# nv-tlabs/ChronoEdit

Measured on AMD Instinct MI355X. Metric: denoising-steps/sec, higher is better.
Workload: dtype bf16

## Files before the change

### chronoedit_amd/csrc/ce_attn.hip

```cpp
#include <cstdlib>

#include "ce_common.h"

namespace {

constexpr int HD = 128;
constexpr int QW = 32;
constexpr int KVB = 64;
constexpr int K_TILE_BYTES = KVB * HD * 2;
constexpr int VT_TILE_BYTES = HD * KVB * 2;
constexpr int BUF_BYTES = K_TILE_BYTES + VT_TILE_BYTES;
constexpr int OST_ROW = HD * 2 + 16;
constexpr int smem_bytes(int nwave, bool two_seg) {
  const int stage = nwave * QW * OST_ROW;
  return two_seg ? 2 * BUF_BYTES + stage : (stage > 2 * BUF_BYTES ? stage : 2 * BUF_BYTES);
}
constexpr float NEG_BIG = -1.0e30f;

__device__ __forceinline__ int vt_swz(int dv) {
  return ((((dv >> 2) & 7) << 1) | (((dv >> 1) ^ (dv >> 5)) & 1)) ^ (((dv >> 6) & 1) << 1);
}

struct KVSeg {
  const bf16* k;
  const bf16* v;
  int len;
  int ldk;
  int ldv;
};
struct BlkRows {
  int rows;
  int stride;
  uint32_t magic;
  int vt_cols;
  unsigned char* q8;
  unsigned char* s8;
  int ld8;
};

template <bool TWO_SEG, int NWAVE>
__global__ __launch_bounds__(NWAVE * 64, NWAVE == 8 ? 2 : 2) void attn_fwd_kernel(const bf16* __restrict__ Q, bf16* __restrict__ O, KVSeg seg0,
                                                       KVSeg seg1, int Nq, int H, int ldq, int ldo, int nqb,
                                                       float scale_log2e) {
  extern __shared__ __attribute__((aligned(16))) unsigned char smem[];
  {
    const size_t bz = blockIdx.y;
    Q += bz * Nq * ldq;
    O += bz * Nq * ldo;
    seg0.k += bz * seg0.len * seg0.ldk;
    seg0.v += bz * seg0.len * seg0.ldv;
    if (TWO_SEG) {
      seg1.k += bz * seg1.len * seg1.ldk;
      seg1.v += bz * seg1.len * seg1.ldv;
    }
  }
  const int tid = threadIdx.x, lane = tid & 63, wave = tid >> 6;
  const int l31 = lane & 31, hh = lane >> 5;

  int head, qb;
  if ((H & 7) == 0) {
    const int xcd = blockIdx.x & 7, local = blockIdx.x >> 3;
    head = xcd + 8 * (local / nqb);
    qb = local % nqb;
  } else {
    head = blockIdx.x / nqb;
    qb = blockIdx.x % nqb;
  }
  constexpr int QB = QW * NWAVE;
  constexpr int NT = NWAVE * 64;
  const int q0 = qb * QB + wave * QW;
  const int hoff = head * HD;

// ... 175 lines not shown
#pragma unroll
  for (int i = 0; i < 8; ++i) {
    const int c = lane + 64 * i;
    const int rl = c >> 4, cc = c & 15;
    const int q = q0 + rl;
    if (q < Nq) {
      const u32x4 v = *reinterpret_cast<const u32x4*>(smem + (TWO_SEG ? 2 * BUF_BYTES : 0) + (size_t)(wave * QW + rl) * OST_ROW + cc * 16);
      *reinterpret_cast<u32x4*>(O + (size_t)q * ldo + hoff + cc * 8) = v;
    }
  }
}


#define CE_EPOCH_BARRIER()                          \
  asm volatile("s_waitcnt lgkmcnt(0)" ::: "memory"); \
  __builtin_amdgcn_s_barrier()
constexpr int PK_ROW = HD * 2 + 16;
constexpr int PV_ROW = KVB * 2 + 16;
constexpr int PK_TILE = KVB * PK_ROW;
constexpr int PV_TILE = HD * PV_ROW;
typedef __attribute__((ext_vector_type(4))) unsigned pp_u4;
typedef __attribute__((ext_vector_type(2))) unsigned pp_u2;

constexpr int K_GRP = 1088;
typedef __attribute__((address_space(3))) void lds_void;
#ifdef CE_DIAGNOSTICS
__device__ unsigned long long g_sp_exact_hits = 0ull;
#endif
constexpr float SP_SPEC_THR = 1024.0f;
constexpr int SP_V0 = 2 * PK_TILE;
constexpr int SP_TILE_BYTES = 2 * PK_TILE + 3 * PV_TILE;
constexpr int sp_smem_bytes(bool two_seg) { return two_seg ? SP_TILE_BYTES + 8 * QW * OST_ROW : SP_TILE_BYTES; }

template <bool TWO_SEG, bool VT = false, bool QOUT = false>
__global__ __launch_bounds__(512, 2) void attn_fwd_sp_kernel(const bf16* __restrict__ Q_, bf16* __restrict__ O_, KVSeg seg0_,
                                                              KVSeg seg1_, int Nq, int H, int ldq, int ldo, int nqb,
                                                              float scale_log2e, int batch, BlkRows blk) {
  extern __shared__ __attribute__((aligned(16))) unsigned char smem[];
  constexpr int NWAVE = 8, QB = QW * NWAVE;
  const int tid = threadIdx.x, lane = tid & 63;
  const int wave = __builtin_amdgcn_readfirstlane(tid >> 6);
  const int l31 = lane & 31, hh = lane >> 5;
  for (int item = blockIdx.x; item < nqb * H * batch; item += gridDim.x) {
  const bf16* Q = Q_;
  bf16* O = O_;
  KVSeg seg0 = seg0_, seg1 = seg1_;

  int head, qb, bz;
  {
    const int nqb_full = Nq / QB;
    if ((H & 7) == 0) {
      const int xcd = item & 7, local = item >> 3, hx_n = H >> 3;
      const int full = batch * hx_n * nqb_full;
      if (local < full) {
        bz = local / (hx_n * nqb_full);
        const int r = local % (hx_n * nqb_full);
        head = xcd + 8 * (r / nqb_full);
        qb = r % nqb_full;
      } else {
        const int l2 = local - full;
        bz = l2 / hx_n;
        head = xcd + 8 * (l2 % hx_n);
        qb = nqb_full;
      }
    } else {
      bz = item / (nqb * H);
      const int r = item % (nqb * H);
      head = r / nqb;
      qb = r % nqb;
    }
  }
  {
    if (VT && blk.rows > 0) {
      Q += (size_t)bz * blk.rows * ldq;
      O += (size_t)bz * blk.rows * ldo;
      seg0.k += (size_t)bz * blk.rows * seg0.ldk;
      seg0.v += (size_t)bz * blk.vt_cols;
    } else {
      Q += (size_t)bz * Nq * ldq;
      O += (size_t)bz * Nq * ldo;
      seg0.k += (size_t)bz * seg0.len * seg0.ldk;
      seg0.v += VT ? (size_t)bz * (TWO_SEG ? blk.vt_cols : seg0.len) : (size_t)bz * seg0.len * seg0.ldv;
    }
    if (TWO_SEG) {
      seg1.k += (size_t)bz * seg1.len * seg1.ldk;
      seg1.v += VT ? (size_t)bz * blk.stride : (size_t)bz * seg1.len * seg1.ldv;
    }
  }
  const int q0 = qb * QB + wave * QW;
  const int hoff = head * HD;
  const bool active = q0 < Nq;
  const int q0row = (VT && blk.rows > 0) ? (q0 / blk.rows) * blk.stride + q0 % blk.rows : q0;

  bf16x8 qf[8];
  {
    const bf16* qrow = Q + (size_t)(q0 + l31 < Nq ? q0row + l31 : 0) * ldq + hoff + 8 * hh;
#pragma unroll
    for (int ks = 0; ks < 8; ++ks) qf[ks] = *reinterpret_cast<const bf16x8*>(qrow + 16 * ks);
  }
  auto scale_q = [&]() __attribute__((always_inline)) {
#pragma unroll
  for (int ks = 0; ks < 8; ++ks) {
    const u32x4 w = __builtin_bit_cast(u32x4, qf[ks]);
    u32x4 o;
#pragma unroll
    for (int i = 0; i < 4; ++i) o[i] = pack_bf16(bf16lo(w[i]) * scale_log2e, bf16hi(w[i]) * scale_log2e);
    qf[ks] = __builtin_bit_cast(bf16x8, o);
  }
#pragma unroll
  for (int ks = 0; ks < 8; ++ks) asm volatile("" : "+v"(qf[ks]));

  };
  const int v_dvq = (tid & 1) | (((tid >> 4) & 15) << 1), v_kvq = ((tid >> 1) & 7) | (((tid >> 8) & 1) << 3);
  const int v_chunk = (v_kvq & ~3) | ((v_kvq & 1) << 1) | ((v_kvq >> 1) & 1);
  unsigned char* ost = smem + (TWO_SEG ? SP_TILE_BYTES : 0) + (size_t)(wave * QW + l31) * OST_ROW;
  const int k_w = l31 & 3;
  const unsigned char* k_rd = smem + (l31 >> 2) * K_GRP + k_w * 256 + ((hh ^ (k_w & 1)) << 4);
  const int k_eo[2] = {(k_w >> 1) << 5, ((k_w >> 1) ^ 1) << 5};
  const unsigned char* v_rd = smem + SP_V0 + l31 * PV_ROW + hh * 16;
  int vt_off[4];
#pragma unroll
  for (int s4 = 0; s4 < 4; ++s4) {
    const int x = (l31 >> 1) & 7;
    vt_off[s4] = l31 * 128 + ((2 * (s4 ^ (x >> 1)) + (hh ^ (x & 1))) << 4);
  }
  unsigned char* v_wr = smem + SP_V0 + (4 * v_dvq) * PV_ROW + v_chunk * 8;

#pragma unroll
  for (int sidx = 0; sidx < (TWO_SEG ? 2 : 1); ++sidx) {
    const KVSeg sg = sidx == 0 ? seg0 : seg1;
    const int ntiles = (sg.len + KVB - 1) / KVB;
    const int k_rows_span = (VT && blk.rows > 0) ? ((sg.len - 1) / blk.rows) * blk.stride + blk.rows : sg.len;
    const auto k_rsrc = __builtin_amdgcn_make_buffer_rsrc((void*)(sg.k + hoff), 0, (k_rows_span - 1) * sg.ldk * 2 + HD * 2, 0x00020000);
// ... 862 lines not shown
CE_API int ce_set_attention_waves(int nwave) {
  const int old = g_attn_nwave;
  if (nwave == 0 || nwave == 4 || nwave == 8 || nwave == 16 || nwave == 64 || nwave == 128 || nwave == 129) g_attn_nwave = nwave;
  return old;
}
#endif

CE_API int ce_attention_batched_bf16(const void* Q, const void* K1, const void* V1, int len1, int ldk1, int ldv1,
                                         const void* K2, const void* V2, int len2, int ldk2, int ldv2, void* O, int Nq, int H,
                                         int head_dim, int ldq, int ldo, float softmax_scale, int batch, hipStream_t stream) {
  if (!Q || !K1 || !V1 || !O) return CE_ERR_ARG;
  if (head_dim != HD || Nq <= 0 || H <= 0 || len1 <= 0 || batch <= 0 || batch > 65535) return CE_ERR_SHAPE;
  if ((ldq & 7) || (ldo & 7) || (ldk1 & 7) || (ldv1 & 3)) return CE_ERR_ALIGN;
  const bool two = (K2 != nullptr && V2 != nullptr && len2 > 0);
  if (two && ((ldk2 & 7) || (ldv2 & 3))) return CE_ERR_ALIGN;
  KVSeg s0{(const bf16*)K1, (const bf16*)V1, len1, ldk1, ldv1};
  KVSeg s1{(const bf16*)K2, (const bf16*)V2, two ? len2 : 0, ldk2, ldv2};
  const float sl2 = softmax_scale * 1.4426950408889634f;
  const bool sp = g_attn_nwave == 64 || g_attn_nwave == 0 || g_attn_nwave >= 128;
  const int nwave = sp ? 8 : g_attn_nwave;
  const int nqb = (Nq + nwave * QW - 1) / (nwave * QW);
  dim3 grid(nqb * H, batch), block(nwave * 64);
  if (sp) {
#define CE_ATTN_SP(TWO)                                                                                              \
  do {                                                                                                               \
    static bool done_[CE_MAX_DEVICES] = {};                                                                          \
    bool& done = done_[ce_device_slot()];                                                                            \
    if (!done) {                                                                                                     \
      (void)hipFuncSetAttribute((const void*)attn_fwd_sp_kernel<TWO>, hipFuncAttributeMaxDynamicSharedMemorySize,    \
                                sp_smem_bytes(TWO));                                                                 \
      done = true;                                                                                                   \
    }                                                                                                                \
    hipLaunchKernelGGL((attn_fwd_sp_kernel<TWO>), dim3(nqb * H * batch), block, sp_smem_bytes(TWO), stream, (const bf16*)Q, \
                       (bf16*)O, s0, s1, Nq, H, ldq, ldo, nqb, sl2, batch, BlkRows{0, 0, 0u, 0});                    \
  } while (0)
    if (two) CE_ATTN_SP(true); else CE_ATTN_SP(false);
#undef CE_ATTN_SP
    return (int)hipGetLastError();
  }
#define CE_ATTN_LAUNCH(TWO, NW)                                                                                     \
  do {                                                                                                              \
    static bool done_[CE_MAX_DEVICES] = {};                                                                         \
    bool& done = done_[ce_device_slot()];                                                                           \
    if (!done) {                                                                                                    \
      (void)hipFuncSetAttribute((const void*)attn_fwd_kernel<TWO, NW>, hipFuncAttributeMaxDynamicSharedMemorySize,  \
                                smem_bytes(NW, TWO));                                                               \
      done = true;                                                                                                  \
    }                                                                                                               \
    hipLaunchKernelGGL((attn_fwd_kernel<TWO, NW>), grid, block, smem_bytes(NW, TWO), stream, (const bf16*)Q, (bf16*)O, \
                       s0, s1, Nq, H, ldq, ldo, nqb, sl2);                                                          \
  } while (0)
  if (two) {
    if (nwave == 8) CE_ATTN_LAUNCH(true, 8); else CE_ATTN_LAUNCH(true, 4);
  } else {
    if (nwave == 8) CE_ATTN_LAUNCH(false, 8); else CE_ATTN_LAUNCH(false, 4);
  }
#undef CE_ATTN_LAUNCH
  return (int)hipGetLastError();
}

CE_API int ce_attention_bf16(const void* Q, const void* K1, const void* V1, int len1, int ldk1, int ldv1, const void* K2,
                                 const void* V2, int len2, int ldk2, int ldv2, void* O, int Nq, int H, int head_dim, int ldq,
                                 int ldo, float softmax_scale, hipStream_t stream) {
  return ce_attention_batched_bf16(Q, K1, V1, len1, ldk1, ldv1, K2, V2, len2, ldk2, ldv2, O, Nq, H, head_dim, ldq, ldo,
                                   softmax_scale, 1, stream);
}

CE_API int ce_v_transpose_bf16(const void* v, int ldv, void* vt, int ldvt, int n_keys, int H, hipStream_t stream) {
  if (!v || !vt) return CE_ERR_ARG;
  if (n_keys <= 0 || H <= 0 || ldvt < n_keys) return CE_ERR_SHAPE;
  if ((ldv & 3) || (ldvt & 7)) return CE_ERR_ALIGN;
  hipLaunchKernelGGL(v_transpose_kernel, dim3((ldvt + KVB - 1) / KVB, H), dim3(256), 0, stream, (const bf16*)v, ldv, (bf16*)vt, ldvt, n_keys, 0, 0, 0);
  return (int)hipGetLastError();
}

CE_API int ce_v_transpose_blocked_bf16(const void* v, int ldv, void* vt, int ldvt, int n_keys, int H, int batch, int blk_rows, int blk_stride,
                                           int vt_sample_cols, hipStream_t stream) {
  if (!v || !vt) return CE_ERR_ARG;
  if (n_keys <= 0 || H <= 0 || batch <= 0 || blk_rows <= 0 || (blk_rows & 63) || blk_stride < batch * blk_rows || (vt_sample_cols & 63) ||
      vt_sample_cols < (n_keys + KVB - 1) / KVB * KVB || ldvt < batch * vt_sample_cols)
    return CE_ERR_SHAPE;
  if ((ldv & 3) || (ldvt & 7)) return CE_ERR_ALIGN;
  hipLaunchKernelGGL(v_transpose_kernel, dim3(vt_sample_cols / KVB, H, batch), dim3(256), 0, stream, (const bf16*)v, ldv, (bf16*)vt, ldvt, n_keys,
                     blk_rows, blk_stride, vt_sample_cols);
  return (int)hipGetLastError();
}

#ifdef CE_DIAGNOSTICS
extern "C" int ce_attn16_launch(const void* Q, const void* K, const void* Vt, int len, int ldk, int ldvt, void* O, int Nq, int H, int ldq, int ldo,
                                float sl2, int batch, int cus, hipStream_t stream);
#endif

static int attention_vt_launch(const void* Q, const void* K, const void* Vt, int len, int ldk, int ldvt, void* O, int Nq, int H, int head_dim,
                               int ldq, int ldo, float softmax_scale, int batch, int blk_rows, int blk_stride, int vt_sample_cols,
                               hipStream_t stream) {
  if (!Q || !K || !Vt || !O) return CE_ERR_ARG;
  if (head_dim != HD || Nq <= 0 || H <= 0 || len <= 0 || batch <= 0 || batch > 65535) return CE_ERR_SHAPE;
  const int ntiles_cols = (len + KVB - 1) / KVB * KVB;
  if (blk_rows == 0) {
    vt_sample_cols = len;
    if (ldvt < (batch - 1) * len + ntiles_cols) return CE_ERR_SHAPE;
  } else {
    if ((blk_rows & 63) || blk_stride < batch * blk_rows || (Nq % blk_rows) || vt_sample_cols < ntiles_cols ||
        ldvt < (batch - 1) * vt_sample_cols + ntiles_cols)
      return CE_ERR_SHAPE;
  }
  if ((ldq & 7) || (ldo & 7) || (ldk & 7) || (ldvt & 7) || (batch > 1 && (vt_sample_cols & 1))) return CE_ERR_ALIGN;
  KVSeg s0{(const bf16*)K, (const bf16*)Vt, len, ldk, ldvt};
  KVSeg s1{nullptr, nullptr, 0, 0, 0};
  BlkRows blk{blk_rows, blk_stride, 0u, vt_sample_cols};
  if (blk_rows > 0) {
    const uint32_t tps = (uint32_t)(blk_rows >> 6);
    blk.magic = tps == 1 ? 0u : (uint32_t)(((1ull << 32) + tps - 1) / tps);
  }
  const float sl2 = softmax_scale * 1.4426950408889634f;
  const int nqb = (Nq + 8 * QW - 1) / (8 * QW);
  static bool done_[CE_MAX_DEVICES] = {};
  bool& done = done_[ce_device_slot()];
  if (!done) {
    (void)hipFuncSetAttribute((const void*)attn_fwd_sp_kernel<false, true>, hipFuncAttributeMaxDynamicSharedMemorySize, sp_smem_bytes(false));
    done = true;
  }
  const int cus = ce_device_cus();
  const int items = nqb * H * batch;
#ifdef CE_DIAGNOSTICS
  if (g_attn_nwave == 16 && blk_rows == 0) {
    const int rc = ce_attn16_launch(Q, K, Vt, len, ldk, ldvt, O, Nq, H, ldq, ldo, sl2, batch, cus, stream);
    if (rc != CE_ERR_ALIGN) return rc;
  }
#endif
  if (g_attn_nwave == 128 || g_attn_nwave == 129) {
    static bool done4_[CE_MAX_DEVICES] = {};
    bool& done4 = done4_[ce_device_slot()];
    if (!done4) {
      (void)hipFuncSetAttribute((const void*)attn_fwd_w4_kernel, hipFuncAttributeMaxDynamicSharedMemorySize, W4_SMEM);
      done4 = true;
    }
    const int grid4 = (g_attn_nwave == 129 && items > cus) ? (cus & ~7) : items;
    hipLaunchKernelGGL(attn_fwd_w4_kernel, dim3(grid4), dim3(256), W4_SMEM, stream, (const bf16*)Q, (bf16*)O, s0, Nq, H, ldq, ldo, nqb,
                       sl2, batch, blk);
    return (int)hipGetLastError();
  }
  const int grid_vt = items <= 2 * cus ? items : ((2 * cus) & ~7);
  hipLaunchKernelGGL((attn_fwd_sp_kernel<false, true>), dim3(grid_vt), dim3(512), sp_smem_bytes(false), stream, (const bf16*)Q, (bf16*)O,
                     s0, s1, Nq, H, ldq, ldo, nqb, sl2, batch, blk);
  return (int)hipGetLastError();
}

CE_API int ce_attention_vt_bf16(const void* Q, const void* K, const void* Vt, int len, int ldk, int ldvt, void* O, int Nq, int H,
                                    int head_dim, int ldq, int ldo, float softmax_scale, int batch, hipStream_t stream) {
  return attention_vt_launch(Q, K, Vt, len, ldk, ldvt, O, Nq, H, head_dim, ldq, ldo, softmax_scale, batch, 0, 0, 0, stream);
}

CE_API int ce_attention_vt_blocked_bf16(const void* Q, const void* K, const void* Vt, int len, int ldk, int ldvt, void* O, int Nq, int H,
                                            int head_dim, int ldq, int ldo, float softmax_scale, int batch, int blk_rows, int blk_stride,
                                            int vt_sample_cols, hipStream_t stream) {
  if (blk_rows <= 0) return CE_ERR_SHAPE;
  return attention_vt_launch(Q, K, Vt, len, ldk, ldvt, O, Nq, H, head_dim, ldq, ldo, softmax_scale, batch, blk_rows, blk_stride, vt_sample_cols,
                             stream);
}


static int attention_2seg_vt_launch(const void* Q, const void* K1, const void* V1t, int len1, int ldk1, int ldv1t, int vt_cols1,
                                    const void* K2, const void* V2t, int len2, int ldk2, int ldv2t, int vt_cols2, void* O, int Nq,
                                    int H, int head_dim, int ldq, int ldo, float softmax_scale, int batch, void* O8, void* S8, int ldo8,
                                    hipStream_t stream) {
  if (!Q || !K1 || !V1t || !K2 || !V2t || (!O && !O8)) return CE_ERR_ARG;
  if (head_dim != HD || Nq <= 0 || H <= 0 || len1 <= 0 || len2 <= 0 || batch <= 0 || batch > 65535) return CE_ERR_SHAPE;
  const int c1 = (len1 + KVB - 1) / KVB * KVB, c2 = (len2 + KVB - 1) / KVB * KVB;
  if (vt_cols1 < len1 || vt_cols2 < len2 || ldv1t < (batch - 1) * vt_cols1 + c1 || ldv2t < (batch - 1) * vt_cols2 + c2) return CE_ERR_SHAPE;
  if ((ldq & 7) || (ldo & 7) || (ldk1 & 7) || (ldk2 & 7) || (ldv1t & 7) || (ldv2t & 7) || (vt_cols1 & 1) || (vt_cols2 & 1)) return CE_ERR_ALIGN;
  KVSeg s0{(const bf16*)K1, (const bf16*)V1t, len1, ldk1, ldv1t};
  KVSeg s1{(const bf16*)K2, (const bf16*)V2t, len2, ldk2, ldv2t};
  const float sl2 = softmax_scale * 1.4426950408889634f;
  const int nqb = (Nq + 8 * QW - 1) / (8 * QW);
  static bool done_[CE_MAX_DEVICES] = {};
  bool& done = done_[ce_device_slot()];
  if (!done) {
    (void)hipFuncSetAttribute((const void*)attn_fwd_sp_kernel<true, true>, hipFuncAttributeMaxDynamicSharedMemorySize, sp_smem_bytes(true));
    (void)hipFuncSetAttribute((const void*)attn_fwd_sp_kernel<true, true, true>, hipFuncAttributeMaxDynamicSharedMemorySize, sp_smem_bytes(true));
    done = true;
  }
  const BlkRows blk{0, vt_cols2, 0u, vt_cols1, (unsigned char*)O8, (unsigned char*)S8, ldo8};
  const int cus = ce_device_cus();
  const int items = nqb * H * batch;
  const int grid = items <= 2 * cus ? items : ((2 * cus) & ~7);
  if (O8)
    hipLaunchKernelGGL((attn_fwd_sp_kernel<true, true, true>), dim3(grid), dim3(512), sp_smem_bytes(true), stream, (const bf16*)Q,
                       (bf16*)O, s0, s1, Nq, H, ldq, ldo, nqb, sl2, batch, blk);
  else
    hipLaunchKernelGGL((attn_fwd_sp_kernel<true, true>), dim3(grid), dim3(512), sp_smem_bytes(true), stream, (const bf16*)Q, (bf16*)O,
                       s0, s1, Nq, H, ldq, ldo, nqb, sl2, batch, blk);
  return (int)hipGetLastError();
}

CE_API int ce_attention_2seg_vt_bf16(const void* Q, const void* K1, const void* V1t, int len1, int ldk1, int ldv1t, int vt_cols1,
                                         const void* K2, const void* V2t, int len2, int ldk2, int ldv2t, int vt_cols2, void* O, int Nq,
                                         int H, int head_dim, int ldq, int ldo, float softmax_scale, int batch, hipStream_t stream) {
  if (!O) return CE_ERR_ARG;
  return attention_2seg_vt_launch(Q, K1, V1t, len1, ldk1, ldv1t, vt_cols1, K2, V2t, len2, ldk2, ldv2t, vt_cols2, O, Nq, H, head_dim, ldq, ldo,
                                  softmax_scale, batch, nullptr, nullptr, 0, stream);
}

CE_API int ce_attention_2seg_vt_quant_bf16(const void* Q, const void* K1, const void* V1t, int len1, int ldk1, int ldv1t, int vt_cols1,
                                               const void* K2, const void* V2t, int len2, int ldk2, int ldv2t, int vt_cols2, void* o8,
                                               void* scale8, int Nq, int H, int head_dim, int ldq, int ldo8, float softmax_scale, int batch,
                                               hipStream_t stream) {
  if (!o8 || !scale8 || (ldo8 & 15) || ((H * head_dim) & 127)) return CE_ERR_ARG;
  return attention_2seg_vt_launch(Q, K1, V1t, len1, ldk1, ldv1t, vt_cols1, K2, V2t, len2, ldk2, ldv2t, vt_cols2, nullptr, Nq, H, head_dim, ldq,
                                  8, softmax_scale, batch, o8, scale8, ldo8, stream);
}
```

### chronoedit_amd/csrc/ce_common.h

```cpp
#pragma once
#include <hip/hip_runtime.h>
#include <stdint.h>

typedef __bf16 bf16;
typedef __attribute__((ext_vector_type(2))) __bf16 bf16x2;
typedef __attribute__((ext_vector_type(4))) __bf16 bf16x4;
typedef __attribute__((ext_vector_type(8))) __bf16 bf16x8;
typedef __attribute__((ext_vector_type(2))) float f32x2;
typedef __attribute__((ext_vector_type(4))) float f32x4;
typedef __attribute__((ext_vector_type(16))) float f32x16;
typedef __attribute__((ext_vector_type(4))) uint32_t u32x4;
typedef __attribute__((ext_vector_type(2))) uint32_t u32x2;

#define CE_WAVE 64

#define CE_API extern "C" __attribute__((visibility("default")))
#ifdef CE_DIAGNOSTICS
#define CE_KNOB static int
#define CE_DIAG_COUNT_EXACT(counter)                                        \
  do {                                                                      \
    if ((threadIdx.x & 63) == 0) atomicAdd(&(counter), 1ull);               \
  } while (0)
#else
#define CE_KNOB static constexpr int
#define CE_DIAG_COUNT_EXACT(counter) do { } while (0)
#endif

#define CE_OK 0
#define CE_ERR_ARG (-1)
#define CE_ERR_SHAPE (-2)
#define CE_ERR_ALIGN (-3)

#define CE_MAX_DEVICES 16
inline int ce_device_slot() {
  int d = 0;
  if (hipGetDevice(&d) != hipSuccess || d < 0 || d >= CE_MAX_DEVICES) d = 0;
  return d;
}

inline int ce_device_cus() {
  static int cus_[CE_MAX_DEVICES] = {};
  int& cus = cus_[ce_device_slot()];
  if (cus == 0) {
    int dev = 0, n = 0;
    cus = (hipGetDevice(&dev) == hipSuccess && hipDeviceGetAttribute(&n, hipDeviceAttributeMultiprocessorCount, dev) == hipSuccess && n > 0) ? n : 256;
  }
  return cus;
}

inline int ce_split_k(int tail, int kt, int cus, long long slab_bytes, long long ws_bytes) {
  if (tail <= 0) return 1;
  for (int s = cus / tail < 8 ? cus / tail : 8; s >= 2; --s)
    if (kt % (2 * s) == 0 && tail * s * slab_bytes <= ws_bytes) return s;
  return 1;
}

inline uint32_t ce_seg_magic(int seg_k, int bk, int kt) {
  if (seg_k <= 0 || seg_k % bk) return 0;
  const int tps = seg_k / bk;
  const uint32_t magic = 65536u / (uint32_t)tps + 1u;
  for (int t = 0; t < kt; ++t)
    if ((int)((uint32_t)t * magic >> 16) != t / tps) return 0;
  return magic;
}

__device__ __forceinline__ float bf16_bits_to_f32(uint32_t bits16) { return __uint_as_float(bits16 << 16); }
__device__ __forceinline__ float bf16lo(uint32_t packed) { return __uint_as_float(packed << 16); }
__device__ __forceinline__ float bf16hi(uint32_t packed) { return __uint_as_float(packed & 0xffff0000u); }

__device__ __forceinline__ uint32_t pack_bf16(float lo, float hi) {
  f32x2 v = {lo, hi};
  bf16x2 r = __builtin_convertvector(v, bf16x2);
  return __builtin_bit_cast(uint32_t, r);
}
__device__ __forceinline__ float round_bf16(float x) {
  bf16 b = (bf16)x;
  return (float)b;
}

__device__ __forceinline__ float mul_then_add(float y, float g, float r) {
#pragma clang fp contract(off)
  const float t = y * g;
  return r + t;
}

__device__ __forceinline__ float wave_sum(float v) {
#pragma unroll
  for (int o = 32; o > 0; o >>= 1) v += __shfl_xor(v, o, 64);
// ... 43 lines not shown
```

### chronoedit_amd/csrc/ce_gemm.hip

```cpp
#include <cmath>

#include "ce_common.h"

#define EPI_BIAS 0
#define EPI_BIAS_GELU 1
#define EPI_GATE_RES 2
#define EPI_BIAS_GELU_ERF 3
#define EPI_F32 4
#define EPI_BIAS_ROW 6
#define EPI_BIAS_T 7
#define EPI_MUL 5

namespace {

constexpr int BM = 128, BN = 128, BK = 64;
constexpr int TILE_BYTES = BM * BK * 2;
constexpr int LDC_BYTES = BN * 2 + 16;

__device__ __forceinline__ int swz_chunk(int row, int chunk) { return chunk ^ ((row >> 1) & 7); }

template <int EPI>
__global__ __launch_bounds__(256) void gemm_bf16_128(const bf16* __restrict__ A, const bf16* __restrict__ W,
                                                     bf16* __restrict__ C, const float* __restrict__ bias,
                                                     const float* __restrict__ gate, const bf16* __restrict__ res, int M,
                                                     int N, int K, int lda, int ldw, int ldc, int ldres, int gate_rows,
                                                     int tiles_m, int tiles_n, int batch0, long long sA0, long long sA1,
                                                     long long sW0, long long sW1, long long sC0, long long sC1,
                                                     int a_seg_tiles, long long a_seg_extra) {
  __shared__ __attribute__((aligned(16))) unsigned char smem[2 * 2 * TILE_BYTES];
  if (gridDim.y > 1) {
    const int z0 = blockIdx.y % batch0, z1 = blockIdx.y / batch0;
    A += z0 * sA0 + z1 * sA1;
    W += z0 * sW0 + z1 * sW1;
    const long long oc = z0 * sC0 + z1 * sC1;
    C = EPI == EPI_F32 ? reinterpret_cast<bf16*>(reinterpret_cast<float*>(C) + oc) : C + oc;
  }
  const int tid = threadIdx.x, lane = tid & 63, wave = tid >> 6;
  const int wm = wave >> 1, wn = wave & 1;

  const int nwg = tiles_m * tiles_n;
  const int wg = xcd_remap(blockIdx.x, nwg);
  constexpr int GROUP = 8;
  const int group_sz = GROUP * tiles_n;
// ... 257 lines not shown
      if (g_gemm_variant == 7 || rows_auto == 288)
        return ce_gemm288_launch(A, W, C, bias, epilogue, gate, res, M, N, K, lda, ldw, ldc, ldres, gate_rows, a_seg_k, a_seg_stride,
                                 w_seg_k, w_seg_stride, slabs, ws_bytes, stream);
      if (g_gemm_variant == 1 || g_gemm_variant == 2)
        return ce_gemm256_launch(A, W, C, bias, epilogue, gate, res, M, N, K, lda, ldw, ldc, ldres, gate_rows, a_seg_k, a_seg_stride,
                                 w_seg_k, w_seg_stride, slabs, ws_bytes, stream);
      return ce_gemm256w4_launch(A, W, C, bias, epilogue, gate, res, M, N, K, lda, ldw, ldc, ldres, gate_rows, a_seg_k, a_seg_stride,
                                 w_seg_k, w_seg_stride, g_gemm_variant == 3 ? 3 : g_gemm_variant == 5 ? 1 : 2, slabs, ws_bytes, stream);
    }
  }
  if (w_seg_k) return CE_ERR_SHAPE;
  const int a_seg_tiles = a_seg_k > 0 ? a_seg_k / BK : 0;
  const long long a_seg_extra = a_seg_k > 0 ? a_seg_stride - a_seg_k : 0;
  const int tiles_m = (M + BM - 1) / BM, tiles_n = (N + BN - 1) / BN;
  dim3 grid(tiles_m * tiles_n), block(256);
#define CE_LAUNCH(E)                                                                                              \
  hipLaunchKernelGGL(gemm_bf16_128<E>, grid, block, 0, stream, (const bf16*)A, (const bf16*)W, (bf16*)C, bias, gate, \
                     (const bf16*)res, M, N, K, lda, ldw, ldc, ldres, gate_rows, tiles_m, tiles_n, 1, 0ll, 0ll, 0ll, 0ll, 0ll, 0ll, \
                     a_seg_tiles, a_seg_extra)
  switch (epilogue) {
    case EPI_BIAS: CE_LAUNCH(EPI_BIAS); break;
    case EPI_BIAS_GELU: CE_LAUNCH(EPI_BIAS_GELU); break;
    case EPI_GATE_RES: CE_LAUNCH(EPI_GATE_RES); break;
    case EPI_BIAS_GELU_ERF: CE_LAUNCH(EPI_BIAS_GELU_ERF); break;
    case EPI_F32: CE_LAUNCH(EPI_F32); break;
    case EPI_MUL: CE_LAUNCH(EPI_MUL); break;
    case EPI_BIAS_ROW: CE_LAUNCH(EPI_BIAS_ROW); break;
    default: return CE_ERR_ARG;
  }
#undef CE_LAUNCH
  return (int)hipGetLastError();
}

CE_API int ce_gemm_batched_bf16(const void* A, const void* W, void* C, const float* bias, int epilogue, int M, int N, int K,
                                    int lda, int ldw, int ldc, int batch0, int batch1, long long sA0, long long sA1, long long sW0,
                                    long long sW1, long long sC0, long long sC1, hipStream_t stream) {
  if (!A || !W || !C) return CE_ERR_ARG;
  if (M <= 0 || N <= 0 || K <= 0 || (K % BK) || (N & 7) || batch0 <= 0 || batch1 <= 0 || (long long)batch0 * batch1 > 65535)
    return CE_ERR_SHAPE;
  if ((lda & 7) || (ldw & 7) || (ldc & 7) || (sA0 & 7) || (sA1 & 7) || (sW0 & 7) || (sW1 & 7) || (sC0 & 7) || (sC1 & 7))
    return CE_ERR_ALIGN;
  if (epilogue != EPI_BIAS && epilogue != EPI_F32) return CE_ERR_ARG;
  const int tiles_m = (M + BM - 1) / BM, tiles_n = (N + BN - 1) / BN;
  dim3 grid(tiles_m * tiles_n, batch0 * batch1), block(256);
#define CE_LAUNCH(E)                                                                                                 \
  hipLaunchKernelGGL(gemm_bf16_128<E>, grid, block, 0, stream, (const bf16*)A, (const bf16*)W, (bf16*)C, bias, nullptr, \
                     nullptr, M, N, K, lda, ldw, ldc, 0, 0, tiles_m, tiles_n, batch0, sA0, sA1, sW0, sW1, sC0, sC1, 0, 0ll)
  if (epilogue == EPI_BIAS) CE_LAUNCH(EPI_BIAS); else CE_LAUNCH(EPI_F32);
#undef CE_LAUNCH
  return (int)hipGetLastError();
}
```

### chronoedit_amd/csrc/ce_gemm256w4.hip

```cpp
#include "ce_common.h"
#include "ce_gemm_epi.h"

namespace {

constexpr int BM = 256, BN = 256, BK = 64;
constexpr int TILE = 256 * BK * 2;
constexpr int CROW = BN * 2 + 16;
constexpr int QROW = 128 * 2 + 16;

typedef __attribute__((address_space(3))) void lds_void;

#define W4_VM(N) asm volatile("s_waitcnt vmcnt(" #N ")" ::: "memory")
#define W4_LGKM0() asm volatile("s_waitcnt lgkmcnt(0)" ::: "memory")
#define W4_BAR() __builtin_amdgcn_s_barrier()
#define W4_PIN() __builtin_amdgcn_sched_barrier(0)

__device__ __forceinline__ void tile_origin_w4(int wg, int tiles_m, int tiles_n, int bn, int& m0, int& n0) {
  constexpr int GROUP = 4;
  const int group_sz = GROUP * tiles_n;
  const int gid = wg / group_sz;
  const int first_m = gid * GROUP;
  const int gm = min(tiles_m - first_m, GROUP);
  m0 = (first_m + (wg % group_sz) % gm) * BM;
  n0 = ((wg % group_sz) / gm) * bn;
}

template <int NG>
struct FragSet {
  bf16x8 a[8], b[NG];
};

#define W4_MMA(F, G, S)                                                                                                      \
  if ((G) < NG) {                                                                                                            \
    if constexpr (REGEPI)                                                                                                    \
      asm volatile("v_mfma_f32_16x16x32_bf16 %0, %1, %2, %0" : "+a"(acc[F][(G) < NG ? (G) : 0]) : "v"((S).a[F]), "v"((S).b[(G) < NG ? (G) : 0])); \
    else                                                                                                                     \
      asm volatile("v_mfma_f32_16x16x32_bf16 %0, %1, %2, %0" : "+a"(acc[F][(G) < NG ? (G) : 0]) : "v"((S).b[(G) < NG ? (G) : 0]), "v"((S).a[F])); \
  }

template <int EPI, int NSA, bool ONEBAR, bool SEG2 = false, int NG = 8>
__global__ __launch_bounds__(256) __attribute__((amdgpu_waves_per_eu(1, 1))) void gemm_bf16_w4(
    const bf16* __restrict__ A, const bf16* __restrict__ W, bf16* __restrict__ C, const float* __restrict__ bias,
    const float* __restrict__ gate, const bf16* __restrict__ res, int M, int N, int K, int lda, int ldw, int ldc, int ldres,
    int gate_rows, int tiles_m, int tiles_n, int t_full, int split, float* __restrict__ ws, uint32_t a_seg_magic,
    uint32_t a_seg_extra, uint32_t w_seg_magic, uint32_t w_seg_extra, uint32_t a_seg2_magic, uint32_t a_seg2_extra) {
  extern __shared__ __attribute__((aligned(16))) unsigned char smem[];
  constexpr int BN = 32 * NG;
  constexpr bool REGEPI = NG == 8;
  constexpr int NW = NG;
  constexpr int WTILE = BN * BK * 2;
  constexpr int CROW = BN * 2 + 16;
  constexpr int W_RING = NSA * TILE;
  const int tid = threadIdx.x, lane = tid & 63;
  const int wave = __builtin_amdgcn_readfirstlane(tid >> 6);
  const int wm = wave >> 1, wn = wave & 1;
  const int fr = lane & 15, fg = lane >> 4;

  const bool partial = (int)blockIdx.x >= t_full;
  int wg, kt0 = 0, ktn = K / BK;
  if (!partial) {
    wg = xcd_remap(blockIdx.x, t_full);
  } else {
    const int tb = blockIdx.x - t_full;
    wg = t_full + tb / split;
    ktn = ktn / split;
    kt0 = (tb % split) * ktn;
  }
  int m0, n0;
  tile_origin_w4(wg, tiles_m, tiles_n, BN, m0, n0);
  const int kt_last = ktn - 1;

  uint32_t a_voff[8], w_voff[8];
#pragma unroll
  for (int p = 0; p < 8; ++p) {
    const int row = 8 * (wave + 4 * p) + (lane >> 3);
    const int chunk = (lane & 7) ^ ((row >> 1) & 7);
    a_voff[p] = (uint32_t)min(m0 + row, M - 1) * (uint32_t)(lda * 2) + chunk * 16;
    const int wrow = REGEPI ? ((row & 128) | ((row & 15) << 3) | ((row & 127) >> 4)) : row;
// ... 114 lines not shown
  asm volatile("s_nop 15\n\ts_nop 15" ::: "memory");
  static_assert(NG == 8 || ((NG == 4 || NG == 3) && NSA == 2 && !ONEBAR), "the 256 x 128 / 256 x 96 tiles exist for the two-stage loop only");
  if constexpr (REGEPI) {
    const int col0 = n0 + wn * 128 + fr * 8;
    const bool col_ok = col0 < N;
    const int colc = min(col0, N - 8);
    const int row_base = m0 + wm * 128 + fg * 4;
    if (partial) {
      float* slab = ws + (size_t)(blockIdx.x - t_full) * (BM * BN);
#pragma unroll
      for (int f = 0; f < 8; ++f) {
        f32x4 av[8];
#pragma unroll
        for (int g = 0; g < 8; ++g) {
          asm volatile("" : "+a"(acc[f][g]));
          av[g] = acc[f][g];
        }
#pragma unroll
        for (int jj = 0; jj < 4; ++jj)
#pragma unroll
          for (int h = 0; h < 2; ++h) {
            const f32x4 o = {av[4 * h + 0][jj], av[4 * h + 1][jj], av[4 * h + 2][jj], av[4 * h + 3][jj]};
            const int lane_o = fg * 4 + jj + 16 * (2 * (fr & 1) + h);
            *reinterpret_cast<f32x4*>(slab + (((wave * 64 + f * 8 + (fr >> 1)) * 64) + lane_o) * 4) = o;
          }
      }
      return;
    }
    f32x4 bvv[2];
#pragma unroll
    for (int h = 0; h < 2; ++h)
      bvv[h] = (EPI != EPI_BIAS_ROW && bias != nullptr) ? *reinterpret_cast<const f32x4*>(bias + colc + 4 * h) : f32x4{0.f, 0.f, 0.f, 0.f};
    const auto c_rsrc = __builtin_amdgcn_make_buffer_rsrc((void*)C, 0, (uint32_t)(M - 1) * (uint32_t)(ldc * 2) + (uint32_t)N * 2u, 0x00020000);
    f32x4 gA[2], gB[2];
    int g_switch = 0x7fffffff;
    u32x4 rv[8][4];
    if (EPI == EPI_GATE_RES) {
      gA[0] = gA[1] = gB[0] = gB[1] = f32x4{1.f, 1.f, 1.f, 1.f};
      if (gate != nullptr) {
        const int s0 = gate_rows > 0 ? m0 / gate_rows : 0;
        const int s1 = gate_rows > 0 ? min(M - 1, m0 + BM - 1) / gate_rows : 0;
        const float* ga = gate + (size_t)s0 * N + colc;
        const float* gb = gate + (size_t)s1 * N + colc;
        gA[0] = *reinterpret_cast<const f32x4*>(ga);
        gA[1] = *reinterpret_cast<const f32x4*>(ga + 4);
        gB[0] = *reinterpret_cast<const f32x4*>(gb);
        gB[1] = *reinterpret_cast<const f32x4*>(gb + 4);
        if (s1 != s0) g_switch = s1 * gate_rows;
      }
#pragma unroll
      for (int f = 0; f < 8; ++f)
#pragma unroll
        for (int jj = 0; jj < 4; ++jj)
          rv[f][jj] = *reinterpret_cast<const u32x4*>(res + (size_t)min(row_base + f * 16 + jj, M - 1) * ldres + colc);
    }
#pragma unroll
    for (int f = 0; f < 8; ++f) {
      f32x4 av[8];
#pragma unroll
      for (int g = 0; g < 8; ++g) {
        asm volatile("" : "+a"(acc[f][g]));
        av[g] = acc[f][g];
      }
      f32x4 brow4 = {0.f, 0.f, 0.f, 0.f};
      if (EPI == EPI_BIAS_ROW) brow4 = *reinterpret_cast<const f32x4*>(bias + min(row_base + f * 16, M - 4));
#pragma unroll
      for (int jj = 0; jj < 4; ++jj) {
        const int m = row_base + f * 16 + jj;
        u32x4 y;
#pragma unroll
        for (int q = 0; q < 4; ++q) {
          const int h = q >> 1, e = 2 * (q & 1);
          const float b0 = EPI == EPI_BIAS_ROW ? brow4[jj] : bvv[h][e], b1 = EPI == EPI_BIAS_ROW ? brow4[jj] : bvv[h][e + 1];
          y[q] = pack_bf16(av[2 * q][jj] + b0, av[2 * q + 1][jj] + b1);
        }
        u32x4 o = y;
        if (EPI == EPI_BIAS_GELU) {
#pragma unroll
          for (int q = 0; q < 4; ++q) o[q] = pack_bf16(gelu_tanh(bf16lo(y[q])), gelu_tanh(bf16hi(y[q])));
        } else if (EPI == EPI_BIAS_GELU_ERF) {
#pragma unroll
          for (int q = 0; q < 4; ++q) o[q] = pack_bf16(gelu_erf(bf16lo(y[q])), gelu_erf(bf16hi(y[q])));
        } else if (EPI == EPI_GATE_RES) {
          const u32x4 r = rv[f][jj];
          const bool second = m >= g_switch;
          const f32x4 g0 = second ? gB[0] : gA[0], g1 = second ? gB[1] : gA[1];
#pragma unroll
          for (int q = 0; q < 4; ++q) {
            const float ga = q < 2 ? g0[2 * q] : g1[2 * q - 4], gb = q < 2 ? g0[2 * q + 1] : g1[2 * q - 3];
            o[q] = pack_bf16(mul_then_add(bf16lo(y[q]), ga, bf16lo(r[q])), mul_then_add(bf16hi(y[q]), gb, bf16hi(r[q])));
          }
        }
        const uint32_t coff = (m < M && col_ok) ? (uint32_t)m * (uint32_t)(ldc * 2) + (uint32_t)col0 * 2u : 0xffffffffu;
        __builtin_amdgcn_raw_buffer_store_b128(o, c_rsrc, coff, 0, 0);
      }
    }
    return;
  }
  W4_BAR();

  if (partial) {
    float* slab = ws + (size_t)(blockIdx.x - t_full) * (BM * BN);
#pragma unroll
    for (int f = 0; f < 8; ++f)
#pragma unroll
      for (int g = 0; g < NG; ++g)
        *reinterpret_cast<f32x4*>(slab + (((wave * 64 + f * 8 + g) * 64) + lane) * 4) = acc[f][g];
    return;
  }
  constexpr int CPR = BN / 8;
  constexpr bool CPOW2 = (CPR & (CPR - 1)) == 0;
  constexpr int RPT = 256 / CPR;
  constexpr int CH = CPOW2 ? 64 * CPR / 256 : (64 + RPT - 1) / RPT;
  const int my_cc = CPOW2 ? (tid & (CPR - 1)) : tid % CPR;
  auto chunk_row = [&](int tt, bool& ok) __attribute__((always_inline)) -> int {
    if (CPOW2) {
      ok = true;
      return (tid + 256 * tt) / CPR;
    }
    const int rl = tid / CPR + RPT * tt;
    ok = tid < RPT * CPR && rl < 64;
    return min(rl, 63);
  };

  f32x4 bcol[NG];
#pragma unroll
  for (int g = 0; g < NG; ++g) {
// ... 97 lines not shown
#pragma unroll
  for (int ff = 0; ff < 2; ++ff) {
    const int f = 2 * w + ff;
    const int rl = f * 16 + fr;
    float brow = 0.f;
    if (EPI == EPI_BIAS_ROW) brow = bias[min(m0 + rl, M - 1)];
#pragma unroll
    for (int g = 0; g < 8; ++g) {
      const int cl = g * 16 + fg * 4;
      f32x4 bv = (EPI != EPI_BIAS_ROW && bias != nullptr) ? *reinterpret_cast<const f32x4*>(bias + min(n0 + cl, N - 4)) : f32x4{0.f, 0.f, 0.f, 0.f};
      if (EPI == EPI_BIAS_ROW) bv[0] = bv[1] = bv[2] = bv[3] = brow;
      const int e = (((q * 64 + f * 8 + g) * 64) + lane) * 4;
      f32x4 v = *reinterpret_cast<const f32x4*>(slab + e);
      for (int sidx = 1; sidx < split; ++sidx) v += *reinterpret_cast<const f32x4*>(slab + (size_t)sidx * (BM * BN) + e);
      const u32x2 pk = {pack_bf16(v[0] + bv[0], v[1] + bv[1]), pack_bf16(v[2] + bv[2], v[3] + bv[3])};
      *reinterpret_cast<u32x2*>(smem + rl * QROW + cl * 2) = pk;
    }
  }
  __syncthreads();
  epi_chunks<EPI, 8>(smem, QROW, [&](int tt, int& rl, int& cc, int& mr) { const int c = tid + 256 * tt; rl = mr = c >> 4; cc = c & 15; }, m0, n0,
                     C, gate, res, M, N, ldc, ldres, gate_rows);
}

}

extern "C" int ce_gemm256_launch(const void* A, const void* W, void* C, const float* bias, int epilogue, const float* gate,
                                 const void* res, int M, int N, int K, int lda, int ldw, int ldc, int ldres, int gate_rows,
                                 int a_seg_k, long long a_seg_stride, int w_seg_k, long long w_seg_stride, float* ws, size_t ws_bytes,
                                 hipStream_t stream);

static int w4_launch(const void* A, const void* W, void* C, const float* bias, int epilogue, const float* gate, const void* res, int M, int N,
                     int K, int lda, int ldw, int ldc, int ldres, int gate_rows, int a_seg_k, long long a_seg_stride, int w_seg_k,
                     long long w_seg_stride, int a_seg2_k, long long a_seg2_stride, int nsa, int ng, float* ws, size_t ws_bytes,
                     hipStream_t stream) {
  const bool seg2 = a_seg2_k > 0;
  if ((ng != 8 && ng != 4 && ng != 3) || (ng != 8 && !seg2)) return CE_ERR_ARG;
  if (seg2 && (a_seg_k <= 0 || a_seg2_k % a_seg_k || (epilogue != EPI_BIAS && epilogue != EPI_GATE_RES) || nsa != 2 ||
               (epilogue == EPI_GATE_RES && gate != nullptr)))
    return CE_ERR_ARG;
  if (epilogue == EPI_GATE_RES && ((gate != nullptr && gate_rows > 0 && gate_rows < BM) || (long long)M * ldc * 2 >= (1ll << 32)))
    return ce_gemm256_launch(A, W, C, bias, epilogue, gate, res, M, N, K, lda, ldw, ldc, ldres, gate_rows, a_seg_k, a_seg_stride, w_seg_k,
                             w_seg_stride, ws, ws_bytes, stream);
  if (ng == 8 && ((long long)M * ldc * 2 >= (1ll << 32) || (epilogue == EPI_BIAS_ROW && (M & 3))))
    return ce_gemm256_launch(A, W, C, bias, epilogue, gate, res, M, N, K, lda, ldw, ldc, ldres, gate_rows, a_seg_k, a_seg_stride, w_seg_k,
                             w_seg_stride, ws, ws_bytes, stream);
  const int bn = 32 * ng;
  const int tiles_m = (M + BM - 1) / BM, tiles_n = (N + bn - 1) / bn;
  const int nwg = tiles_m * tiles_n, kt = K / BK;
  uint32_t a_seg_magic = 0, a_seg_extra = 0, w_seg_magic = 0, w_seg_extra = 0;
  auto seg = [&](int seg_k, long long seg_stride, uint32_t& magic, uint32_t& extra_out) -> int {
    if (seg_k <= 0 || seg_k >= K) return CE_OK;
    magic = ce_seg_magic(seg_k, BK, kt);
    const long long extra = (seg_stride - seg_k) * 2;
    if (!magic || extra < 0 || extra * ((K + seg_k - 1) / seg_k) + (long long)K * 2 >= (1ll << 31)) return CE_ERR_SHAPE;
    extra_out = (uint32_t)extra;
    return CE_OK;
  };
  if (int rc = seg(a_seg_k, a_seg_stride, a_seg_magic, a_seg_extra)) return rc;
  if (int rc = seg(w_seg_k, w_seg_stride, w_seg_magic, w_seg_extra)) return rc;
  uint32_t a_seg2_magic = 0, a_seg2_extra = 0;
  if (seg2 && a_seg2_k < K) {
    a_seg2_magic = ce_seg_magic(a_seg2_k, BK, kt);
    if (!a_seg2_magic) return CE_ERR_SHAPE;
    const long long extra = (a_seg2_stride - (long long)(a_seg2_k / a_seg_k) * a_seg_stride) * 2;
    const long long reach = ((long long)(K - 1) / a_seg2_k) * a_seg2_stride * 2 + (long long)(a_seg2_k / a_seg_k) * a_seg_stride * 2 + (long long)a_seg_k * 2;
    if (extra < 0 || reach >= (1ll << 31)) return CE_ERR_SHAPE;
    a_seg2_extra = (uint32_t)extra;
  }
  const int cus = ce_device_cus();
  int tail = nwg % cus;
  const int split = seg2 ? 1 : ce_split_k(tail, kt, cus, BM * BN * sizeof(float), ws ? (long long)ws_bytes : 0);
  if (split == 1) tail = 0;
  const int t_full2 = nwg - tail;
  dim3 grid(t_full2 + tail * split), block(256);
  const int lds3 = 5 * TILE, lds2 = 4 * TILE;
  if (seg2) {
    const int lds2n = 2 * TILE + 2 * (128 * BK * 2);
    const int lds2m = 2 * TILE + 2 * (96 * BK * 2);
    static bool seg2_done_[CE_MAX_DEVICES] = {};
    bool& seg2_done = seg2_done_[ce_device_slot()];
    if (!seg2_done) {
      if (hipFuncSetAttribute((const void*)gemm_bf16_w4<EPI_BIAS, 2, false, true>, hipFuncAttributeMaxDynamicSharedMemorySize, lds2) != hipSuccess ||
          hipFuncSetAttribute((const void*)gemm_bf16_w4<EPI_GATE_RES, 2, false, true>, hipFuncAttributeMaxDynamicSharedMemorySize, lds2) != hipSuccess ||
          hipFuncSetAttribute((const void*)gemm_bf16_w4<EPI_BIAS, 2, false, true, 4>, hipFuncAttributeMaxDynamicSharedMemorySize, lds2n) != hipSuccess ||
          hipFuncSetAttribute((const void*)gemm_bf16_w4<EPI_GATE_RES, 2, false, true, 4>, hipFuncAttributeMaxDynamicSharedMemorySize, lds2n) != hipSuccess ||
          hipFuncSetAttribute((const void*)gemm_bf16_w4<EPI_BIAS, 2, false, true, 3>, hipFuncAttributeMaxDynamicSharedMemorySize, lds2m) != hipSuccess ||
          hipFuncSetAttribute((const void*)gemm_bf16_w4<EPI_GATE_RES, 2, false, true, 3>, hipFuncAttributeMaxDynamicSharedMemorySize, lds2m) != hipSuccess)
        return CE_ERR_ARG;
      seg2_done = true;
    }
#define CE_LAUNCH_SEG2(E, NGV, LDS)                                                                                                     \
  hipLaunchKernelGGL((gemm_bf16_w4<E, 2, false, true, NGV>), grid, block, LDS, stream, (const bf16*)A, (const bf16*)W, (bf16*)C, bias, gate, \
                     (const bf16*)res, M, N, K, lda, ldw, ldc, ldres, gate_rows, tiles_m, tiles_n, t_full2, split, ws, a_seg_magic,   \
                     a_seg_extra, w_seg_magic, w_seg_extra, a_seg2_magic, a_seg2_extra)
    if (epilogue == EPI_BIAS) {
      if (ng == 8) CE_LAUNCH_SEG2(EPI_BIAS, 8, lds2); else if (ng == 4) CE_LAUNCH_SEG2(EPI_BIAS, 4, lds2n); else CE_LAUNCH_SEG2(EPI_BIAS, 3, lds2m);
    } else {
      if (ng == 8) CE_LAUNCH_SEG2(EPI_GATE_RES, 8, lds2); else if (ng == 4) CE_LAUNCH_SEG2(EPI_GATE_RES, 4, lds2n); else CE_LAUNCH_SEG2(EPI_GATE_RES, 3, lds2m);
    }
#undef CE_LAUNCH_SEG2
    return (int)hipGetLastError();
  }
  static bool attr_done_[CE_MAX_DEVICES][8] = {};
  bool* attr_done = attr_done_[ce_device_slot()];
#define CE_LAUNCH(E)                                                                                                       \
  do {                                                                                                                     \
    if (!attr_done[E]) {                                                                                                   \
      if (hipFuncSetAttribute((const void*)gemm_bf16_w4<E, 3, false>, hipFuncAttributeMaxDynamicSharedMemorySize, lds3) != hipSuccess) return CE_ERR_ARG; \
      if (hipFuncSetAttribute((const void*)gemm_bf16_w4<E, 3, true>, hipFuncAttributeMaxDynamicSharedMemorySize, lds3) != hipSuccess) return CE_ERR_ARG; \
      if (hipFuncSetAttribute((const void*)gemm_bf16_w4<E, 2, false>, hipFuncAttributeMaxDynamicSharedMemorySize, lds2) != hipSuccess) return CE_ERR_ARG; \
      (void)hipFuncSetAttribute((const void*)gemm256w4_reduce<E>, hipFuncAttributeMaxDynamicSharedMemorySize, 128 * QROW); \
      attr_done[E] = true;                                                                                                 \
    }                                                                                                                      \
    if (nsa == 1)                                                                                                          \
      hipLaunchKernelGGL((gemm_bf16_w4<E, 3, true>), grid, block, lds3, stream, (const bf16*)A, (const bf16*)W, (bf16*)C, bias, gate, \
                         (const bf16*)res, M, N, K, lda, ldw, ldc, ldres, gate_rows, tiles_m, tiles_n, t_full2, split, ws, \
                         a_seg_magic, a_seg_extra, w_seg_magic, w_seg_extra, 0u, 0u);                                      \
    else if (nsa == 3)                                                                                                     \
      hipLaunchKernelGGL((gemm_bf16_w4<E, 3, false>), grid, block, lds3, stream, (const bf16*)A, (const bf16*)W, (bf16*)C, bias, gate, \
                         (const bf16*)res, M, N, K, lda, ldw, ldc, ldres, gate_rows, tiles_m, tiles_n, t_full2, split, ws, \
                         a_seg_magic, a_seg_extra, w_seg_magic, w_seg_extra, 0u, 0u);                                      \
    else                                                                                                                   \
      hipLaunchKernelGGL((gemm_bf16_w4<E, 2, false>), grid, block, lds2, stream, (const bf16*)A, (const bf16*)W, (bf16*)C, bias, gate, \
                         (const bf16*)res, M, N, K, lda, ldw, ldc, ldres, gate_rows, tiles_m, tiles_n, t_full2, split, ws, \
                         a_seg_magic, a_seg_extra, w_seg_magic, w_seg_extra, 0u, 0u);                                      \
    if (tail)                                                                                                              \
      hipLaunchKernelGGL((gemm256w4_reduce<E>), dim3(4 * tail), block, 128 * QROW, stream, (bf16*)C, bias, gate,           \
                         (const bf16*)res, M, N, ldc, ldres, gate_rows, tiles_m, tiles_n, t_full2, split, ws);           \
  } while (0)
  switch (epilogue) {
    case EPI_BIAS: CE_LAUNCH(EPI_BIAS); break;
    case EPI_BIAS_GELU: CE_LAUNCH(EPI_BIAS_GELU); break;
    case EPI_GATE_RES: CE_LAUNCH(EPI_GATE_RES); break;
    case EPI_BIAS_GELU_ERF: CE_LAUNCH(EPI_BIAS_GELU_ERF); break;
    case EPI_BIAS_ROW: CE_LAUNCH(EPI_BIAS_ROW); break;
    default: return CE_ERR_ARG;
  }
#undef CE_LAUNCH
  return (int)hipGetLastError();
}

extern "C" int ce_gemm256w4_launch(const void* A, const void* W, void* C, const float* bias, int epilogue, const float* gate,
                                   const void* res, int M, int N, int K, int lda, int ldw, int ldc, int ldres, int gate_rows,
                                   int a_seg_k, long long a_seg_stride, int w_seg_k, long long w_seg_stride, int nsa, float* ws,
                                   size_t ws_bytes, hipStream_t stream) {
  return w4_launch(A, W, C, bias, epilogue, gate, res, M, N, K, lda, ldw, ldc, ldres, gate_rows, a_seg_k, a_seg_stride, w_seg_k, w_seg_stride,
                   0, 0, nsa, 8, ws, ws_bytes, stream);
}

extern "C" int ce_gemm256w4_seg2_launch(const void* A, const void* W, void* C, const float* bias, int epilogue, const void* res, int M, int N,
                                        int K, int lda, int ldw, int ldc, int ldres, int a_seg_k, long long a_seg_stride, int a_seg2_k,
                                        long long a_seg2_stride, int n_tile, hipStream_t stream) {
  return w4_launch(A, W, C, bias, epilogue, nullptr, res, M, N, K, lda, ldw, ldc, ldres, 0, a_seg_k, a_seg_stride, 0, 0, a_seg2_k, a_seg2_stride,
                   2, n_tile / 32, nullptr, 0, stream);
}

extern "C" int ce_gemm256w4_reduce_launch(int epilogue, void* C, const float* bias, const float* gate, const void* res, int M, int N, int ldc,
                                          int ldres, int gate_rows, int tiles_m, int tiles_n, int t_full, int split, const float* ws, int tail,
                                          hipStream_t stream) {
  static bool done_[CE_MAX_DEVICES][8] = {};
  bool* done = done_[ce_device_slot()];
#define CE_RED(E)                                                                                                            \
  do {                                                                                                                       \
    if (!done[E]) {                                                                                                          \
      (void)hipFuncSetAttribute((const void*)gemm256w4_reduce<E>, hipFuncAttributeMaxDynamicSharedMemorySize, 128 * QROW);    \
      done[E] = true;                                                                                                        \
    }                                                                                                                        \
    hipLaunchKernelGGL((gemm256w4_reduce<E>), dim3(4 * tail), dim3(256), 128 * QROW, stream, (bf16*)C, bias, gate, (const bf16*)res, M, N, \
                       ldc, ldres, gate_rows, tiles_m, tiles_n, t_full, split, ws);                                          \
  } while (0)
  switch (epilogue) {
    case EPI_BIAS: CE_RED(EPI_BIAS); break;
// ... 8 lines not shown
```

### chronoedit_amd/csrc/ce_gemm384.hip

```cpp
#include "ce_common.h"
#include "ce_gemm_epi.h"

namespace {

constexpr int BN = 256, BK = 64;
constexpr int W_TILE = BN * BK * 2;
template <int NF> struct T384 {
  static constexpr int BM = 32 * NF;
  static constexpr int A_TILE = BM * BK * 2;
  static constexpr int STAGE = A_TILE + W_TILE;
  static constexpr int NG = 2 * NF;
  static constexpr int NP = NF + 8;
};
constexpr int CROW = BN * 2 + 16;
constexpr int QROW = 128 * 2 + 16;

typedef __attribute__((address_space(3))) void lds_void;

#define X_BAR() __builtin_amdgcn_s_barrier()
#define X_PIN() __builtin_amdgcn_sched_barrier(0)

template <int BM>
__device__ __forceinline__ void tile_origin_384(int wg, int tiles_m, int tiles_n, int& m0, int& n0) {
  constexpr int GROUP = 4;
  const int group_sz = GROUP * tiles_n;
  const int gid = wg / group_sz;
  const int first_m = gid * GROUP;
  const int gm = min(tiles_m - first_m, GROUP);
  m0 = (first_m + (wg % group_sz) % gm) * BM;
  n0 = ((wg % group_sz) / gm) * BN;
}

template <int F>
__device__ __forceinline__ void mma1(f32x4& acc, const bf16x8& b, const bf16x8& a) {
  if constexpr (F < 8)
    asm volatile("v_mfma_f32_16x16x32_bf16 %0, %1, %2, %0" : "+a"(acc) : "v"(a), "v"(b));
  else
    asm volatile("v_mfma_f32_16x16x32_bf16 %0, %1, %2, %0" : "+v"(acc) : "v"(a), "v"(b));
}

template <int EPI, int NF = 12>
__global__ __launch_bounds__(256) __attribute__((amdgpu_waves_per_eu(1, 1))) void gemm_bf16_384(
    const bf16* __restrict__ A, const bf16* __restrict__ W, bf16* __restrict__ C, const float* __restrict__ bias,
    const float* __restrict__ gate, const bf16* __restrict__ res, int M, int N, int K, int lda, int ldw, int ldc, int ldres,
    int gate_rows, int tiles_m, int tiles_n, int t_full, int split, float* __restrict__ ws, uint32_t a_seg_magic,
    uint32_t a_seg_extra, uint32_t w_seg_magic, uint32_t w_seg_extra) {
  constexpr int BM = T384<NF>::BM, A_TILE = T384<NF>::A_TILE, STAGE = T384<NF>::STAGE, NG = T384<NF>::NG, NP = T384<NF>::NP;
  static_assert(NF >= 9 && NF <= 12, "the W fragments of the second k-step are read in groups 1..8 of the first; rows 8.. of the accumulator live in 128 VGPRs");
  extern __shared__ __attribute__((aligned(16))) unsigned char smem[];
  const int tid = threadIdx.x, lane = tid & 63;
  const int wave = __builtin_amdgcn_readfirstlane(tid >> 6);
  const int wm = wave >> 1, wn = wave & 1;
  const int fr = lane & 15, fg = lane >> 4;

#ifdef G384_STAGGER_CYC
  if (blockIdx.x < 256) {
    const long long t0 = __builtin_readcyclecounter();
    const long long wait = (long long)((blockIdx.x >> 3) & 3) * G384_STAGGER_CYC;
    while (__builtin_readcyclecounter() - t0 < wait) __builtin_amdgcn_s_sleep(8);
  }
#endif
  const bool partial = (int)blockIdx.x >= t_full;
  int wg, kt0 = 0, ktn = K / BK;
  if (!partial) {
    wg = xcd_remap(blockIdx.x, t_full);
  } else {
    const int tb = blockIdx.x - t_full;
    wg = t_full + tb / split;
    ktn = ktn / split;
    kt0 = (tb % split) * ktn;
  }
  int m0, n0;
  tile_origin_384<BM>(wg, tiles_m, tiles_n, m0, n0);
  const int kt_last = ktn - 1;

  const int prow = 8 * wave + (lane >> 3);
  const uint32_t pchunk = (uint32_t)(((lane & 7) ^ ((prow >> 1) & 7)) << 4);
  const uint32_t a_off0 = (uint32_t)(m0 + prow) * (uint32_t)(lda * 2) + pchunk, a_lim = (uint32_t)(M - 1) * (uint32_t)(lda * 2) + pchunk;
  const uint32_t w_rowb = (uint32_t)(ldw * 2);
// ... 177 lines not shown
        asm volatile("s_waitcnt lgkmcnt(0)" ::: "memory");
#pragma unroll
        for (int i = 0; i < 16; ++i) {
          const int r = 8 * i + (lane >> 3), c = lane & 7;
          const u32x4 v = *reinterpret_cast<const u32x4*>(tb + r * TROW + c * 16);
          const int n = n_base + r, m = m_base + pass * 64 + c * 8;
          const uint32_t toff = (n < N && m < M) ? (uint32_t)n * (uint32_t)(ldc * 2) + (uint32_t)m * 2u : 0xffffffffu;
          __builtin_amdgcn_raw_buffer_store_b128(v, t_rsrc, toff, 0, 0);
        }
        asm volatile("s_waitcnt lgkmcnt(0)" ::: "memory");
      }
      return;
    }
#pragma unroll
    for (int f = 0; f < NF; ++f) {
      f32x4 av[8];
#pragma unroll
      for (int g = 0; g < 8; ++g) {
        if (f < 8) asm volatile("" : "+a"(acc[f][g])); else asm volatile("" : "+v"(acc[f][g]));
        av[g] = acc[f][g];
      }
      const int m = row_base + f * 16;
#pragma unroll
      for (int g = 0; g < 8; ++g) {
        const float b = bvv[g >> 2][g & 3];
        const u32x2 y = {pack_bf16(av[g][0] + b, av[g][1] + b), pack_bf16(av[g][2] + b, av[g][3] + b)};
        const uint32_t toff = (m < M && col_ok) ? (uint32_t)(col0 + g) * (uint32_t)(ldc * 2) + (uint32_t)m * 2u : 0xffffffffu;
        __builtin_amdgcn_raw_buffer_store_b64(y, t_rsrc, toff, 0, 0);
      }
    }
    return;
  }
  const auto c_rsrc = __builtin_amdgcn_make_buffer_rsrc((void*)C, 0, (uint32_t)(M - 1) * (uint32_t)(ldc * 2) + (uint32_t)N * 2u, 0x00020000);
  f32x4 gA[2], gB[2];
  int g_switch = 0x7fffffff;
  constexpr int RA = 2;
  u32x4 rv[RA + 1][4];
  auto res_load = [&](int f, u32x4* dst) __attribute__((always_inline)) {
#pragma unroll
    for (int jj = 0; jj < 4; ++jj) dst[jj] = *reinterpret_cast<const u32x4*>(res + (size_t)min(row_base + f * 16 + jj, M - 1) * ldres + colc);
  };
  if (EPI == EPI_GATE_RES) {
    gA[0] = gA[1] = gB[0] = gB[1] = f32x4{1.f, 1.f, 1.f, 1.f};
    if (gate != nullptr) {
      const int s0 = gate_rows > 0 ? m0 / gate_rows : 0;
      const int s1 = gate_rows > 0 ? min(M - 1, m0 + BM - 1) / gate_rows : 0;
      const float* ga = gate + (size_t)s0 * N + colc;
      const float* gb = gate + (size_t)s1 * N + colc;
      gA[0] = *reinterpret_cast<const f32x4*>(ga);
      gA[1] = *reinterpret_cast<const f32x4*>(ga + 4);
      gB[0] = *reinterpret_cast<const f32x4*>(gb);
      gB[1] = *reinterpret_cast<const f32x4*>(gb + 4);
      if (s1 != s0) g_switch = s1 * gate_rows;
    }
#pragma unroll
    for (int f = 0; f < RA; ++f) res_load(f, rv[f % (RA + 1)]);
  }
#pragma unroll
  for (int f = 0; f < NF; ++f) {
    if (EPI == EPI_GATE_RES && f + RA < NF) res_load(f + RA, rv[(f + RA) % (RA + 1)]);
    f32x4 av[8];
#pragma unroll
    for (int g = 0; g < 8; ++g) {
      if (f < 8) asm volatile("" : "+a"(acc[f][g])); else asm volatile("" : "+v"(acc[f][g]));
      av[g] = acc[f][g];
    }
    f32x4 brow4 = {0.f, 0.f, 0.f, 0.f};
    if (EPI == EPI_BIAS_ROW) brow4 = *reinterpret_cast<const f32x4*>(bias + min(row_base + f * 16, M - 4));
#pragma unroll
    for (int jj = 0; jj < 4; ++jj) {
      const int m = row_base + f * 16 + jj;
      u32x4 y;
#pragma unroll
      for (int q = 0; q < 4; ++q) {
        const int h = q >> 1, e = 2 * (q & 1);
        const float b0 = EPI == EPI_BIAS_ROW ? brow4[jj] : bvv[h][e], b1 = EPI == EPI_BIAS_ROW ? brow4[jj] : bvv[h][e + 1];
        y[q] = pack_bf16(av[2 * q][jj] + b0, av[2 * q + 1][jj] + b1);
      }
      u32x4 o = y;
      if (EPI == EPI_BIAS_GELU) {
#pragma unroll
        for (int q = 0; q < 4; ++q) o[q] = pack_bf16(gelu_tanh(bf16lo(y[q])), gelu_tanh(bf16hi(y[q])));
      } else if (EPI == EPI_BIAS_GELU_ERF) {
#pragma unroll
        for (int q = 0; q < 4; ++q) o[q] = pack_bf16(gelu_erf(bf16lo(y[q])), gelu_erf(bf16hi(y[q])));
      } else if (EPI == EPI_GATE_RES) {
        const u32x4 r = rv[f % (RA + 1)][jj];
        const bool second = m >= g_switch;
        const f32x4 g0 = second ? gB[0] : gA[0], g1 = second ? gB[1] : gA[1];
#pragma unroll
        for (int q = 0; q < 4; ++q) {
          const float ga = q < 2 ? g0[2 * q] : g1[2 * q - 4], gb = q < 2 ? g0[2 * q + 1] : g1[2 * q - 3];
          o[q] = pack_bf16(mul_then_add(bf16lo(y[q]), ga, bf16lo(r[q])), mul_then_add(bf16hi(y[q]), gb, bf16hi(r[q])));
        }
      }
      const uint32_t coff = (m < M && col_ok) ? (uint32_t)m * (uint32_t)(ldc * 2) + (uint32_t)col0 * 2u : 0xffffffffu;
      __builtin_amdgcn_raw_buffer_store_b128(o, c_rsrc, coff, 0, 0);
    }
  }
}

template <int EPI, int NF = 12>
__global__ __launch_bounds__(256) void gemm384_reduce(bf16* __restrict__ C, const float* __restrict__ bias, const float* __restrict__ gate,
                                                      const bf16* __restrict__ res, int M, int N, int ldc, int ldres, int gate_rows,
                                                      int tiles_m, int tiles_n, int t_full, int split, const float* __restrict__ ws) {
  extern __shared__ __attribute__((aligned(16))) unsigned char smem[];
  const int tid = threadIdx.x, lane = tid & 63, w = tid >> 6;
  const int fr = lane & 15, fg = lane >> 4;
  const int tile = blockIdx.x >> 2, q = blockIdx.x & 3;
  constexpr int BM = T384<NF>::BM;
  int m0, n0;
  tile_origin_384<BM>(t_full + tile, tiles_m, tiles_n, m0, n0);
  m0 += (q >> 1) * (16 * NF);
  n0 += (q & 1) * 128;
  const float* slab = ws + (size_t)tile * split * (BM * BN);
#pragma unroll
  for (int ff = 0; ff < 3; ++ff) {
    const int f = 3 * w + ff;
    if (f >= NF) break;
    const int rl = f * 16 + fr;
    float brow = 0.f;
    if (EPI == EPI_BIAS_ROW) brow = bias[min(m0 + rl, M - 1)];
#pragma unroll
    for (int g = 0; g < 8; ++g) {
      const int cl = g * 16 + fg * 4;
      f32x4 bv = (EPI != EPI_BIAS_ROW && bias != nullptr) ? *reinterpret_cast<const f32x4*>(bias + min(n0 + cl, N - 4)) : f32x4{0.f, 0.f, 0.f, 0.f};
      if (EPI == EPI_BIAS_ROW) bv[0] = bv[1] = bv[2] = bv[3] = brow;
      const int e = (((q * (8 * NF) + f * 8 + g) * 64) + lane) * 4;
      f32x4 v = *reinterpret_cast<const f32x4*>(slab + e);
      for (int sidx = 1; sidx < split; ++sidx) v += *reinterpret_cast<const f32x4*>(slab + (size_t)sidx * (BM * BN) + e);
      const u32x2 pk = {pack_bf16(v[0] + bv[0], v[1] + bv[1]), pack_bf16(v[2] + bv[2], v[3] + bv[3])};
      *reinterpret_cast<u32x2*>(smem + rl * QROW + cl * 2) = pk;
    }
  }
  __syncthreads();
  epi_chunks<EPI, NF>(smem, QROW, [&](int tt, int& rl, int& cc, int& mr) { const int c = tid + 256 * tt; rl = mr = c >> 4; cc = c & 15; }, m0, n0,
                      C, gate, res, M, N, ldc, ldres, gate_rows);
}

}

extern "C" int ce_gemm256_launch(const void* A, const void* W, void* C, const float* bias, int epilogue, const float* gate,
                                 const void* res, int M, int N, int K, int lda, int ldw, int ldc, int ldres, int gate_rows,
                                 int a_seg_k, long long a_seg_stride, int w_seg_k, long long w_seg_stride, float* ws, size_t ws_bytes,
                                 hipStream_t stream);

template <int NF>
static int gemm384_launch_impl(const void* A, const void* W, void* C, const float* bias, int epilogue, const float* gate, const void* res, int M, int N,
                               int K, int lda, int ldw, int ldc, int ldres, int gate_rows, int a_seg_k, long long a_seg_stride, int w_seg_k,
                               long long w_seg_stride, float* ws, size_t ws_bytes, hipStream_t stream) {
  constexpr int BM = T384<NF>::BM, STAGE = T384<NF>::STAGE;
  if (epilogue == EPI_BIAS_T) {
    if ((M & 7) || (long long)N * ldc * 2 >= (1ll << 32) || !bias) return CE_ERR_SHAPE;
  } else
  if ((epilogue == EPI_GATE_RES && gate != nullptr && gate_rows > 0 && gate_rows < BM) || (long long)M * ldc * 2 >= (1ll << 32) ||
      (epilogue == EPI_BIAS_ROW && (M & 3)))
    return ce_gemm256_launch(A, W, C, bias, epilogue, gate, res, M, N, K, lda, ldw, ldc, ldres, gate_rows, a_seg_k, a_seg_stride, w_seg_k,
                             w_seg_stride, ws, ws_bytes, stream);
  const int tiles_m = (M + BM - 1) / BM, tiles_n = (N + BN - 1) / BN;
  const int nwg = tiles_m * tiles_n, kt = K / BK;
  uint32_t a_seg_magic = 0, a_seg_extra = 0, w_seg_magic = 0, w_seg_extra = 0;
  auto seg = [&](int seg_k, long long seg_stride, uint32_t& magic, uint32_t& extra_out) -> int {
    if (seg_k <= 0 || seg_k >= K) return CE_OK;
    magic = ce_seg_magic(seg_k, BK, kt);
    const long long extra = (seg_stride - seg_k) * 2;
    if (!magic || extra < 0 || extra * (K / seg_k) + (long long)K * 2 >= (1ll << 31)) return CE_ERR_SHAPE;
    extra_out = (uint32_t)extra;
    return CE_OK;
  };
  if (int rc = seg(a_seg_k, a_seg_stride, a_seg_magic, a_seg_extra)) return rc;
  if (int rc = seg(w_seg_k, w_seg_stride, w_seg_magic, w_seg_extra)) return rc;
  const int cus = ce_device_cus();
  int tail = nwg % cus;
  const int split = epilogue == EPI_BIAS_T ? 1 : ce_split_k(tail, kt, cus, BM * BN * sizeof(float), ws ? (long long)ws_bytes : 0);
  if (split == 1) tail = 0;
  const int t_full2 = nwg - tail;
  dim3 grid(t_full2 + tail * split), block(256);
  const int lds = 2 * STAGE;
  static bool attr_done_[CE_MAX_DEVICES][8] = {};
  bool* attr_done = attr_done_[ce_device_slot()];
#define CE_LAUNCH(E)                                                                                                       \
  do {                                                                                                                     \
    if (!attr_done[E]) {                                                                                                   \
      if (hipFuncSetAttribute((const void*)gemm_bf16_384<E, NF>, hipFuncAttributeMaxDynamicSharedMemorySize, lds) != hipSuccess) return CE_ERR_ARG; \
      (void)hipFuncSetAttribute((const void*)gemm384_reduce<E, NF>, hipFuncAttributeMaxDynamicSharedMemorySize, 16 * NF * QROW); \
      attr_done[E] = true;                                                                                                 \
    }                                                                                                                      \
    hipLaunchKernelGGL((gemm_bf16_384<E, NF>), grid, block, lds, stream, (const bf16*)A, (const bf16*)W, (bf16*)C, bias, gate, \
                       (const bf16*)res, M, N, K, lda, ldw, ldc, ldres, gate_rows, tiles_m, tiles_n, t_full2, split, ws, \
                       a_seg_magic, a_seg_extra, w_seg_magic, w_seg_extra);                                                \
    if (tail)                                                                                                              \
      hipLaunchKernelGGL((gemm384_reduce<E, NF>), dim3(4 * tail), block, 16 * NF * QROW, stream, (bf16*)C, bias, gate,     \
                         (const bf16*)res, M, N, ldc, ldres, gate_rows, tiles_m, tiles_n, t_full2, split, ws);           \
  } while (0)
  switch (epilogue) {
    case EPI_BIAS: CE_LAUNCH(EPI_BIAS); break;
    case EPI_BIAS_GELU: CE_LAUNCH(EPI_BIAS_GELU); break;
    case EPI_GATE_RES: CE_LAUNCH(EPI_GATE_RES); break;
    case EPI_BIAS_GELU_ERF: CE_LAUNCH(EPI_BIAS_GELU_ERF); break;
    case EPI_BIAS_ROW: CE_LAUNCH(EPI_BIAS_ROW); break;
    case EPI_BIAS_T: {
      static bool t_done_[CE_MAX_DEVICES] = {};
      bool& t_done = t_done_[ce_device_slot()];
      if (!t_done) {
        if (hipFuncSetAttribute((const void*)gemm_bf16_384<EPI_BIAS_T, NF>, hipFuncAttributeMaxDynamicSharedMemorySize, lds) != hipSuccess) return CE_ERR_ARG;
        t_done = true;
      }
      hipLaunchKernelGGL((gemm_bf16_384<EPI_BIAS_T, NF>), grid, block, lds, stream, (const bf16*)A, (const bf16*)W, (bf16*)C, bias, gate, (const bf16*)res,
                         M, N, K, lda, ldw, ldc, ldres, gate_rows, tiles_m, tiles_n, t_full2, split, ws, a_seg_magic, a_seg_extra, w_seg_magic,
                         w_seg_extra);
      break;
    }
    default: return CE_ERR_ARG;
  }
#undef CE_LAUNCH
  return (int)hipGetLastError();
}

extern "C" int ce_gemm384_launch(const void* A, const void* W, void* C, const float* bias, int epilogue, const float* gate,
                                 const void* res, int M, int N, int K, int lda, int ldw, int ldc, int ldres, int gate_rows,
                                 int a_seg_k, long long a_seg_stride, int w_seg_k, long long w_seg_stride, float* ws, size_t ws_bytes,
                                 hipStream_t stream) {
  return gemm384_launch_impl<12>(A, W, C, bias, epilogue, gate, res, M, N, K, lda, ldw, ldc, ldres, gate_rows, a_seg_k, a_seg_stride, w_seg_k,
                                 w_seg_stride, ws, ws_bytes, stream);
}

extern "C" int ce_gemm288_launch(const void* A, const void* W, void* C, const float* bias, int epilogue, const float* gate,
                                 const void* res, int M, int N, int K, int lda, int ldw, int ldc, int ldres, int gate_rows,
                                 int a_seg_k, long long a_seg_stride, int w_seg_k, long long w_seg_stride, float* ws, size_t ws_bytes,
                                 hipStream_t stream) {
  return gemm384_launch_impl<9>(A, W, C, bias, epilogue, gate, res, M, N, K, lda, ldw, ldc, ldres, gate_rows, a_seg_k, a_seg_stride, w_seg_k,
                                w_seg_stride, ws, ws_bytes, stream);
}
```

### chronoedit_amd/csrc/ce_gemm_epi.h

```cpp
#pragma once
#include "ce_common.h"

#ifndef EPI_BIAS
#define EPI_BIAS 0
#define EPI_BIAS_GELU 1
#define EPI_GATE_RES 2
#define EPI_BIAS_GELU_ERF 3
#endif
#ifndef EPI_BIAS_ROW
#define EPI_BIAS_ROW 6
#endif
#ifndef EPI_BIAS_T
#define EPI_BIAS_T 7
#endif

namespace {

template <int EPI, int NCH, bool HAS_GATE, typename RowCol>
__device__ __forceinline__ void epi_chunks_impl(const unsigned char* smem, int row_bytes, RowCol rowcol, int m0, int n0,
                                                bf16* __restrict__ C, const float* __restrict__ gate, const bf16* __restrict__ res,
                                                int M, int N, int ldc, int ldres, int gate_rows) {
  u32x4 v[NCH], rv[NCH];
  f32x4 g0[NCH], g1[NCH];
  int ms[NCH], ns[NCH];
#pragma unroll
  for (int t = 0; t < NCH; ++t) {
    int rl, cc, mr;
    rowcol(t, rl, cc, mr);
    ms[t] = m0 + mr;
    ns[t] = n0 + cc * 8;
    v[t] = *reinterpret_cast<const u32x4*>(smem + rl * row_bytes + cc * 16);
    if (EPI == EPI_GATE_RES) {
      const int mc = min(ms[t], M - 1), nc = min(ns[t], N - 8);
      rv[t] = *reinterpret_cast<const u32x4*>(res + (size_t)mc * ldres + nc);
      if (HAS_GATE) {
        const float* gp = gate + (gate_rows > 0 ? (size_t)(mc / gate_rows) * N : 0) + nc;
        g0[t] = *reinterpret_cast<const f32x4*>(gp);
        g1[t] = *reinterpret_cast<const f32x4*>(gp + 4);
      }
    }
  }
#pragma unroll
  for (int t = 0; t < NCH; ++t) {
    u32x4 o = v[t];
    if (EPI == EPI_BIAS_GELU) {
#pragma unroll
      for (int q = 0; q < 4; ++q) o[q] = pack_bf16(gelu_tanh(bf16lo(o[q])), gelu_tanh(bf16hi(o[q])));
    } else if (EPI == EPI_BIAS_GELU_ERF) {
#pragma unroll
// ... 24 lines not shown
```

### chronoedit_amd/csrc/ce_rowops.hip

```cpp
#include "ce_common.h"

#define ROW_MAXC 10
#ifndef CE_LN_ROWS
#define CE_LN_ROWS 2
#endif

template <int FP8, bool FULL, int R>
__global__ __launch_bounds__(256) void ln_affine_kernel(const bf16* __restrict__ x, bf16* __restrict__ y,
                                                        const float* __restrict__ a, const float* __restrict__ b,
                                                        int M, int D, int ldx, int ldy, float eps, int ab_rows, int ab_stride,
                                                        unsigned char* __restrict__ q8, float* __restrict__ qscale, int ldq) {
  const int lane = threadIdx.x & 63;
  const int row0 = (blockIdx.x * 4 + (threadIdx.x >> 6)) * R;
  if (row0 >= M) return;
  if (ab_rows > 0) {
    a += (size_t)(row0 / ab_rows) * ab_stride;
    b += (size_t)(row0 / ab_rows) * ab_stride;
  }
  const int nch = D >> 3;
  u32x4 raw[R][ROW_MAXC];
  float mean[R], rstd[R];
#pragma unroll
  for (int k = 0; k < R; ++k) {
    const bf16* xr = x + (size_t)min(row0 + k, M - 1) * ldx;
// ... 79 lines not shown
          if ((lane & 3) == 0) reinterpret_cast<unsigned char*>(qscale)[mx_gemm_scale_offset(row0 + k, c >> 2, D >> 7)] = (unsigned char)byte;
        }
      }
    }
  }
  if (FP8 == 1) {
#pragma unroll
    for (int k = 0; k < R; ++k) {
      const float am = wave_max(amax[k]);
      const float sc = am > 0.f ? am * (1.0f / 448.0f) : 1.0f;
      const float inv = 1.0f / sc;
      if (row0 + k >= M) continue;
      if (lane == 0) qscale[row0 + k] = sc;
      unsigned char* qr = q8 + (size_t)(row0 + k) * ldq;
#pragma unroll
      for (int i = 0; i < ROW_MAXC; ++i) {
        const int c = lane + 64 * i;
        if (FULL || c < nch) {
          const u32x4 v = raw[k][i];
          int w0 = 0, w1 = 0;
          w0 = __builtin_amdgcn_cvt_pk_fp8_f32(bf16lo(v[0]) * inv, bf16hi(v[0]) * inv, w0, false);
          w0 = __builtin_amdgcn_cvt_pk_fp8_f32(bf16lo(v[1]) * inv, bf16hi(v[1]) * inv, w0, true);
          w1 = __builtin_amdgcn_cvt_pk_fp8_f32(bf16lo(v[2]) * inv, bf16hi(v[2]) * inv, w1, false);
          w1 = __builtin_amdgcn_cvt_pk_fp8_f32(bf16lo(v[3]) * inv, bf16hi(v[3]) * inv, w1, true);
          u32x2 o = {(uint32_t)w0, (uint32_t)w1};
          *reinterpret_cast<u32x2*>(qr + c * 8) = o;
        }
      }
    }
  }
}

template <bool FULL>
__global__ __launch_bounds__(256) void rmsnorm_rope_kernel(bf16* __restrict__ x0, const float* __restrict__ w0,
                                                           bf16* __restrict__ x1, const float* __restrict__ w1,
                                                           const float* __restrict__ cs, int M, int D, int ld,
                                                           int head_dim, float eps, int rope_rows) {
  const int lane = threadIdx.x & 63;
  const int row = blockIdx.x * 4 + (threadIdx.x >> 6);
  if (row >= M) return;
  bf16* __restrict__ x = blockIdx.y ? x1 : x0;
  const float* __restrict__ w = blockIdx.y ? w1 : w0;
  const int cs_row = rope_rows > 0 ? row % rope_rows : row;
  const int nch = D >> 3;
  bf16* xr = x + (size_t)row * ld;
  u32x4 raw[ROW_MAXC];
  float s = 0.f;
#pragma unroll
  for (int i = 0; i < ROW_MAXC; ++i) {
    const int c = lane + 64 * i;
    if (FULL || c < nch) {
      raw[i] = *reinterpret_cast<const u32x4*>(xr + c * 8);
#pragma unroll
      for (int j = 0; j < 4; ++j) {
        const float v0 = bf16lo(raw[i][j]), v1 = bf16hi(raw[i][j]);
        s += v0 * v0 + v1 * v1;
      }
    }
  }
  const float rstd = 1.0f / sqrtf(wave_sum(s) / (float)D + eps);
  const int half = head_dim >> 1;
  const bool cs_once = cs != nullptr && (512 % head_dim) == 0;
  f32x4 csa = {0.f, 0.f, 0.f, 0.f}, csb = {0.f, 0.f, 0.f, 0.f};
  if (cs_once) {
    const float* p = cs + ((size_t)cs_row * half + (((lane * 8) % head_dim) >> 1)) * 2;
    csa = *reinterpret_cast<const f32x4*>(p);
    csb = *reinterpret_cast<const f32x4*>(p + 4);
  }
#pragma unroll
  for (int i = 0; i < ROW_MAXC; ++i) {
    const int c = lane + 64 * i;
    if (FULL || c < nch) {
      const f32x4 w0 = *reinterpret_cast<const f32x4*>(w + c * 8), w1 = *reinterpret_cast<const f32x4*>(w + c * 8 + 4);
      u32x4 o;
      f32x4 cs0 = csa, cs1 = csb;
      if (cs != nullptr && !cs_once) {
        const int pair0 = ((c * 8) % head_dim) >> 1;
        const float* p = cs + ((size_t)cs_row * half + pair0) * 2;
        cs0 = *reinterpret_cast<const f32x4*>(p);
        cs1 = *reinterpret_cast<const f32x4*>(p + 4);
      }
#pragma unroll
      for (int j = 0; j < 4; ++j) {
        const float ww0 = j < 2 ? w0[2 * j] : w1[2 * j - 4], ww1 = j < 2 ? w0[2 * j + 1] : w1[2 * j - 3];
        float v0 = round_bf16(round_bf16(bf16lo(raw[i][j]) * rstd) * ww0);
        float v1 = round_bf16(round_bf16(bf16hi(raw[i][j]) * rstd) * ww1);
        if (cs != nullptr) {
          const float co = j < 2 ? cs0[2 * j] : cs1[2 * j - 4], si = j < 2 ? cs0[2 * j + 1] : cs1[2 * j - 3];
          const float r0 = v0 * co - v1 * si, r1 = v0 * si + v1 * co;
          v0 = r0;
          v1 = r1;
        }
        o[j] = pack_bf16(v0, v1);
      }
      *reinterpret_cast<u32x4*>(xr + c * 8) = o;
    }
  }
}

template <bool FULL>
__global__ __launch_bounds__(256) void rope_scatter_kernel(const bf16* __restrict__ x, int ldx, bf16* __restrict__ send,
                                                           int M, int D, int W, int nt, int col0, const float* __restrict__ w0,
                                                           int col1, const float* __restrict__ w1, int col2,
                                                           const float* __restrict__ w2, const float* __restrict__ cs,
                                                           int head_dim, float eps, int rope_rows) {
  const int lane = threadIdx.x & 63;
  const int row = blockIdx.x * 4 + (threadIdx.x >> 6);
  if (row >= M) return;
  const int ti = blockIdx.y;
  const int col = ti == 0 ? col0 : ti == 1 ? col1 : col2;
  const float* __restrict__ w = ti == 0 ? w0 : ti == 1 ? w1 : w2;
  const int cs_row = rope_rows > 0 ? row % rope_rows : row;
  const int nch = D >> 3;
  const int Dl = D / W;
  const bf16* xr = x + (size_t)row * ldx + col;
  u32x4 raw[ROW_MAXC];
  float s = 0.f;
#pragma unroll
  for (int i = 0; i < ROW_MAXC; ++i) {
    const int c = lane + 64 * i;
    if (FULL || c < nch) {
      raw[i] = *reinterpret_cast<const u32x4*>(xr + c * 8);
#pragma unroll
      for (int j = 0; j < 4; ++j) {
        const float v0 = bf16lo(raw[i][j]), v1 = bf16hi(raw[i][j]);
        s += v0 * v0 + v1 * v1;
      }
    }
  }
  const float rstd = 1.0f / sqrtf(wave_sum(s) / (float)D + eps);
// ... 159 lines not shown
                       ldx, 0, eps, ab_rows, ab_stride, (unsigned char*)q, scale, ldq);
  else
    hipLaunchKernelGGL((ln_affine_kernel<1, false, 1>), dim3((M + 3) / 4), dim3(256), 0, stream, (const bf16*)x, nullptr, a, b, M, D,
                       ldx, 0, eps, ab_rows, ab_stride, (unsigned char*)q, scale, ldq);
  return (int)hipGetLastError();
}

CE_API int ce_ln_affine_mxfp8(const void* x, void* q, void* scale8, const float* a, const float* b, int M, int D, int ldx, int ldq, float eps,
                                  int ab_rows, int ab_stride, hipStream_t stream) {
  if (!x || !q || !scale8 || !a || !b) return CE_ERR_ARG;
  if (M <= 0 || D <= 0 || (D & 127) || D > 64 * 8 * ROW_MAXC || (ldx & 7) || (ldq & 7) || (ab_rows > 0 && (ab_stride & 3))) return CE_ERR_SHAPE;
  if (D == 64 * 8 * ROW_MAXC)
    hipLaunchKernelGGL((ln_affine_kernel<2, true, 1>), dim3((M + 3) / 4), dim3(256), 0, stream, (const bf16*)x, nullptr, a, b, M, D, ldx, 0, eps,
                       ab_rows, ab_stride, (unsigned char*)q, (float*)scale8, ldq);
  else
    hipLaunchKernelGGL((ln_affine_kernel<2, false, 1>), dim3((M + 3) / 4), dim3(256), 0, stream, (const bf16*)x, nullptr, a, b, M, D, ldx, 0, eps,
                       ab_rows, ab_stride, (unsigned char*)q, (float*)scale8, ldq);
  return (int)hipGetLastError();
}

CE_API int ce_rmsnorm_rope_bf16(void* x, const float* w, void* x2, const float* w2, const float* cos_sin, int M, int D, int ld,
                                    int head_dim, float eps, int rope_rows, hipStream_t stream) {
  if (!x || !w || (x2 && !w2)) return CE_ERR_ARG;
  if (M <= 0 || D <= 0 || (D & 7) || D > 64 * 8 * ROW_MAXC || (ld & 7) || (head_dim & 7) || D % head_dim) return CE_ERR_SHAPE;
  if (D == 64 * 8 * ROW_MAXC)
    hipLaunchKernelGGL(rmsnorm_rope_kernel<true>, dim3((M + 3) / 4, x2 ? 2 : 1), dim3(256), 0, stream, (bf16*)x, w, (bf16*)x2, w2,
                       cos_sin, M, D, ld, head_dim, eps, rope_rows);
  else
    hipLaunchKernelGGL(rmsnorm_rope_kernel<false>, dim3((M + 3) / 4, x2 ? 2 : 1), dim3(256), 0, stream, (bf16*)x, w, (bf16*)x2, w2,
                       cos_sin, M, D, ld, head_dim, eps, rope_rows);
  return (int)hipGetLastError();
}

CE_API int ce_timestep_sinusoid(const int64_t* t, float* out, int dim, hipStream_t stream) {
  if (!t || !out || dim <= 0 || (dim & 1)) return CE_ERR_ARG;
  hipLaunchKernelGGL(timestep_sinusoid_kernel<int64_t>, dim3((dim + 255) / 256), dim3(256), 0, stream, t, out, dim);
  return (int)hipGetLastError();
}

CE_API int ce_timestep_sinusoid_f32(const float* t, float* out, int dim, hipStream_t stream) {
  if (!t || !out || dim <= 0 || (dim & 1)) return CE_ERR_ARG;
  hipLaunchKernelGGL(timestep_sinusoid_kernel<float>, dim3((dim + 255) / 256), dim3(256), 0, stream, t, out, dim);
  return (int)hipGetLastError();
}

CE_API int ce_gemv(const void* W, int w_is_bf16, const float* x, const float* bias, float* y, int N, int K, int flags,
                       hipStream_t stream) {
  if (!W || !x || !y || N <= 0 || K <= 0) return CE_ERR_ARG;
  if (K > 16384) return CE_ERR_SHAPE;
  if (w_is_bf16)
    hipLaunchKernelGGL(gemv_kernel<bf16>, dim3((N + GEMV_ROWS - 1) / GEMV_ROWS), dim3(256), (size_t)K * 4, stream, (const bf16*)W, x, bias, y,
                       N, K, flags);
  else
    hipLaunchKernelGGL(gemv_kernel<float>, dim3((N + GEMV_ROWS - 1) / GEMV_ROWS), dim3(256), (size_t)K * 4, stream, (const float*)W, x, bias,
                       y, N, K, flags);
  return (int)hipGetLastError();
}

CE_API int ce_modulation(const float* table, const float* v, float* mod, int L, int J, int D, int v_rows, int one_mask,
                             hipStream_t stream) {
  if (!table || !v || !mod || L <= 0 || J <= 0 || D <= 0 || (v_rows != 1 && v_rows != J)) return CE_ERR_ARG;
  const size_t total = (size_t)L * J * D;
  hipLaunchKernelGGL(modulation_kernel, dim3((unsigned)((total + 255) / 256)), dim3(256), 0, stream, table, v, mod, L, J, D,
                     v_rows, one_mask);
  return (int)hipGetLastError();
}
// ... 39 lines not shown
```

### chronoedit_amd/hiplib.py

```python
from __future__ import annotations

import ctypes
import os
import re
import subprocess
from typing import Dict, List

PKG_DIR = os.path.dirname(os.path.abspath(__file__))
ROOT = os.path.dirname(PKG_DIR)
CSRC = os.path.join(PKG_DIR, "csrc")
LIB_DIR = os.path.join(PKG_DIR, "lib")
LIB_PATH = os.path.join(LIB_DIR, "libchronoedit_hip.so")
DIAG_LIB_PATH = os.path.join(LIB_DIR, "libchronoedit_hip_diag.so")
OBJ_DIR = os.path.join(LIB_DIR, "obj")
HEADER = os.path.join(ROOT, "include", "chronoedit_hip.h")
DIAG_HEADER = os.path.join(ROOT, "include", "chronoedit_hip_diag.h")

DIAG_SOURCES = ["ce_gemm.hip", "ce_gemm256.hip", "ce_attn.hip", "ce_attn_fp8.hip", "ce_gemm_fp8.hip", "ce_gemm_fp8w4.hip"]
DIAG_ONLY_SOURCES = ["ce_attn16.hip"]
SOURCES = ["ce_rowops.hip", "ce_gemm.hip", "ce_gemm256.hip", "ce_gemm256w4.hip", "ce_gemm384.hip", "ce_attn.hip", "ce_attn16.hip", "ce_attn_fp8.hip", "ce_sched.hip", "ce_conv.hip", "ce_enc.hip", "ce_gemm_fp8.hip", "ce_gemm_fp8w4.hip", "ce_comm.hip"]

_c = ctypes
_P, _I, _F = _c.c_void_p, _c.c_int, _c.c_float

SIGNATURES: Dict[str, List] = {
    "ce_ln_affine_bf16": [_P, _P, _P, _P, _I, _I, _I, _I, _F, _I, _I, _P],
    "ce_rmsnorm_rope_bf16": [_P, _P, _P, _P, _P, _I, _I, _I, _I, _F, _I, _P],
    "ce_gemm_bf16": [_P, _P, _P, _P, _I, _P, _P, _I, _I, _I, _I, _I, _I, _I, _I, _I, _c.c_longlong, _I, _c.c_longlong, _P, _c.c_size_t, _P],
    "ce_rmsnorm_rope_mxfp8": [_P, _P, _P, _P, _P, _I, _I, _I, _I, _I, _F, _I, _F, _P],
    "ce_v_mxfp8_transpose": [_P, _I, _P, _P, _I, _I, _I, _I, _P],
    "ce_attention_mxfp8": [_P, _P, _P, _P, _P, _P, _P, _I, _I, _I, _I, _I, _I, _I, _I, _I, _P],
    "ce_attention_mxfp8_quant": [_P, _P, _P, _P, _P, _P, _P, _P, _I, _I, _I, _I, _I, _I, _I, _I, _I, _P],
    "ce_attention_mxfp8_add": [_P, _P, _P, _P, _P, _P, _P, _I, _P, _I, _P, _P, _I, _I, _I, _I, _I, _I, _I, _I, _I, _P],
    "ce_rope_scatter_bf16": [_P, _I, _P, _I, _I, _I, _I, _I, _P, _I, _P, _I, _P, _P, _I, _F, _I, _P],
    "ce_patchify_rows_bf16": [_P, _P, _I, _I, _I, _I, _I, _I, _I, _P],
    "ce_comm_load": [ctypes.c_char_p],
    "ce_comm_unique_id": [_P],
    "ce_comm_init": [ctypes.POINTER(ctypes.c_void_p), _P, _I, _I],
    "ce_comm_destroy": [_P],
    "ce_comm_all_to_all": [_P, _P, _P, ctypes.c_size_t, _P],
    "ce_comm_all_gather": [_P, _P, _P, ctypes.c_size_t, _P],
    "ce_ln_affine_fp8": [_P, _P, _P, _P, _P, _I, _I, _I, _I, _F, _I, _I, _P],
    "ce_quant_rows_fp8": [_P, _P, _P, _I, _I, _I, _I, _P],
    "ce_gemm_fp8": [_P, _P, _P, _P, _P, _P, _I, _P, _P, _I, _I, _I, _I, _I, _I, _I, _I, _P, _c.c_size_t, _P],
    "ce_quant_rows_mxfp8": [_P, _P, _P, _I, _I, _I, _I, _P],
    "ce_quant_rows_mxfp8_w": [_P, _P, _P, _I, _I, _I, _I, _P],
    "ce_ln_affine_mxfp8": [_P, _P, _P, _P, _P, _I, _I, _I, _I, _F, _I, _I, _P],
    "ce_gemm_mxfp8": [_P, _P, _P, _P, _P, _P, _I, _P, _P, _I, _I, _I, _I, _I, _I, _I, _I, _P, _c.c_size_t, _P],
    "ce_gemm_mxfp8_gelu_quant": [_P, _P, _P, _P, _P, _P, _P, _I, _I, _I, _I, _I, _I, _P, _c.c_size_t, _P],
    "ce_gemm_batched_bf16": [_P, _P, _P, _P, _I, _I, _I, _I, _I, _I, _I, _I, _I] + [ctypes.c_longlong] * 6 + [_P],
    "ce_im2col_patch2d_bf16": [_P, _P, _I, _I, _I, _I, _I, _I, _P],
    "ce_gather_rows_bf16": [_P, _P, _P, _I, _I, _I, _I, _I, _P],
    "ce_rmsnorm_bf16": [_P, _P, _P, _I, _I, _I, _I, _F, _P],
    "ce_softmax_t5_bf16": [_P, _P, _I, _I, _I, _I, _I, _I, _P, _P, _P, _P],
    "ce_attention_bf16": [_P, _P, _P, _I, _I, _I, _P, _P, _I, _I, _I, _P, _I, _I, _I, _I, _I, _F, _P],
    "ce_attention_batched_bf16": [_P, _P, _P, _I, _I, _I, _P, _P, _I, _I, _I, _P, _I, _I, _I, _I, _I, _F, _I, _P],
    "ce_attention_vt_bf16": [_P, _P, _P, _I, _I, _I, _P, _I, _I, _I, _I, _I, _F, _I, _P],
    "ce_attention_2seg_vt_bf16": [_P, _P, _P, _I, _I, _I, _I, _P, _P, _I, _I, _I, _I, _P, _I, _I, _I, _I, _I, _F, _I, _P],
    "ce_attention_2seg_vt_quant_bf16": [_P, _P, _P, _I, _I, _I, _I, _P, _P, _I, _I, _I, _I, _P, _P, _I, _I, _I, _I, _I, _F, _I, _P],
    "ce_v_transpose_bf16": [_P, _I, _P, _I, _I, _I, _P],
    "ce_attention_vt_blocked_bf16": [_P, _P, _P, _I, _I, _I, _P, _I, _I, _I, _I, _I, _F, _I, _I, _I, _I, _P],
    "ce_v_transpose_blocked_bf16": [_P, _I, _P, _I, _I, _I, _I, _I, _I, _I, _P],
    "ce_timestep_sinusoid": [_P, _P, _I, _P],
    "ce_timestep_sinusoid_f32": [_P, _P, _I, _P],
    "ce_gemv": [_P, _I, _P, _P, _P, _I, _I, _I, _P],
    "ce_modulation": [_P, _P, _P, _I, _I, _I, _I, _I, _P],
    "ce_patchify_bf16": [_P, _P, _I, _I, _I, _I, _I, _P],
    "ce_unpatchify_bf16": [_P, _P, _I, _I, _I, _I, _I, _P],
    "ce_conv_igemm_bf16": [_P, _I, _P, _P, _P, _I, _P] + [_I] * 16 + [_P],
    "ce_conv3d_head_bf16": [_P, _I, _P, _P, _P, _I] + [_I] * 10 + [_P],
    "ce_gemm_bf16_tile_rows": [_I, _I, _I, _I, _c.c_longlong],
    "ce_zero_border_bf16": [_P, _I, _I, _I, _I, _I, _P],
    "ce_conv3d_gemm_bf16": [_P, _P, _I, _P, _P, _P, _I, _I, _I, _I, _I, _I, _I, _I, _P],
    "ce_conv3d_gemm_rms_silu_bf16": [_P, _P, _I, _P, _P, _P, _P, _I, _I, _I, _I, _I, _I, _I, _P, _I, _P],
    "ce_rms_silu_bf16": [_P, _P, _P, _c.c_longlong, _I, _I, _I, _I, _I, _I, _P],
    "ce_upsample2x_bf16": [_P, _P, _I, _I, _I, _I, _P],
    "ce_softmax_rows_f32_bf16": [_P, _P, _I, _I, _I, _I, _I, _F, _P],
    "ce_attention_1head_bf16": [_P, _P, _P, _P, _I, _I, _I, _I, _I, _I, _I, _F, _P, _c.c_longlong, _P],
    "ce_cfg_unipc_step": [_P, _P, _P, _P, _P, _P, _P, _P, _P, _c.c_longlong, _I, _P],
    "ce_build_info": [],
}
DIAG_SIGNATURES: Dict[str, List] = {
    "ce_set_gemm_variant": [_I],
    "ce_set_attention_waves": [_I],
    "ce_set_gemm_fp8_variant": [_I],
    "ce_set_attention_mxfp8_variant": [_I],
    "ce_set_attention_mxfp8_persistent": [_I],
    "ce_diag_attention_exact_route_hits": [_P, _I],
}


def header_symbols(diag: bool = False) -> List[str]:
    txt = open(DIAG_HEADER if diag else HEADER).read()
    return re.findall(r"^int (ce_\w+)\(", txt, flags=re.M)


def exported_symbols(path: str) -> List[str]:
    nm = "/opt/rocm/lib/llvm/bin/llvm-nm" if os.path.exists("/opt/rocm/lib/llvm/bin/llvm-nm") else "nm"
    out = subprocess.run([nm, "-D", "--defined-only", path], check=True, capture_output=True, text=True).stdout
    return sorted(l.split()[-1] for l in out.splitlines() if l.split() and l.split()[-2] in ("T", "t", "W", "D", "B"))


HIPCC_FLAGS = ["--offload-arch=gfx950", "-O3", "-std=c++17", "-fPIC", "-fvisibility=hidden"]


def build(force: bool = False, verbose: bool = False, jobs: int = 0) -> str:
    import glob
    from concurrent.futures import ThreadPoolExecutor
    srcs = [s for s in SOURCES if os.path.exists(os.path.join(CSRC, s))]
    hdrs = sorted(glob.glob(os.path.join(CSRC, "*.h"))) + [HEADER, DIAG_HEADER]
    hdr_m = max(os.path.getmtime(d) for d in hdrs)
    os.makedirs(OBJ_DIR, exist_ok=True)
    hipcc = os.environ.get("HIPCC", "/opt/rocm/bin/hipcc")
    todo, objs, diag_objs = [], [], []
    for s_ in srcs:
        src, stem = os.path.join(CSRC, s_), s_[:-4]
        variants = [("", [])] + ([(".diag", ["-DCE_DIAGNOSTICS"])] if s_ in DIAG_SOURCES else [])
        for tag, defs in variants:
            obj = os.path.join(OBJ_DIR, stem + tag + ".o")
            if force or not os.path.exists(obj) or os.path.getmtime(obj) < max(os.path.getmtime(src), hdr_m):
                todo.append([hipcc, *HIPCC_FLAGS, *defs, "-I", CSRC, "-c", src, "-o", obj])
# ... 79 lines not shown
```

### chronoedit_amd/ops.py

```python
from __future__ import annotations

import ctypes
from typing import Optional

import torch

from . import hiplib

EPI_BIAS, EPI_BIAS_GELU, EPI_GATE_RES, EPI_BIAS_GELU_ERF = 0, 1, 2, 3
EPI_F32, EPI_MUL, EPI_BIAS_ROW, EPI_BIAS_T = 4, 5, 6, 7

_lib = None
_product = None

_KNOB_DEFAULTS = {"ce_set_gemm_variant": -1, "ce_set_attention_waves": 0, "ce_set_gemm_fp8_variant": 1,
                  "ce_set_attention_mxfp8_variant": 1, "ce_set_attention_mxfp8_persistent": 512}
_knobs = dict(_KNOB_DEFAULTS)


def lib():
    global _lib, _product
    if _lib is None:
        _lib = _product = hiplib.load()
        import os
# ... 150 lines not shown
        S, M, Ks = a.shape
        if a.stride(2) != 1 or a.stride(1) < Ks:
            raise ValueError(f"gemm: segmented a needs unit inner stride, got {a.stride()}")
        K, lda, a_seg_k, a_seg_stride = S * Ks, a.stride(1), Ks, a.stride(0)
    else:
        M, K, lda = _rows(a, "a")
    N, K2, ldw = _rows(w, "w")
    if K != K2:
        raise ValueError(f"gemm: K mismatch {K} vs {K2}")
    if bias is not None:
        _dev(bias, torch.float32, "bias")
        assert bias.numel() == (M if epilogue == EPI_BIAS_ROW else N) and bias.is_contiguous()
    oshape = (N, M) if epilogue == EPI_BIAS_T else (M, N)
    if out is None:
        out = torch.empty(oshape, dtype=torch.bfloat16, device=a.device)
    _dev(out, torch.bfloat16, "out")
    Mo, No, ldc = _rows(out, "out")
    assert (Mo, No) == oshape, ((Mo, No), oshape)
    ldres = 0
    if epilogue in (EPI_GATE_RES, EPI_MUL):
        if res is None:
            raise ValueError("EPI_GATE_RES / EPI_MUL need res")
        _dev(res, torch.bfloat16, "res")
        _, _, ldres = _rows(res, "res")
        if gate is not None:
            _dev(gate, torch.float32, "gate")
            assert gate.is_contiguous() and gate.numel() == (N if gate_rows <= 0 else (M + gate_rows - 1) // gate_rows * N)
    ws, ws_bytes = _gemm_scratch(a.device)
    st = _prof_begin()
    _check(lib().ce_gemm_bf16(_ptr(a), _ptr(w), _ptr(out), _ptr(bias), epilogue, _ptr(gate), _ptr(res), M, N, K, lda, ldw, ldc, ldres,
                              int(gate_rows), int(a_seg_k), int(a_seg_stride), 0, 0, ws, ws_bytes, _stream()), "ce_gemm_bf16")
    _prof_end(st, f"gemm_{M}x{N}x{K}_epi{epilogue}", 2.0 * M * N * K)
    return out


def rope_scatter(x: torch.Tensor, cols, weights, D: int, world: int, cos_sin: Optional[torch.Tensor], head_dim: int, eps: float,
                 out: Optional[torch.Tensor] = None):
    _dev(x, torch.bfloat16, "x")
    M, _, ldx = _rows(x, "x")
    nt = len(cols)
    assert 1 <= nt <= 3 and len(weights) == nt
    for w in weights:
        if w is not None:
            _dev(w, torch.float32, "w")
            assert w.is_contiguous() and w.numel() == D
    rope_rows = 0
    if cos_sin is not None:
        _dev(cos_sin, torch.float32, "cos_sin")
        assert cos_sin.is_contiguous() and cos_sin.shape[1:] == (head_dim // 2, 2) and M % cos_sin.shape[0] == 0
        rope_rows = cos_sin.shape[0]
    if out is None:
        out = torch.empty((world, M, nt, D // world), dtype=torch.bfloat16, device=x.device)
    _dev(out, torch.bfloat16, "out")
    assert out.is_contiguous() and out.numel() == M * nt * D
    c = list(cols) + [0] * (3 - nt)
    w = list(weights) + [None] * (3 - nt)
    st = _prof_begin()
    _check(lib().ce_rope_scatter_bf16(_ptr(x), ldx, _ptr(out), M, D, world, nt, c[0], _ptr(w[0]), c[1], _ptr(w[1]), c[2], _ptr(w[2]),
                                      _ptr(cos_sin), head_dim, float(eps), rope_rows, _stream()), "ce_rope_scatter_bf16")
    _prof_end(st, f"rope_scatter_{M}x{D}x{nt}", 4.0 * M * D * nt)
    return out


_gemm_split = True
GEMM_WS_BYTES = 256 * 384 * 256 * 4

# ... 65 lines not shown
        _dev(k2, torch.bfloat16, "k2"), _dev(v2, torch.bfloat16, "v2")
        L2, _, ldk2 = _rows(k2, "k2")
        _, _, ldv2 = _rows(v2, "v2")
    if scale is None:
        scale = head_dim ** -0.5
    st = _prof_begin()
    nq, l1, l2 = Nq // batch, L1 // batch, L2 // batch
    _check(lib().ce_attention_batched_bf16(_ptr(q), _ptr(k), _ptr(v), l1, ldk, ldv, _ptr(k2), _ptr(v2), l2, ldk2, ldv2, _ptr(out),
                                           nq, heads, head_dim, ldq, ldo, float(scale), batch, _stream()), "ce_attention_bf16")
    _prof_end(st, f"attention_{nq}x{l1}+{l2}_h{heads}" + (f"_b{batch}" if batch > 1 else ""),
              4.0 * nq * (l1 + l2) * head_dim * heads * batch)
    return out


def vt_columns(n_keys_total: int) -> int:
    return (n_keys_total + 63) // 64 * 64 + 64


def v_transpose(v: torch.Tensor, heads: int, out: Optional[torch.Tensor] = None):
    _dev(v, torch.bfloat16, "v")
    n, D, ldv = _rows(v, "v")
    assert D == heads * 128
    if out is None:
        out = torch.empty((D, vt_columns(n)), dtype=torch.bfloat16, device=v.device)
    _dev(out, torch.bfloat16, "vt")
    assert out.shape[0] == D and out.is_contiguous() and out.shape[1] >= n
    st = _prof_begin()
    _check(lib().ce_v_transpose_bf16(_ptr(v), ldv, _ptr(out), out.shape[1], n, heads, _stream()), "ce_v_transpose_bf16")
    _prof_end(st, f"v_transpose_{n}x{D}", 4.0 * n * D)
    return out


def attention_vt(q: torch.Tensor, k: torch.Tensor, vt: torch.Tensor, heads: int, out: Optional[torch.Tensor] = None,
                 scale: Optional[float] = None, batch: int = 1):
    for n, t in (("q", q), ("k", k), ("vt", vt)):
        _dev(t, torch.bfloat16, n)
    Nq, Dq, ldq = _rows(q, "q")
    L1, _, ldk = _rows(k, "k")
    assert Dq == heads * 128 and vt.shape[0] == Dq and vt.stride(1) == 1
    if batch < 1 or Nq % batch or L1 % batch:
        raise ValueError(f"attention_vt: row counts must be multiples of batch={batch}")
    if out is None:
        out = torch.empty((Nq, Dq), dtype=torch.bfloat16, device=q.device)
    _, _, ldo = _rows(out, "out")
    if scale is None:
        scale = 128 ** -0.5
    st = _prof_begin()
    nq, l1 = Nq // batch, L1 // batch
    _check(lib().ce_attention_vt_bf16(_ptr(q), _ptr(k), _ptr(vt), l1, ldk, vt.stride(0), _ptr(out), nq, heads, 128, ldq, ldo, float(scale),
                                      batch, _stream()), "ce_attention_vt_bf16")
    _prof_end(st, f"attention_{nq}x{l1}+0_h{heads}" + (f"_b{batch}" if batch > 1 else ""), 4.0 * nq * l1 * 128 * heads * batch)
    return out


def attention_2seg_vt(q: torch.Tensor, k1: torch.Tensor, v1t: torch.Tensor, len1: int, k2: torch.Tensor, v2t: torch.Tensor, len2: int,
                      heads: int, out: Optional[torch.Tensor] = None, scale: Optional[float] = None, batch: int = 1,
                      cols1: Optional[int] = None, cols2: Optional[int] = None, out8: Optional[torch.Tensor] = None,
                      scale8: Optional[torch.Tensor] = None):
    for n, t in (("q", q), ("k1", k1), ("v1t", v1t), ("k2", k2), ("v2t", v2t)):
        _dev(t, torch.bfloat16, n)
    Nq, Dq, ldq = _rows(q, "q")
    _, _, ldk1 = _rows(k1, "k1")
    _, _, ldk2 = _rows(k2, "k2")
    assert Dq == heads * 128 and v1t.shape[0] == Dq and v2t.shape[0] == Dq and v1t.stride(1) == 1 and v2t.stride(1) == 1
    assert Nq % batch == 0 and k1.shape[0] == batch * len1 and k2.shape[0] == batch * len2
    if cols1 is None:
        assert v1t.shape[1] % batch == 0
        cols1 = v1t.shape[1] // batch
    if cols2 is None:
        assert v2t.shape[1] % batch == 0
        cols2 = v2t.shape[1] // batch
    if scale is None:
        scale = 128 ** -0.5
    nq = Nq // batch
    if out8 is not None:
        _dev(out8, torch.uint8, "out8"), _dev(scale8, torch.uint8, "scale8")
        _, D8, ld8 = _rows(out8, "out8")
        assert out8.shape[0] == Nq and D8 == Dq and scale8.is_contiguous() and scale8.numel() >= mx_scale_bytes(Nq, Dq)
        st = _prof_begin()
        _check(lib().ce_attention_2seg_vt_quant_bf16(_ptr(q), _ptr(k1), _ptr(v1t), len1, ldk1, v1t.stride(0), int(cols1), _ptr(k2), _ptr(v2t),
                                                     len2, ldk2, v2t.stride(0), int(cols2), _ptr(out8), _ptr(scale8), nq, heads, 128, ldq, ld8,
                                                     float(scale), batch, _stream()), "ce_attention_2seg_vt_quant_bf16")
        _prof_end(st, f"attention_{nq}x{len1}+{len2}_h{heads}" + (f"_b{batch}" if batch > 1 else "") + "_mxq",
                  4.0 * nq * (len1 + len2) * 128 * heads * batch)
        return out8
    if out is None:
        out = torch.empty((Nq, Dq), dtype=torch.bfloat16, device=q.device)
    _, _, ldo = _rows(out, "out")
    st = _prof_begin()
    _check(lib().ce_attention_2seg_vt_bf16(_ptr(q), _ptr(k1), _ptr(v1t), len1, ldk1, v1t.stride(0), int(cols1), _ptr(k2), _ptr(v2t),
                                           len2, ldk2, v2t.stride(0), int(cols2), _ptr(out), nq, heads, 128, ldq, ldo,
                                           float(scale), batch, _stream()), "ce_attention_2seg_vt_bf16")
    _prof_end(st, f"attention_{nq}x{len1}+{len2}_h{heads}" + (f"_b{batch}" if batch > 1 else ""), 4.0 * nq * (len1 + len2) * 128 * heads * batch)
    return out


def v_transpose_blocked(v: torch.Tensor, heads: int, batch: int, blk_rows: int, n_keys: int, out: Optional[torch.Tensor] = None):
    _dev(v, torch.bfloat16, "v")
    rows, D, ldv = _rows(v, "v")
    assert D == heads * 128 and blk_rows % 64 == 0 and rows % (batch * blk_rows) == 0
    cols = (n_keys + 63) // 64 * 64 + 64
    if out is None:
        out = torch.empty((D, batch * cols), dtype=torch.bfloat16, device=v.device)
    assert out.shape == (D, batch * cols) and out.is_contiguous()
    st = _prof_begin()
    _check(lib().ce_v_transpose_blocked_bf16(_ptr(v), ldv, _ptr(out), out.shape[1], n_keys, heads, batch, blk_rows, batch * blk_rows, cols,
                                             _stream()), "ce_v_transpose_blocked_bf16")
    _prof_end(st, f"v_transpose_{batch * n_keys}x{D}", 4.0 * batch * n_keys * D)
    return out


def attention_vt_blocked(q: torch.Tensor, k: torch.Tensor, vt: torch.Tensor, heads: int, batch: int, blk_rows: int, n_keys: int,
                         out: Optional[torch.Tensor] = None, scale: Optional[float] = None):
    for n, t in (("q", q), ("k", k), ("vt", vt)):
        _dev(t, torch.bfloat16, n)
    rows, Dq, ldq = _rows(q, "q")
    rk, _, ldk = _rows(k, "k")
    assert Dq == heads * 128 and vt.shape[0] == Dq and vt.stride(1) == 1 and rows == rk and rows % (batch * blk_rows) == 0
    nq = rows // batch
    cols = vt.shape[1] // batch
    if out is None:
        out = torch.empty((rows, Dq), dtype=torch.bfloat16, device=q.device)
    _, _, ldo = _rows(out, "out")
    if scale is None:
        scale = 128 ** -0.5
# ... 564 lines not shown
```

### chronoedit_amd/transformer.py

```python
from __future__ import annotations

import inspect
import math
from dataclasses import dataclass
from types import SimpleNamespace
from typing import Any, Dict, Optional, Tuple, Union

import torch
import torch.nn as nn

from . import ops, weights
from .weights import LoraMixin


_VT_GEMM_SWAPPED = __import__("os").environ.get("CE_VT_GEMM") == "row"


@dataclass
class Transformer2DModelOutput:
    sample: torch.Tensor


class _Config(SimpleNamespace):
    def __getitem__(self, k):
        return getattr(self, k)

    def get(self, k, d=None):
        return getattr(self, k, d)


class RMSNormParams(nn.Module):

    def __init__(self, dim: int, eps: float, device=None, dtype=None):
        super().__init__()
        self.eps = eps
        self.weight = nn.Parameter(torch.ones(dim, device=device, dtype=dtype))


class AttentionParams(nn.Module):

    def __init__(self, dim: int, heads: int, eps: float, added_kv_proj_dim: Optional[int], device=None, dtype=None):
        super().__init__()
        kw = dict(device=device, dtype=dtype)
        self.heads = heads
        self.to_q = nn.Linear(dim, dim, **kw)
        self.to_k = nn.Linear(dim, dim, **kw)
        self.to_v = nn.Linear(dim, dim, **kw)
        self.to_out = nn.ModuleList([nn.Linear(dim, dim, **kw), nn.Dropout(0.0)])
# ... 104 lines not shown
        super().__init__()
        if qk_norm != "rms_norm_across_heads":
            raise NotImplementedError("only qk_norm='rms_norm_across_heads' (the ChronoEdit/Wan setting) is supported")
        if tuple(patch_size) != (1, 2, 2):
            raise NotImplementedError("patch_size must be (1, 2, 2)")
        if attention_head_dim != 128:
            raise NotImplementedError("the gfx950 attention kernel is specialised for head_dim 128")
        self.config = _Config(
            patch_size=tuple(patch_size), num_attention_heads=num_attention_heads, attention_head_dim=attention_head_dim,
            in_channels=in_channels, out_channels=out_channels or in_channels, text_dim=text_dim, freq_dim=freq_dim,
            ffn_dim=ffn_dim, num_layers=num_layers, cross_attn_norm=cross_attn_norm, qk_norm=qk_norm, eps=eps,
            image_dim=image_dim, added_kv_proj_dim=added_kv_proj_dim, rope_max_seq_len=rope_max_seq_len,
            rope_temporal_skip_len=rope_temporal_skip_len,
        )
        inner = num_attention_heads * attention_head_dim
        kw = dict(device=device, dtype=dtype)
        self.patch_embedding = nn.Conv3d(in_channels, inner, kernel_size=patch_size, stride=patch_size, **kw)
        self.condition_embedder = ConditionEmbedderParams(inner, freq_dim, inner * 6, text_dim, image_dim, **kw)
        self.blocks = nn.ModuleList(
            [BlockParams(inner, ffn_dim, num_attention_heads, cross_attn_norm, eps, added_kv_proj_dim, **kw) for _ in range(num_layers)]
        )
        self.proj_out = nn.Linear(inner, self.config.out_channels * math.prod(patch_size), **kw)
        self.scale_shift_table = nn.Parameter(torch.randn(1, 2, inner, device=device, dtype=torch.float32) / inner**0.5)
        self._engine: Optional["DiTEngine"] = None
        self._gen = next(_GENERATION)
        self.cache_context = False
        self.gemm_dtype = "bf16"
        self.fp8_linears = self.FP8_LINEARS
        self.attn_dtype = "bf16"
        self.v_transposed = True
        self.sp_batch_cfg = True
        self.fp8_fuse_quant = True
        self.fp8_fuse_attn_quant = True
        self.cross_vt = True
        self._sp = None
        self._cfgp = None

    @property
    def dtype(self) -> torch.dtype:
        return self.proj_out.weight.dtype

    @property
    def device(self) -> torch.device:
        return self.proj_out.weight.device

    @classmethod
    def from_pretrained(cls, path: str, subfolder: Optional[str] = None, torch_dtype: torch.dtype = torch.bfloat16,
                        device=None, **unused) -> "ChronoEditTransformer3DModel":
        cfg = weights.read_config(path, subfolder)
        known = set(inspect.signature(cls.__init__).parameters) - {"self", "device", "dtype"}
        model = cls(**{k: v for k, v in cfg.items() if k in known}, device=device, dtype=torch_dtype)
        sd = weights.load_state_dict_files(weights.shard_files(path, subfolder))
        weights.assign_state_dict(model, sd, ignore_unexpected=cls._keys_to_ignore_on_load_unexpected)
        model.invalidate()
        return model

    def load_wan_native_state_dict(self, sd: Dict[str, torch.Tensor]):
        renamed = weights.wan_native_to_diffusers(sd, [k for k, _ in self.named_parameters()])
        weights.assign_state_dict(self, renamed, ignore_unexpected=self._keys_to_ignore_on_load_unexpected)
        self.invalidate()
        return self

    def wan_native_state_dict(self) -> Dict[str, torch.Tensor]:
        return {weights.diffusers_to_wan_native_key(k): p.detach() for k, p in self.named_parameters()}

    def save_pretrained(self, path: str, max_shard_bytes: int = 5 << 30):
# ... 41 lines not shown
        if self.cache_context:
            self.engine()._context(encoder_hidden_states, encoder_hidden_states_image)

    def invalidate(self):
        self._engine = None

    FP8_LINEARS = ("qkv", "o1", "q2", "o2", "f1", "f2")
    FP8_POLICIES = {"fast": ("qkv", "o1", "q2", "o2", "f1", "f2"), "accurate": ("qkv", "o1", "q2", "f1", "f2")}

    def enable_fp8_gemms(self, on: bool = True, mx: bool = True, linears=None, policy: Optional[str] = None):
        if policy is not None:
            if linears is not None:
                raise ValueError("enable_fp8_gemms: give `linears` or `policy`, not both")
            if policy not in self.FP8_POLICIES:
                raise ValueError(f"enable_fp8_gemms: unknown policy {policy!r} (one of {sorted(self.FP8_POLICIES)})")
            linears = self.FP8_POLICIES[policy]
        linears = tuple(self.FP8_LINEARS if linears is None else linears)
        bad = [n for n in linears if n not in self.FP8_LINEARS]
        if bad:
            raise ValueError(f"enable_fp8_gemms: unknown Linear name(s) {bad} (of {self.FP8_LINEARS})")
        self.fp8_linears = tuple(n for n in self.FP8_LINEARS if n in linears)
        self.gemm_dtype = ("mxfp8" if mx else "fp8") if (on and self.fp8_linears) else "bf16"
        self._engine = None
        return self

    def enable_transposed_v(self, on: bool = True):
        self.v_transposed = bool(on)
        if self._engine is not None:
            self._engine.v_transposed = self.v_transposed
            self._engine._ws = {}
            self._engine.ws_generation += 1
        return self

    def enable_cross_vt(self, on: bool = True):
        self.cross_vt = bool(on)
        self._engine = None
        return self

    def enable_fp8_attention(self, on: bool = True, cross: bool = False):
        self.attn_dtype = "mxfp8" if on else "bf16"
        self.fp8_cross = bool(on and cross)
        self._engine = None
        return self

    def attention_path(self) -> str:
        sharded = self._sp is not None and self._sp.sharded
        return "mxfp8" if (self.attn_dtype == "mxfp8" and not sharded) else "bf16"

    def _apply(self, fn, *a, **kw):
        self._engine = None
        return super()._apply(fn, *a, **kw)

    def load_state_dict(self, *a, **kw):
        self._engine = None
        return super().load_state_dict(*a, **kw)

    def engine(self) -> "DiTEngine":
        if self._engine is None:
            self._engine = DiTEngine(self)
            self._gen = next(_GENERATION)
        return self._engine

    def engine_generation(self):
        eng = self._engine
        sp = self._sp
        return (self._gen, None if eng is None else eng.ws_generation, self.gemm_dtype, self.fp8_linears, self.attn_dtype, self.v_transposed, self.cross_vt,
                self.sp_batch_cfg, bool(getattr(self, "rope_plain_temporal", False)), self.cache_context,
                None if sp is None else (sp.world, sp.rank), self._cfgp is not None)

    @torch.no_grad()
    def forward(
        self,
        hidden_states: torch.Tensor,
        timestep: torch.LongTensor,
        encoder_hidden_states: torch.Tensor,
        encoder_hidden_states_image: Optional[torch.Tensor] = None,
        return_dict: bool = True,
        attention_kwargs: Optional[Dict[str, Any]] = None,
    ) -> Union[Transformer2DModelOutput, Tuple[torch.Tensor]]:
        if not hidden_states.is_cuda:
            raise ops.HipKernelError("ChronoEditTransformer3DModel (chronoedit_amd) runs only on an MI355X device: "
                                     "there is no CPU fallback (use oracle/ for CPU reference numbers)")
        B = hidden_states.shape[0]
        ts = timestep.reshape(-1)
        if ts.numel() == 1 and B > 1:
            ts = ts.expand(B)
        output = self.engine().forward(hidden_states, ts, encoder_hidden_states, encoder_hidden_states_image).to(hidden_states.dtype)
        if not return_dict:
            return (output,)
        return Transformer2DModelOutput(sample=output)


def rope_cos_sin(head_dim: int, max_len: int, skip_len: int, T: int, Hp: int, Wp: int, theta: float = 10000.0,
                 plain_temporal: bool = False) -> torch.Tensor:
    assert plain_temporal or T == 2 or T == skip_len, f"num_frames must be 2 or {skip_len}, but got {T}"
    h_dim = w_dim = 2 * (head_dim // 6)
    t_dim = head_dim - h_dim - w_dim

    def ang(dim, idx):
        f = 1.0 / (theta ** (torch.arange(0, dim, 2, dtype=torch.float64)[: dim // 2] / dim))
# ... 71 lines not shown
            self.im_n2 = (f32(ie.norm2.weight), f32(ie.norm2.bias), ie.norm2.eps)

        self.blk = []
        tables = []
        for blk in model.blocks:
            p = SimpleNamespace()
            a1, a2 = blk.attn1, blk.attn2
            p.w_qkv = self._fuse([a1.to_q, a1.to_k, a1.to_v])
            p.b_qkv = torch.cat([f32(a1.to_q.bias), f32(a1.to_k.bias), f32(a1.to_v.bias)])
            p.nq1, p.nk1 = f32(a1.norm_q.weight), f32(a1.norm_k.weight)
            p.w_o1, p.b_o1 = a1.to_out[0].weight.detach().contiguous(), f32(a1.to_out[0].bias)
            p.w_q2, p.b_q2 = a2.to_q.weight.detach().contiguous(), f32(a2.to_q.bias)
            p.nq2, p.nk2 = f32(a2.norm_q.weight), f32(a2.norm_k.weight)
            p.has_img = a2.add_k_proj is not None
            if p.has_img:
                p.nk_i = f32(a2.norm_added_k.weight)
            p.w_o2, p.b_o2 = a2.to_out[0].weight.detach().contiguous(), f32(a2.to_out[0].bias)
            if cfg.cross_attn_norm:
                p.n2w, p.n2b = f32(blk.norm2.weight), f32(blk.norm2.bias)
            else:
                p.n2w = p.n2b = None
            p.w_f1, p.b_f1 = blk.ffn.net[0].proj.weight.detach().contiguous(), f32(blk.ffn.net[0].proj.bias)
            p.w_f2, p.b_f2 = blk.ffn.net[2].weight.detach().contiguous(), f32(blk.ffn.net[2].bias)
            tables.append(f32(blk.scale_shift_table).reshape(6, self.D))
            self.blk.append(p)
        self.fp8_attn = model.attn_dtype == "mxfp8"
        self.fp8_cross = self.fp8_attn and bool(getattr(model, "fp8_cross", False))
        self.fp8 = model.gemm_dtype in ("fp8", "mxfp8")
        self.mx = model.gemm_dtype == "mxfp8"
        self.fp8_set = frozenset(getattr(model, "fp8_linears", model.FP8_LINEARS)) if self.fp8 else frozenset()
        self.fuse_quant = bool(getattr(model, "fp8_fuse_quant", True)) and self.F % 128 == 0
        self.fuse_attn_quant = self.fuse_quant and bool(getattr(model, "fp8_fuse_attn_quant", True))
        self.v_transposed = bool(getattr(model, "v_transposed", True))
        if self.fp8:
            if self.D % 256 or self.F % 256:
                raise NotImplementedError("fp8 GEMMs need inner and ffn dims that are multiples of 256")
            for p in self.blk:
                for name in sorted(self.fp8_set):
                    w = getattr(p, "w_" + name)
                    setattr(p, "q_" + name, ops.quant_rows_mxfp8(w, w_order=True) if self.mx else ops.quant_rows_fp8(w))
        self.w_k_t_all = self._fuse([blk.attn2.to_k for blk in model.blocks])
        self.b_k_t_all = torch.cat([f32(blk.attn2.to_k.bias) for blk in model.blocks])
        self.w_v_t_all = self._fuse([blk.attn2.to_v for blk in model.blocks])
        self.b_v_t_all = torch.cat([f32(blk.attn2.to_v.bias) for blk in model.blocks])
        self.all_img = all(p.has_img for p in self.blk)
        if self.all_img:
            self.w_k_i_all = self._fuse([blk.attn2.add_k_proj for blk in model.blocks])
            self.b_k_i_all = torch.cat([f32(blk.attn2.add_k_proj.bias) for blk in model.blocks])
            self.w_v_i_all = self._fuse([blk.attn2.add_v_proj for blk in model.blocks])
            self.b_v_i_all = torch.cat([f32(blk.attn2.add_v_proj.bias) for blk in model.blocks])
        self.cross_vt = bool(getattr(model, "cross_vt", True))
        self._ctx_bufs = {}
        self.tables = torch.stack(tables, 0).contiguous()
        self.table_out = f32(model.scale_shift_table).reshape(1, 2, self.D)
        self.w_out, self.b_out = _pad_n(model.proj_out.weight.detach().contiguous(), f32(model.proj_out.bias))
        self.ones = torch.ones(self.D, dtype=torch.float32, device=dev)
        self.zeros = torch.zeros(self.D, dtype=torch.float32, device=dev)
        self._rope = {}
        self._ws = {}
        self.ws_generation = 0
        self._ctx_key = None
        self._ctx = None
        self._ctx_refs = None

    def _fuse(self, linears) -> torch.Tensor:
        w = torch.cat([l.weight.detach() for l in linears], dim=0).contiguous()
        o = 0
        for l in linears:
            n = l.weight.shape[0]
            l.weight.data = w[o : o + n]
            o += n
        return w

    def _ln_linear(self, ws, x: torch.Tensor, a_row, b_row, p, name: str, out: torch.Tensor, ab_rows: int = 0, ab_stride: int = 0, **kw):
        eps = self.cfg.eps
        if name not in self.fp8_set:
            ops.ln_affine(x, a_row, b_row, eps, out=ws.h, ab_rows=ab_rows, ab_stride=ab_stride)
            return ops.gemm(ws.h, getattr(p, "w_" + name), getattr(p, "b_" + name), out=out, **kw)
        aq = ws.a8[:, : x.shape[1]]
        wq, sw = getattr(p, "q_" + name)
        if self.mx:
            ops.ln_affine_mxfp8(x, a_row, b_row, eps, out=aq, scale=ws.s8, ab_rows=ab_rows, ab_stride=ab_stride)
            return ops.gemm_mxfp8(aq, ws.s8, wq, sw, getattr(p, "b_" + name), out=out, **kw)
# ... 27 lines not shown
            if self.mx:
                ops.ln_affine_mxfp8(x, a_row, b_row, eps, out=aq, scale=ws.s8, ab_rows=Nl, ab_stride=6 * D)
                sblk = (D // 128) * 512
                lin = lambda lo, hi, out: ops.gemm_mxfp8(aq, ws.s8, wq[lo:hi], sw[lo // 128 * sblk: hi // 128 * sblk], p.b_qkv[lo:hi], out=out)
            else:
                ops.ln_affine_fp8(x, a_row, b_row, eps, out=aq, scale=ws.s8, ab_rows=Nl, ab_stride=6 * D)
                lin = lambda lo, hi, out: ops.gemm_fp8(aq, ws.s8, wq[lo:hi], sw[lo:hi], p.b_qkv[lo:hi], out=out)
        lin(D, 3 * D, ws.qkv[:, D:])
        ops.rope_scatter(ws.qkv, (D, 2 * D), (p.nk1, None), D, W, cs, hd, eps, out=ws.send_kv)
        _, wait_kv = sp.all_to_all(ws.send_kv, ws.recv_kv, async_op=True)
        lin(0, D, ws.qkv[:, :D])
        ops.rope_scatter(ws.qkv, (0,), (p.nq1,), D, W, cs, hd, eps, out=ws.send_q)
        _, wait_q = sp.all_to_all(ws.send_q, ws.recv_q, async_op=True)
        wait_kv.wait()
        wait_q.wait()
        kv = sp.gathered_view(ws.recv_kv)
        if B > 1:
            vt_shape = (Dl, B * ops.vt_columns(N))
            ws.vt_sp = ops.v_transpose_blocked(kv[:, Dl:], H // W, B, Nl, N, out=ws.vt_sp if getattr(ws, "vt_sp", torch.empty(0)).shape == vt_shape else None)
            ops.attention_vt_blocked(sp.gathered_view(ws.recv_q), kv[:, :Dl], ws.vt_sp, H // W, B, Nl, N, out=ws.att_g)
        elif self.v_transposed:
            if getattr(ws, "vt_sp", None) is None or ws.vt_sp.shape != (Dl, ops.vt_columns(N)):
                ws.vt_sp = torch.zeros((Dl, ops.vt_columns(N)), dtype=torch.bfloat16, device=self.dev)
            ops.v_transpose(kv[:N, Dl:], H // W, out=ws.vt_sp)
            ops.attention_vt(sp.gathered_view(ws.recv_q), kv[:N, :Dl], ws.vt_sp, H // W, out=ws.att_g)
        else:
            ops.attention(sp.gathered_view(ws.recv_q), kv[:N, :Dl], kv[:N, Dl:], H // W, out=ws.att_g)
        y, _ = sp.all_to_all(ws.att_g.view(W, B * Nl, Dl), ws.att_seg)
        if "o1" in self.fp8_set:
            ws.att.copy_(sp.merge_heads_reference(y))
            return ws.att
        return y

    def _workspace(self, N: int):
        ws = self._ws.get(N)
        if ws is None:
            D, F, dev = self.D, self.F, self.dev
            e = lambda *s: torch.empty(s, dtype=torch.bfloat16, device=dev)
            ws = SimpleNamespace(x=e(N, D), h=e(N, D), qkv=e(N, 3 * D), att=e(N, D), q2=e(N, D), ffn=e(N, F),
                                 cols=e(N, self.kpatch), head=e(N, self.w_out.shape[0]))
            if self.fp8:
                ws.a8 = torch.empty((N, max(D, F)), dtype=torch.uint8, device=dev)
                ws.s8 = (torch.empty((ops.mx_scale_bytes(N, max(D, F)),), dtype=torch.uint8, device=dev) if self.mx else
                         torch.empty((N,), dtype=torch.float32, device=dev))
                if self.mx and self.fuse_quant and F % 128 == 0:
                    ws.a8b = torch.empty((N, F), dtype=torch.uint8, device=dev)
                    ws.s8b = torch.empty((ops.mx_scale_bytes(N, F),), dtype=torch.uint8, device=dev)
            if self.fp8_attn:
                u8 = lambda *s: torch.empty(s, dtype=torch.uint8, device=dev)
                ws.q8, ws.k8, ws.sq, ws.sk = u8(N, D), u8(N, D), u8(N, D // 32), u8(N, D // 32)
                ws.v8t = ws.sv = None
            sp = self.model._sp
            if sp is not None and sp.sharded:
                W, Dl = sp.world, D // sp.world
                ws.send_kv, ws.recv_kv = e(W, N, 2, Dl), e(W, N, 2, Dl)
                ws.send_q, ws.recv_q = e(W, N, 1, Dl), e(W, N, 1, Dl)
                ws.att_g, ws.att_seg = e(W * N, Dl), e(W, N, Dl)
            if len(self._ws) > 1:
                self.ws_generation += 1
            keep = list(self._ws.items())[-1:]
            self._ws = dict(keep + [(N, ws)])
        return ws

    def _rope_table(self, T, Hp, Wp):
        plain = bool(getattr(self.model, "rope_plain_temporal", False))
        key = (T, Hp, Wp, plain)
        if key not in self._rope:
            c = self.cfg
            if len(self._rope) >= 4:
                self._rope.pop(next(iter(self._rope)))
            self._rope[key] = rope_cos_sin(c.attention_head_dim, c.rope_max_seq_len, c.rope_temporal_skip_len, T, Hp, Wp,
                                           plain_temporal=plain).to(self.dev)
        return self._rope[key]
# ... 42 lines not shown
            w, b, eps = self.im_n2
            enc_i = ops.ln_affine(h_img, w, b, eps)
        eps = self.cfg.eps
        hd = self.cfg.attention_head_dim
        L = self.L
        f8 = self.fp8_cross and (self.model._sp is None or not self.model._sp.sharded) and getattr(self.model, "_cfgp", None) is None
        use_vt = self.cross_vt and enc_i is not None and self.all_img and Tt % 8 == 0 and not f8
        k_t_all = ops.gemm(enc_t, self.w_k_t_all, self.b_k_t_all)
        k_i_all = v_t_all = v_i_all = v1t = v2t = None
        c1 = c2 = 0
        if enc_i is not None and self.all_img:
            k_i_all = ops.gemm(enc_i, self.w_k_i_all, self.b_k_i_all)
        if use_vt:
            c1, c2 = Tt, (Ti + 7) // 8 * 8
            ld1 = ((B - 1) * c1 + (Tt + 63) // 64 * 64 + 7) // 8 * 8
            ld2 = ((B - 1) * c2 + (Ti + 63) // 64 * 64 + 7) // 8 * 8
            bufs = self._ctx_bufs.get((B, Tt, Ti))
            if bufs is None:
                z = lambda *sh: torch.zeros(sh, dtype=torch.bfloat16, device=self.dev)
                bufs = SimpleNamespace(enc_i_pad=z(B * c2, D), v1t=z(L * D, ld1), v2t=z(L * D, ld2))
                self._ctx_bufs = dict(list(self._ctx_bufs.items())[-1:] + [((B, Tt, Ti), bufs)])
            v1t, v2t = bufs.v1t, bufs.v2t
            self._ctx_key = self._ctx = self._ctx_refs = None
            w, b, eps_i = self.im_n2
            for bi in range(B):
                ops.ln_affine(h_img[bi * Ti:(bi + 1) * Ti], w, b, eps_i, out=bufs.enc_i_pad[bi * c2: bi * c2 + Ti])
            ops.gemm(self.w_v_t_all, enc_t, self.b_v_t_all, out=v1t[:, : B * Tt], epilogue=ops.EPI_BIAS_ROW)
            ops.gemm(self.w_v_i_all, bufs.enc_i_pad, self.b_v_i_all, out=v2t[:, : B * c2], epilogue=ops.EPI_BIAS_ROW)
        else:
            v_t_all = ops.gemm(enc_t, self.w_v_t_all, self.b_v_t_all)
            if k_i_all is not None:
                v_i_all = ops.gemm(enc_i, self.w_v_i_all, self.b_v_i_all)
        kv = []
        for li, p in enumerate(self.blk if not f8 else ()):
            cols = slice(li * D, (li + 1) * D)
            k_t = k_t_all[:, cols]
            ops.rmsnorm_rope_(k_t, p.nk2, None, hd, eps)
            k_i = None
            if k_i_all is not None:
                k_i = k_i_all[:, cols]
                ops.rmsnorm_rope_(k_i, p.nk_i, None, hd, eps)
            if use_vt:
                kv.append((k_t, v1t[cols], k_i, v2t[cols]))
            else:
                kv.append((k_t, v_t_all[:, cols], k_i, None if v_i_all is None else v_i_all[:, cols]))
        if f8:
            for li, p in enumerate(self.blk):
                cols = slice(li * D, (li + 1) * D)
                seg_t = ops.rmsnorm_rope_mxfp8(k_t_all[:, cols], p.nk2, None, hd, eps) + ops.v_mxfp8_transpose(v_t_all[:, cols], Tt, B, self.H)
                seg_i = None
                if k_i_all is not None:
                    seg_i = ops.rmsnorm_rope_mxfp8(k_i_all[:, cols], p.nk_i, None, hd, eps) + ops.v_mxfp8_transpose(v_i_all[:, cols], Ti, B, self.H)
                kv.append((seg_t, seg_i))
        ctx = SimpleNamespace(kv=kv, Tt=Tt, Ti=Ti, vt=use_vt, c1=c1, c2=c2, f8=f8)
        if key is not None:
            self._ctx_key, self._ctx, self._ctx_refs = key, ctx, keyed
        return ctx

    def clear_context_cache(self):
        self._ctx_key = self._ctx = self._ctx_refs = None

    def forward(self, hidden: torch.Tensor, timestep: torch.Tensor, text: torch.Tensor, image: Optional[torch.Tensor]):
        cfg, D, H = self.cfg, self.D, self.H
        B, C, T, Hh, Ww = hidden.shape
        if C != cfg.in_channels:
            raise ValueError(f"expected {cfg.in_channels} input channels, got {C}")
        Hp, Wp = Hh // 2, Ww // 2
        N = T * Hp * Wp
        hd = cfg.attention_head_dim
        eps = cfg.eps
        cs = self._rope_table(T, Hp, Wp)
        sp = self.model._sp
        if sp is not None and sp.sharded:
            if B != 1 and not self.v_transposed:
# ... 37 lines not shown
        mod_out = torch.stack(mods_out, dim=0).contiguous()
        if B > 1:
            gate_msa = mod[:, :, 2].contiguous()
            gate_ffn = mod[:, :, 5].contiguous()

        if text.shape[0] != B or (image is not None and image.shape[0] != B):
            raise ValueError("encoder_hidden_states / encoder_hidden_states_image batch size must match hidden_states")
        ctx = self._context(text, image)
        Tt, Ti = ctx.Tt, ctx.Ti
        grow = Nl if B > 1 else 0

        x = ws.x
        fuse_o = self.mx and self.fuse_attn_quant and D % 128 == 0
        fuse_o1, fuse_o2 = fuse_o and "o1" in self.fp8_set, fuse_o and "o2" in self.fp8_set
        for li, p in enumerate(self.blk):
            q_o1 = False
            if sp is None and self.fp8_attn:
                self._ln_linear(ws, x, mod[li, 0, 1], mod[li, 0, 0], p, "qkv", ws.qkv, ab_rows=Nl, ab_stride=6 * D)
                ops.rmsnorm_rope_mxfp8(ws.qkv[:, :D], p.nq1, cs, hd, eps, out=ws.q8, scale=ws.sq, post_scale=ops.MXFP8_Q_SCALE)
                ops.rmsnorm_rope_mxfp8(ws.qkv[:, D : 2 * D], p.nk1, cs, hd, eps, out=ws.k8, scale=ws.sk)
                if ws.v8t is None or ws.v8t.shape[0] != B:
                    ws.v8t = ws.sv = None
                ws.v8t, ws.sv = ops.v_mxfp8_transpose(ws.qkv[:, 2 * D :], Nl, B, H, out=ws.v8t, scale=ws.sv)
                if fuse_o1:
                    ops.attention_mxfp8(ws.q8, ws.sq, ws.k8, ws.sk, ws.v8t, ws.sv, H, batch=B, out8=ws.a8[:, :D], scale8=ws.s8)
                    q_o1 = True
                else:
                    ops.attention_mxfp8(ws.q8, ws.sq, ws.k8, ws.sk, ws.v8t, ws.sv, H, out=ws.att, batch=B)
                att = ws.att
            elif sp is None and self.v_transposed and "qkv" not in self.fp8_set and (B * Nl) % 8 == 0 and (B == 1 or Nl % 2 == 0):
                if getattr(ws, "vt", None) is None:
                    ws.vt = torch.zeros((D, ops.vt_columns(B * Nl)), dtype=torch.bfloat16, device=self.dev)
                ops.ln_affine(x, mod[li, 0, 1], mod[li, 0, 0], eps, out=ws.h, ab_rows=Nl, ab_stride=6 * D)
                ops.gemm(ws.h, p.w_qkv[: 2 * D], p.b_qkv[: 2 * D], out=ws.qkv[:, : 2 * D])
                if _VT_GEMM_SWAPPED:
                    ops.gemm(p.w_qkv[2 * D :], ws.h, p.b_qkv[2 * D :], out=ws.vt[:, : B * Nl], epilogue=ops.EPI_BIAS_ROW)
                else:
                    ops.gemm(ws.h, p.w_qkv[2 * D :], p.b_qkv[2 * D :], out=ws.vt[:, : B * Nl], epilogue=ops.EPI_BIAS_T)
                ops.rmsnorm_rope_(ws.qkv[:, :D], p.nq1, cs, hd, eps, x2=ws.qkv[:, D : 2 * D], w2=p.nk1)
                ops.attention_vt(ws.qkv[:, :D], ws.qkv[:, D : 2 * D], ws.vt, H, out=ws.att, batch=B)
                att = ws.att
            elif sp is None:
                self._ln_linear(ws, x, mod[li, 0, 1], mod[li, 0, 0], p, "qkv", ws.qkv, ab_rows=Nl, ab_stride=6 * D)
                ops.rmsnorm_rope_(ws.qkv[:, :D], p.nq1, cs, hd, eps, x2=ws.qkv[:, D : 2 * D], w2=p.nk1)
                ops.attention(ws.qkv[:, :D], ws.qkv[:, D : 2 * D], ws.qkv[:, 2 * D :], H, out=ws.att, batch=B)
                att = ws.att
            else:
                att = self._self_attention_ulysses(ws, sp, x, mod[li, 0, 1], mod[li, 0, 0], p, cs, N, Nl, B)
            self._linear(ws, att, p, "o1", x, quantised=q_o1, epilogue=ops.EPI_GATE_RES, gate=gate_msa[li] if B > 1 else mods[0][li, 2],
                         res=x, gate_rows=grow)
            if p.n2w is not None:
                self._ln_linear(ws, x, p.n2w, p.n2b, p, "q2", ws.q2)
            else:
                self._linear(ws, x, p, "q2", ws.q2)
            q_o2 = bool(ctx.vt and fuse_o2)
            if ctx.f8:
                seg_t, seg_i = ctx.kv[li]
                ops.rmsnorm_rope_mxfp8(ws.q2, p.nq2, None, hd, eps, out=ws.q8, scale=ws.sq, post_scale=ops.MXFP8_Q_SCALE)
                if seg_i is None and fuse_o2:
                    ops.attention_mxfp8(ws.q8, ws.sq, *seg_t, H, batch=B, out8=ws.a8[:, :D], scale8=ws.s8)
                else:
                    ops.attention_mxfp8(ws.q8, ws.sq, *seg_t, H, out=ws.att, batch=B)
                    if seg_i is not None and fuse_o2:
                        ops.attention_mxfp8(ws.q8, ws.sq, *seg_i, H, batch=B, out8=ws.a8[:, :D], scale8=ws.s8, add=ws.att)
                    elif seg_i is not None:
                        ops.attention_mxfp8(ws.q8, ws.sq, *seg_i, H, out=ws.att, batch=B, add=ws.att)
                q_o2 = fuse_o2
                self._linear(ws, ws.att, p, "o2", x, quantised=q_o2, epilogue=ops.EPI_GATE_RES, gate=None, res=x)
                k_t = None
            else:
                ops.rmsnorm_rope_(ws.q2, p.nq2, None, hd, eps)
                k_t, v_t, k_i, v_i = ctx.kv[li]
            if k_t is None:
                pass
            elif ctx.vt and fuse_o2:
                ops.attention_2seg_vt(ws.q2, k_t, v_t, Tt, k_i, v_i, Ti, H, batch=B, cols1=ctx.c1, cols2=ctx.c2, out8=ws.a8[:, :D], scale8=ws.s8)
            elif ctx.vt:
                ops.attention_2seg_vt(ws.q2, k_t, v_t, Tt, k_i, v_i, Ti, H, out=ws.att, batch=B, cols1=ctx.c1, cols2=ctx.c2)
            elif k_i is not None:
                ops.attention(ws.q2, k_t, v_t, H, out=ws.att, k2=k_i, v2=v_i, batch=B)
            else:
                ops.attention(ws.q2, k_t, v_t, H, out=ws.att, batch=B)
            if k_t is not None:
                self._linear(ws, ws.att, p, "o2", x, quantised=q_o2, epilogue=ops.EPI_GATE_RES, gate=None, res=x)
            if self.mx and self.fuse_quant and "f1" in self.fp8_set and "f2" in self.fp8_set:
                aq = ws.a8[:, :D]
                ops.ln_affine_mxfp8(x, mod[li, 0, 4], mod[li, 0, 3], eps, out=aq, scale=ws.s8, ab_rows=Nl, ab_stride=6 * D)
                ops.gemm_mxfp8_gelu_quant(aq, ws.s8, *p.q_f1, p.b_f1, out=ws.a8b, scale=ws.s8b)
                ops.gemm_mxfp8(ws.a8b, ws.s8b, *p.q_f2, p.b_f2, out=x, epilogue=ops.EPI_GATE_RES,
                               gate=gate_ffn[li] if B > 1 else mods[0][li, 5], res=x, gate_rows=grow)
            else:
                self._ln_linear(ws, x, mod[li, 0, 4], mod[li, 0, 3], p, "f1", ws.ffn, ab_rows=Nl, ab_stride=6 * D, epilogue=ops.EPI_BIAS_GELU)
                self._linear(ws, ws.ffn, p, "f2", x, epilogue=ops.EPI_GATE_RES, gate=gate_ffn[li] if B > 1 else mods[0][li, 5],
                             res=x, gate_rows=grow)

        ops.ln_affine(x, mod_out[0, 0, 1], mod_out[0, 0, 0], eps, out=ws.h, ab_rows=Nl, ab_stride=2 * D)
        ops.gemm(ws.h, self.w_out, self.b_out, out=ws.head)
        out = torch.empty((B, cfg.out_channels, T, Hh, Ww), dtype=torch.bfloat16, device=self.dev)
        if sp is None:
            for b in range(B):
                ops.unpatchify(ws.head[rows[b]], cfg.out_channels, T, Hh, Ww, out=out[b])
        else:
            full = sp.all_gather_rows(ws.head).view(sp.world, B, Nl, -1)
            for b in range(B):
                ops.unpatchify(full[:, b].reshape(sp.world * Nl, -1)[:N].contiguous(), cfg.out_channels, T, Hh, Ww, out=out[b])
        return out
```

### include/chronoedit_hip.h

```cpp
#ifndef CHRONOEDIT_HIP_H
#define CHRONOEDIT_HIP_H

#include <stddef.h>
#include <stdint.h>

#ifdef __cplusplus
extern "C" {
#endif

#ifndef __HIP_PLATFORM_AMD__
typedef struct ihipStream_t* hipStream_t;
#endif

#define CE_OK 0
#define CE_ERR_ARG (-1)
#define CE_ERR_SHAPE (-2)
#define CE_ERR_ALIGN (-3)

#define CE_EPI_BIAS 0
#define CE_EPI_BIAS_GELU 1
#define CE_EPI_GATE_RES 2
#define CE_EPI_BIAS_GELU_ERF 3
#define CE_EPI_BIAS_ROW 6
#define CE_EPI_BIAS_T 7
#define CE_EPI_F32 4

int ce_ln_affine_bf16(const void* x, void* y, const float* a, const float* b, int M, int D, int ldx, int ldy, float eps,
                      int ab_rows, int ab_stride, hipStream_t stream);

int ce_rmsnorm_rope_bf16(void* x, const float* w, void* x2, const float* w2, const float* cos_sin, int M, int D, int ld,
                         int head_dim, float eps, int rope_rows, hipStream_t stream);

int ce_gemm_bf16(const void* A, const void* W, void* C, const float* bias, int epilogue, const float* gate, const void* res,
                 int M, int N, int K, int lda, int ldw, int ldc, int ldres, int gate_rows, int a_seg_k, long long a_seg_stride,
                 int w_seg_k, long long w_seg_stride, void* ws, size_t ws_bytes, hipStream_t stream);



int ce_gemm_bf16_tile_rows(int M, int N, int K, int cus, long long ws_bytes);

int ce_attention_bf16(const void* Q, const void* K1, const void* V1, int len1, int ldk1, int ldv1, const void* K2,
                      const void* V2, int len2, int ldk2, int ldv2, void* O, int Nq, int H, int head_dim, int ldq, int ldo,
                      float softmax_scale, hipStream_t stream);

int ce_attention_batched_bf16(const void* Q, const void* K1, const void* V1, int len1, int ldk1, int ldv1, const void* K2,
                              const void* V2, int len2, int ldk2, int ldv2, void* O, int Nq, int H, int head_dim, int ldq,
                              int ldo, float softmax_scale, int batch, hipStream_t stream);

int ce_attention_vt_bf16(const void* Q, const void* K, const void* Vt, int len, int ldk, int ldvt, void* O, int Nq, int H, int head_dim,
                         int ldq, int ldo, float softmax_scale, int batch, hipStream_t stream);

int ce_attention_2seg_vt_bf16(const void* Q, const void* K1, const void* V1t, int len1, int ldk1, int ldv1t, int vt_cols1, const void* K2,
                              const void* V2t, int len2, int ldk2, int ldv2t, int vt_cols2, void* O, int Nq, int H, int head_dim, int ldq,
                              int ldo, float softmax_scale, int batch, hipStream_t stream);

int ce_attention_2seg_vt_quant_bf16(const void* Q, const void* K1, const void* V1t, int len1, int ldk1, int ldv1t, int vt_cols1, const void* K2,
                                    const void* V2t, int len2, int ldk2, int ldv2t, int vt_cols2, void* o8, void* scale8, int Nq, int H,
                                    int head_dim, int ldq, int ldo8, float softmax_scale, int batch, hipStream_t stream);

int ce_attention_vt_blocked_bf16(const void* Q, const void* K, const void* Vt, int len, int ldk, int ldvt, void* O, int Nq, int H, int head_dim,
                                 int ldq, int ldo, float softmax_scale, int batch, int blk_rows, int blk_stride, int vt_sample_cols,
                                 hipStream_t stream);

int ce_v_transpose_blocked_bf16(const void* v, int ldv, void* vt, int ldvt, int n_keys, int H, int batch, int blk_rows, int blk_stride,
                                int vt_sample_cols, hipStream_t stream);

int ce_v_transpose_bf16(const void* v, int ldv, void* vt, int ldvt, int n_keys, int H, hipStream_t stream);


int ce_timestep_sinusoid(const int64_t* t, float* out, int dim, hipStream_t stream);

int ce_timestep_sinusoid_f32(const float* t, float* out, int dim, hipStream_t stream);

int ce_gemv(const void* W, int w_is_bf16, const float* x, const float* bias, float* y, int N, int K, int flags,
            hipStream_t stream);

int ce_modulation(const float* table, const float* v, float* mod, int L, int J, int D, int v_rows, int one_mask,
                  hipStream_t stream);

int ce_patchify_bf16(const void* x, void* cols, int C, int T, int H, int W, int Kpad, hipStream_t stream);

int ce_patchify_rows_bf16(const void* x, void* cols, int C, int T, int H, int W, int Kpad, int row0, int nrows, hipStream_t stream);

int ce_rope_scatter_bf16(const void* x, int ldx, void* send, int M, int D, int W, int nt, int col0, const float* w0, int col1,
                         const float* w1, int col2, const float* w2, const float* cos_sin, int head_dim, float eps,
                         int rope_rows, hipStream_t stream);

// ... 109 lines not shown
```

### include/chronoedit_hip_diag.h

```cpp
#ifndef CHRONOEDIT_HIP_DIAG_H
#define CHRONOEDIT_HIP_DIAG_H

#include "chronoedit_hip.h"

#ifdef __cplusplus
extern "C" {
#endif

int ce_set_gemm_variant(int variant);

int ce_set_attention_waves(int nwave);

int ce_set_gemm_fp8_variant(int variant);

int ce_set_attention_mxfp8_variant(int variant);

int ce_set_attention_mxfp8_persistent(int n);

int ce_diag_attention_exact_route_hits(unsigned long long* hits, int reset);

#ifdef __cplusplus
}
#endif
#endif
```

Baseline: 3.050.

## Fuse query RMSNorm and RoPE into GEMM epilogue and attention prologue

The QKV and Q2 GEMM epilogues now write per-row, per-head-slab sums of squares into a small fp32 buffer. The attention kernel gains a RAWQ variant that reads the raw Q, reduces those partial sums, and applies the RMSNorm weight and RoPE in its prologue. This removes the separate read-modify-write rmsnorm_rope pass over Q. Cross-attention key norms across all layers are also batched into one rmsnorm_layers launch. In exchange the GEMM epilogue does extra reductions, the attention prologue does more loads and math, and rounding order differs slightly from the standalone norm.

```diff
diff --git a/chronoedit_amd/csrc/ce_attn.hip b/chronoedit_amd/csrc/ce_attn.hip
--- a/chronoedit_amd/csrc/ce_attn.hip
+++ b/chronoedit_amd/csrc/ce_attn.hip
@@ -38,6 +38,16 @@
   int ld8;
 };
 
+struct QNorm {
+  const float* ssq;
+  const float* w;
+  const float* cs;
+  int ssq_ld;
+  int rope_rows;
+  float eps;
+  bf16* qdump;
+};
+
 template <bool TWO_SEG, int NWAVE>
 __global__ __launch_bounds__(NWAVE * 64, NWAVE == 8 ? 2 : 2) void attn_fwd_kernel(const bf16* __restrict__ Q, bf16* __restrict__ O, KVSeg seg0,
                                                        KVSeg seg1, int Nq, int H, int ldq, int ldo, int nqb,
@@ -279,10 +289,10 @@
 constexpr int SP_TILE_BYTES = 2 * PK_TILE + 3 * PV_TILE;
 constexpr int sp_smem_bytes(bool two_seg) { return two_seg ? SP_TILE_BYTES + 8 * QW * OST_ROW : SP_TILE_BYTES; }
 
-template <bool TWO_SEG, bool VT = false, bool QOUT = false>
+template <bool TWO_SEG, bool VT = false, bool QOUT = false, bool RAWQ = false>
 __global__ __launch_bounds__(512, 2) void attn_fwd_sp_kernel(const bf16* __restrict__ Q_, bf16* __restrict__ O_, KVSeg seg0_,
                                                               KVSeg seg1_, int Nq, int H, int ldq, int ldo, int nqb,
-                                                              float scale_log2e, int batch, BlkRows blk) {
+                                                              float scale_log2e, int batch, BlkRows blk, QNorm qn) {
   extern __shared__ __attribute__((aligned(16))) unsigned char smem[];
   constexpr int NWAVE = 8, QB = QW * NWAVE;
   const int tid = threadIdx.x, lane = tid & 63;
@@ -345,7 +355,63 @@
 #pragma unroll
     for (int ks = 0; ks < 8; ++ks) qf[ks] = *reinterpret_cast<const bf16x8*>(qrow + 16 * ks);
   }
+  const int q_grow = bz * Nq + (q0 + l31 < Nq ? q0 + l31 : 0);
+  f32x4 q_p4[10];
+  if constexpr (RAWQ) {
+    const float* pp = qn.ssq + (size_t)q_grow * qn.ssq_ld;
+#pragma unroll
+    for (int j = 0; j < 10; ++j) q_p4[j] = *reinterpret_cast<const f32x4*>(pp + min(4 * j, H - 4));
+  }
   auto scale_q = [&]() __attribute__((always_inline)) {
+  if constexpr (RAWQ) {
+    float ss = 0.f;
+#pragma unroll
+    for (int j = 0; j < 10; ++j)
+      if (4 * j < H) ss = ((((ss + q_p4[j][0]) + q_p4[j][1]) + q_p4[j][2]) + q_p4[j][3]);
+    const float q_rstd = 1.0f / sqrtf(ss / (float)(H * HD) + qn.eps);
+    constexpr bool ROPE = !TWO_SEG;
+    const int cs_row = qn.rope_rows > 0 ? q_grow % qn.rope_rows : q_grow;
+    const float* wp = qn.w + hoff + 8 * hh;
+    const float* cp = qn.cs != nullptr ? qn.cs + ((size_t)cs_row * (HD / 2) + 4 * hh) * 2 : nullptr;
+#pragma unroll
+    for (int half = 0; half < 2; ++half) {
+      f32x4 w0[4], w1[4], cs0[4], cs1[4];
+#pragma unroll
+      for (int k4 = 0; k4 < 4; ++k4) {
+        const int ks = 4 * half + k4;
+        w0[k4] = *reinterpret_cast<const f32x4*>(wp + 16 * ks);
+        w1[k4] = *reinterpret_cast<const f32x4*>(wp + 16 * ks + 4);
+        cs0[k4] = cs1[k4] = f32x4{1.f, 0.f, 1.f, 0.f};
+        if (ROPE && qn.cs != nullptr) {
+          cs0[k4] = *reinterpret_cast<const f32x4*>(cp + 16 * ks);
+          cs1[k4] = *reinterpret_cast<const f32x4*>(cp + 16 * ks + 4);
+        }
+      }
+#pragma unroll
+      for (int k4 = 0; k4 < 4; ++k4) {
+        const int ks = 4 * half + k4;
+        const u32x4 raw = __builtin_bit_cast(u32x4, qf[ks]);
+        u32x4 o;
+#pragma unroll
+        for (int j = 0; j < 4; ++j) {
+          const float ww0 = j < 2 ? w0[k4][2 * j] : w1[k4][2 * j - 4], ww1 = j < 2 ? w0[k4][2 * j + 1] : w1[k4][2 * j - 3];
+          float v0 = round_bf16(round_bf16(bf16lo(raw[j]) * q_rstd) * ww0);
+          float v1 = round_bf16(round_bf16(bf16hi(raw[j]) * q_rstd) * ww1);
+          if (ROPE) {
+            const float co = j < 2 ? cs0[k4][2 * j] : cs1[k4][2 * j - 4], si = j < 2 ? cs0[k4][2 * j + 1] : cs1[k4][2 * j - 3];
+            const float r0 = v0 * co - v1 * si, r1 = v0 * si + v1 * co;
+            v0 = r0;
+            v1 = r1;
+          }
+          o[j] = pack_bf16(v0, v1);
+        }
+        qf[ks] = __builtin_bit_cast(bf16x8, o);
+#ifdef CE_DIAGNOSTICS
+        if (qn.qdump != nullptr && q0 + l31 < Nq) *reinterpret_cast<u32x4*>(qn.qdump + (size_t)q_grow * ldq + hoff + 16 * ks + 8 * hh) = o;
+#endif
+      }
+    }
+  }
 #pragma unroll
   for (int ks = 0; ks < 8; ++ks) {
     const u32x4 w = __builtin_bit_cast(u32x4, qf[ks]);
@@ -1274,7 +1340,7 @@
       done = true;                                                                                                   \
     }                                                                                                                \
     hipLaunchKernelGGL((attn_fwd_sp_kernel<TWO>), dim3(nqb * H * batch), block, sp_smem_bytes(TWO), stream, (const bf16*)Q, \
-                       (bf16*)O, s0, s1, Nq, H, ldq, ldo, nqb, sl2, batch, BlkRows{0, 0, 0u, 0});                    \
+                       (bf16*)O, s0, s1, Nq, H, ldq, ldo, nqb, sl2, batch, BlkRows{0, 0, 0u, 0}, QNorm{});           \
   } while (0)
     if (two) CE_ATTN_SP(true); else CE_ATTN_SP(false);
 #undef CE_ATTN_SP
@@ -1335,8 +1401,10 @@
 
 static int attention_vt_launch(const void* Q, const void* K, const void* Vt, int len, int ldk, int ldvt, void* O, int Nq, int H, int head_dim,
                                int ldq, int ldo, float softmax_scale, int batch, int blk_rows, int blk_stride, int vt_sample_cols,
-                               hipStream_t stream) {
+                               hipStream_t stream, const QNorm* qn = nullptr) {
   if (!Q || !K || !Vt || !O) return CE_ERR_ARG;
+  if (qn && (!qn->ssq || !qn->w || blk_rows != 0)) return CE_ERR_ARG;
+  if (qn && ((H & 3) || H > 40 || (qn->ssq_ld & 3) || qn->ssq_ld < H)) return CE_ERR_SHAPE;
   if (head_dim != HD || Nq <= 0 || H <= 0 || len <= 0 || batch <= 0 || batch > 65535) return CE_ERR_SHAPE;
   const int ntiles_cols = (len + KVB - 1) / KVB * KVB;
   if (blk_rows == 0) {
@@ -1365,6 +1433,18 @@
   }
   const int cus = ce_device_cus();
   const int items = nqb * H * batch;
+  if (qn) {
+    static bool doneq_[CE_MAX_DEVICES] = {};
+    bool& doneq = doneq_[ce_device_slot()];
+    if (!doneq) {
+      (void)hipFuncSetAttribute((const void*)attn_fwd_sp_kernel<false, true, false, true>, hipFuncAttributeMaxDynamicSharedMemorySize, sp_smem_bytes(false));
+      doneq = true;
+    }
+    const int grid_q = items <= 2 * cus ? items : ((2 * cus) & ~7);
+    hipLaunchKernelGGL((attn_fwd_sp_kernel<false, true, false, true>), dim3(grid_q), dim3(512), sp_smem_bytes(false), stream, (const bf16*)Q, (bf16*)O,
+                       s0, s1, Nq, H, ldq, ldo, nqb, sl2, batch, blk, *qn);
+    return (int)hipGetLastError();
+  }
 #ifdef CE_DIAGNOSTICS
   if (g_attn_nwave == 16 && blk_rows == 0) {
     const int rc = ce_attn16_launch(Q, K, Vt, len, ldk, ldvt, O, Nq, H, ldq, ldo, sl2, batch, cus, stream);
@@ -1385,8 +1465,26 @@
   }
   const int grid_vt = items <= 2 * cus ? items : ((2 * cus) & ~7);
   hipLaunchKernelGGL((attn_fwd_sp_kernel<false, true>), dim3(grid_vt), dim3(512), sp_smem_bytes(false), stream, (const bf16*)Q, (bf16*)O,
-                     s0, s1, Nq, H, ldq, ldo, nqb, sl2, batch, blk);
+                     s0, s1, Nq, H, ldq, ldo, nqb, sl2, batch, blk, QNorm{});
   return (int)hipGetLastError();
+}
+
+#ifdef CE_DIAGNOSTICS
+static void* g_rawq_dump = nullptr;
+CE_API int ce_diag_attention_rawq_dump(void* q_out) {
+  g_rawq_dump = q_out;
+  return CE_OK;
+}
+#define CE_RAWQ_DUMP ((bf16*)g_rawq_dump)
+#else
+#define CE_RAWQ_DUMP nullptr
+#endif
+
+CE_API int ce_attention_vt_rawq_bf16(const void* Q, const void* K, const void* Vt, int len, int ldk, int ldvt, void* O, int Nq, int H,
+                                     int head_dim, int ldq, int ldo, float softmax_scale, int batch, const float* ssq, int ssq_ld,
+                                     const float* nw, const float* cs, int rope_rows, float eps, hipStream_t stream) {
+  const QNorm qn{ssq, nw, cs, ssq_ld, rope_rows, eps, CE_RAWQ_DUMP};
+  return attention_vt_launch(Q, K, Vt, len, ldk, ldvt, O, Nq, H, head_dim, ldq, ldo, softmax_scale, batch, 0, 0, 0, stream, &qn);
 }
 
 CE_API int ce_attention_vt_bf16(const void* Q, const void* K, const void* Vt, int len, int ldk, int ldvt, void* O, int Nq, int H,
@@ -1406,8 +1504,10 @@
 static int attention_2seg_vt_launch(const void* Q, const void* K1, const void* V1t, int len1, int ldk1, int ldv1t, int vt_cols1,
                                     const void* K2, const void* V2t, int len2, int ldk2, int ldv2t, int vt_cols2, void* O, int Nq,
                                     int H, int head_dim, int ldq, int ldo, float softmax_scale, int batch, void* O8, void* S8, int ldo8,
-                                    hipStream_t stream) {
+                                    hipStream_t stream, const QNorm* qn = nullptr) {
   if (!Q || !K1 || !V1t || !K2 || !V2t || (!O && !O8)) return CE_ERR_ARG;
+  if (qn && (!qn->ssq || !qn->w || O8)) return CE_ERR_ARG;
+  if (qn && ((H & 3) || H > 40 || (qn->ssq_ld & 3) || qn->ssq_ld < H)) return CE_ERR_SHAPE;
   if (head_dim != HD || Nq <= 0 || H <= 0 || len1 <= 0 || len2 <= 0 || batch <= 0 || batch > 65535) return CE_ERR_SHAPE;
   const int c1 = (len1 + KVB - 1) / KVB * KVB, c2 = (len2 + KVB - 1) / KVB * KVB;
   if (vt_cols1 < len1 || vt_cols2 < len2 || ldv1t < (batch - 1) * vt_cols1 + c1 || ldv2t < (batch - 1) * vt_cols2 + c2) return CE_ERR_SHAPE;
@@ -1421,19 +1521,33 @@
   if (!done) {
     (void)hipFuncSetAttribute((const void*)attn_fwd_sp_kernel<true, true>, hipFuncAttributeMaxDynamicSharedMemorySize, sp_smem_bytes(true));
     (void)hipFuncSetAttribute((const void*)attn_fwd_sp_kernel<true, true, true>, hipFuncAttributeMaxDynamicSharedMemorySize, sp_smem_bytes(true));
+    (void)hipFuncSetAttribute((const void*)attn_fwd_sp_kernel<true, true, false, true>, hipFuncAttributeMaxDynamicSharedMemorySize, sp_smem_bytes(true));
     done = true;
   }
   const BlkRows blk{0, vt_cols2, 0u, vt_cols1, (unsigned char*)O8, (unsigned char*)S8, ldo8};
   const int cus = ce_device_cus();
   const int items = nqb * H * batch;
   const int grid = items <= 2 * cus ? items : ((2 * cus) & ~7);
-  if (O8)
+  if (qn)
+    hipLaunchKernelGGL((attn_fwd_sp_kernel<true, true, false, true>), dim3(grid), dim3(512), sp_smem_bytes(true), stream, (const bf16*)Q, (bf16*)O,
+                       s0, s1, Nq, H, ldq, ldo, nqb, sl2, batch, blk, *qn);
+  else if (O8)
     hipLaunchKernelGGL((attn_fwd_sp_kernel<true, true, true>), dim3(grid), dim3(512), sp_smem_bytes(true), stream, (const bf16*)Q,
-                       (bf16*)O, s0, s1, Nq, H, ldq, ldo, nqb, sl2, batch, blk);
+                       (bf16*)O, s0, s1, Nq, H, ldq, ldo, nqb, sl2, batch, blk, QNorm{});
   else
     hipLaunchKernelGGL((attn_fwd_sp_kernel<true, true>), dim3(grid), dim3(512), sp_smem_bytes(true), stream, (const bf16*)Q, (bf16*)O,
-                       s0, s1, Nq, H, ldq, ldo, nqb, sl2, batch, blk);
+                       s0, s1, Nq, H, ldq, ldo, nqb, sl2, batch, blk, QNorm{});
   return (int)hipGetLastError();
+}
+
+CE_API int ce_attention_2seg_vt_rawq_bf16(const void* Q, const void* K1, const void* V1t, int len1, int ldk1, int ldv1t, int vt_cols1,
+                                          const void* K2, const void* V2t, int len2, int ldk2, int ldv2t, int vt_cols2, void* O, int Nq,
+                                          int H, int head_dim, int ldq, int ldo, float softmax_scale, int batch, const float* ssq, int ssq_ld,
+                                          const float* nw, float eps, hipStream_t stream) {
+  if (!O) return CE_ERR_ARG;
+  const QNorm qn{ssq, nw, nullptr, ssq_ld, 0, eps, CE_RAWQ_DUMP};
+  return attention_2seg_vt_launch(Q, K1, V1t, len1, ldk1, ldv1t, vt_cols1, K2, V2t, len2, ldk2, ldv2t, vt_cols2, O, Nq, H, head_dim, ldq, ldo,
+                                  softmax_scale, batch, nullptr, nullptr, 0, stream, &qn);
 }
 
 CE_API int ce_attention_2seg_vt_bf16(const void* Q, const void* K1, const void* V1t, int len1, int ldk1, int ldv1t, int vt_cols1,
diff --git a/chronoedit_amd/csrc/ce_common.h b/chronoedit_amd/csrc/ce_common.h
--- a/chronoedit_amd/csrc/ce_common.h
+++ b/chronoedit_amd/csrc/ce_common.h
@@ -54,6 +54,13 @@
     if (kt % (2 * s) == 0 && tail * s * slab_bytes <= ws_bytes) return s;
   return 1;
 }
+
+struct RowSsq {
+  float* out;
+  int ld;
+  int col0;
+  int col1;
+};
 
 inline uint32_t ce_seg_magic(int seg_k, int bk, int kt) {
   if (seg_k <= 0 || seg_k % bk) return 0;
diff --git a/chronoedit_amd/csrc/ce_gemm.hip b/chronoedit_amd/csrc/ce_gemm.hip
--- a/chronoedit_amd/csrc/ce_gemm.hip
+++ b/chronoedit_amd/csrc/ce_gemm.hip
@@ -9,6 +9,7 @@
 #define EPI_F32 4
 #define EPI_BIAS_ROW 6
 #define EPI_BIAS_T 7
+#define EPI_BIAS_SSQ 8
 #define EPI_MUL 5
 
 namespace {
@@ -332,6 +333,24 @@
   return (int)hipGetLastError();
 }
 
+extern "C" int ce_gemm384_ssq_launch(int rows, const void* A, const void* W, void* C, const float* bias, int M, int N, int K, int lda, int ldw, int ldc,
+                                     float* ws, size_t ws_bytes, RowSsq ssq, hipStream_t stream);
+extern "C" int ce_gemm256w4_ssq_launch(const void* A, const void* W, void* C, const float* bias, int M, int N, int K, int lda, int ldw, int ldc,
+                                       float* ws, size_t ws_bytes, RowSsq ssq, hipStream_t stream);
+
+CE_API int ce_gemm_bf16_rowssq(const void* A, const void* W, void* C, const float* bias, int M, int N, int K, int lda, int ldw, int ldc,
+                               float* ssq, int ssq_ld, int ssq_col0, int ssq_col1, void* ws, size_t ws_bytes, hipStream_t stream) {
+  if (!A || !W || !C || !ssq) return CE_ERR_ARG;
+  if (M <= 0 || N <= 0 || K <= 0 || (K % BK) || (N & 7)) return CE_ERR_SHAPE;
+  if ((lda & 7) || (ldw & 7) || (ldc & 7)) return CE_ERR_ALIGN;
+  if ((long long)M * N < 256ll * 256 * 128 || !ce_gemm256_supported(M, N, K, lda, ldw)) return CE_ERR_SHAPE;
+  const RowSsq q{ssq, ssq_ld, ssq_col0, ssq_col1};
+  const int rows = ce_gemm_bf16_tile_rows(M, N, K, ce_device_cus(), ws ? (long long)ws_bytes : 0);
+  if (rows == 384 || rows == 288)
+    return ce_gemm384_ssq_launch(rows, A, W, C, bias, M, N, K, lda, ldw, ldc, static_cast<float*>(ws), ws_bytes, q, stream);
+  return ce_gemm256w4_ssq_launch(A, W, C, bias, M, N, K, lda, ldw, ldc, static_cast<float*>(ws), ws_bytes, q, stream);
+}
+
 CE_API int ce_gemm_batched_bf16(const void* A, const void* W, void* C, const float* bias, int epilogue, int M, int N, int K,
                                     int lda, int ldw, int ldc, int batch0, int batch1, long long sA0, long long sA1, long long sW0,
                                     long long sW1, long long sC0, long long sC1, hipStream_t stream) {
diff --git a/chronoedit_amd/csrc/ce_gemm256w4.hip b/chronoedit_amd/csrc/ce_gemm256w4.hip
--- a/chronoedit_amd/csrc/ce_gemm256w4.hip
+++ b/chronoedit_amd/csrc/ce_gemm256w4.hip
@@ -43,7 +43,7 @@
     const bf16* __restrict__ A, const bf16* __restrict__ W, bf16* __restrict__ C, const float* __restrict__ bias,
     const float* __restrict__ gate, const bf16* __restrict__ res, int M, int N, int K, int lda, int ldw, int ldc, int ldres,
     int gate_rows, int tiles_m, int tiles_n, int t_full, int split, float* __restrict__ ws, uint32_t a_seg_magic,
-    uint32_t a_seg_extra, uint32_t w_seg_magic, uint32_t w_seg_extra, uint32_t a_seg2_magic, uint32_t a_seg2_extra) {
+    uint32_t a_seg_extra, uint32_t w_seg_magic, uint32_t w_seg_extra, uint32_t a_seg2_magic, uint32_t a_seg2_extra, RowSsq ssq) {
   extern __shared__ __attribute__((aligned(16))) unsigned char smem[];
   constexpr int BN = 32 * NG;
   constexpr bool REGEPI = NG == 8;
@@ -224,6 +224,8 @@
     for (int h = 0; h < 2; ++h)
       bvv[h] = (EPI != EPI_BIAS_ROW && bias != nullptr) ? *reinterpret_cast<const f32x4*>(bias + colc + 4 * h) : f32x4{0.f, 0.f, 0.f, 0.f};
     const auto c_rsrc = __builtin_amdgcn_make_buffer_rsrc((void*)C, 0, (uint32_t)(M - 1) * (uint32_t)(ldc * 2) + (uint32_t)N * 2u, 0x00020000);
+    const int slab_col = n0 + wn * 128;
+    const bool ssq_on = EPI == EPI_BIAS && ssq.out != nullptr && slab_col >= ssq.col0 && slab_col + 128 <= ssq.col1;
     f32x4 gA[2], gB[2];
     int g_switch = 0x7fffffff;
     u32x4 rv[8][4];
@@ -285,6 +287,10 @@
         }
         const uint32_t coff = (m < M && col_ok) ? (uint32_t)m * (uint32_t)(ldc * 2) + (uint32_t)col0 * 2u : 0xffffffffu;
         __builtin_amdgcn_raw_buffer_store_b128(o, c_rsrc, coff, 0, 0);
+        if (EPI == EPI_BIAS && ssq_on) {
+          const float s = row16_sum(row_ssq8(y));
+          if (fr == 0 && m < M) ssq.out[(size_t)m * ssq.ld + ((slab_col - ssq.col0) >> 7)] = s;
+        }
       }
     }
     return;
@@ -448,8 +454,14 @@
 static int w4_launch(const void* A, const void* W, void* C, const float* bias, int epilogue, const float* gate, const void* res, int M, int N,
                      int K, int lda, int ldw, int ldc, int ldres, int gate_rows, int a_seg_k, long long a_seg_stride, int w_seg_k,
                      long long w_seg_stride, int a_seg2_k, long long a_seg2_stride, int nsa, int ng, float* ws, size_t ws_bytes,
-                     hipStream_t stream) {
+                     hipStream_t stream, RowSsq ssq = RowSsq{nullptr, 0, 0, 0}) {
   const bool seg2 = a_seg2_k > 0;
+  const bool want_ssq = epilogue == EPI_BIAS_SSQ;
+  if (want_ssq) {
+    if (!ssq.out || (ssq.col0 & 127) || (ssq.col1 & 127) || ssq.col0 < 0 || ssq.col1 > N || ssq.col1 <= ssq.col0 || ssq.ld < ((ssq.col1 - ssq.col0) >> 7)) return CE_ERR_ARG;
+    if (seg2 || ng != 8 || nsa != 2 || (long long)M * ldc * 2 >= (1ll << 32)) return CE_ERR_SHAPE;
+    epilogue = EPI_BIAS;
+  }
   if ((ng != 8 && ng != 4 && ng != 3) || (ng != 8 && !seg2)) return CE_ERR_ARG;
   if (seg2 && (a_seg_k <= 0 || a_seg2_k % a_seg_k || (epilogue != EPI_BIAS && epilogue != EPI_GATE_RES) || nsa != 2 ||
                (epilogue == EPI_GATE_RES && gate != nullptr)))
@@ -486,6 +498,7 @@
   const int cus = ce_device_cus();
   int tail = nwg % cus;
   const int split = seg2 ? 1 : ce_split_k(tail, kt, cus, BM * BN * sizeof(float), ws ? (long long)ws_bytes : 0);
+  if (want_ssq && split != 1) return CE_ERR_SHAPE;
   if (split == 1) tail = 0;
   const int t_full2 = nwg - tail;
   dim3 grid(t_full2 + tail * split), block(256);
@@ -508,7 +521,7 @@
 #define CE_LAUNCH_SEG2(E, NGV, LDS)                                                                                                     \
   hipLaunchKernelGGL((gemm_bf16_w4<E, 2, false, true, NGV>), grid, block, LDS, stream, (const bf16*)A, (const bf16*)W, (bf16*)C, bias, gate, \
                      (const bf16*)res, M, N, K, lda, ldw, ldc, ldres, gate_rows, tiles_m, tiles_n, t_full2, split, ws, a_seg_magic,   \
-                     a_seg_extra, w_seg_magic, w_seg_extra, a_seg2_magic, a_seg2_extra)
+                     a_seg_extra, w_seg_magic, w_seg_extra, a_seg2_magic, a_seg2_extra, ssq)
     if (epilogue == EPI_BIAS) {
       if (ng == 8) CE_LAUNCH_SEG2(EPI_BIAS, 8, lds2); else if (ng == 4) CE_LAUNCH_SEG2(EPI_BIAS, 4, lds2n); else CE_LAUNCH_SEG2(EPI_BIAS, 3, lds2m);
     } else {
@@ -531,15 +544,15 @@
     if (nsa == 1)                                                                                                          \
       hipLaunchKernelGGL((gemm_bf16_w4<E, 3, true>), grid, block, lds3, stream, (const bf16*)A, (const bf16*)W, (bf16*)C, bias, gate, \
                          (const bf16*)res, M, N, K, lda, ldw, ldc, ldres, gate_rows, tiles_m, tiles_n, t_full2, split, ws, \
-                         a_seg_magic, a_seg_extra, w_seg_magic, w_seg_extra, 0u, 0u);                                      \
+                         a_seg_magic, a_seg_extra, w_seg_magic, w_seg_extra, 0u, 0u, ssq);                                 \
     else if (nsa == 3)                                                                                                     \
       hipLaunchKernelGGL((gemm_bf16_w4<E, 3, false>), grid, block, lds3, stream, (const bf16*)A, (const bf16*)W, (bf16*)C, bias, gate, \
                          (const bf16*)res, M, N, K, lda, ldw, ldc, ldres, gate_rows, tiles_m, tiles_n, t_full2, split, ws, \
-                         a_seg_magic, a_seg_extra, w_seg_magic, w_seg_extra, 0u, 0u);                                      \
+                         a_seg_magic, a_seg_extra, w_seg_magic, w_seg_extra, 0u, 0u, ssq);                                 \
     else                                                                                                                   \
       hipLaunchKernelGGL((gemm_bf16_w4<E, 2, false>), grid, block, lds2, stream, (const bf16*)A, (const bf16*)W, (bf16*)C, bias, gate, \
                          (const bf16*)res, M, N, K, lda, ldw, ldc, ldres, gate_rows, tiles_m, tiles_n, t_full2, split, ws, \
-                         a_seg_magic, a_seg_extra, w_seg_magic, w_seg_extra, 0u, 0u);                                      \
+                         a_seg_magic, a_seg_extra, w_seg_magic, w_seg_extra, 0u, 0u, ssq);                                 \
     if (tail)                                                                                                              \
       hipLaunchKernelGGL((gemm256w4_reduce<E>), dim3(4 * tail), block, 128 * QROW, stream, (bf16*)C, bias, gate,           \
                          (const bf16*)res, M, N, ldc, ldres, gate_rows, tiles_m, tiles_n, t_full2, split, ws);           \
@@ -554,6 +567,11 @@
   }
 #undef CE_LAUNCH
   return (int)hipGetLastError();
+}
+
+extern "C" int ce_gemm256w4_ssq_launch(const void* A, const void* W, void* C, const float* bias, int M, int N, int K, int lda, int ldw, int ldc,
+                                       float* ws, size_t ws_bytes, RowSsq ssq, hipStream_t stream) {
+  return w4_launch(A, W, C, bias, EPI_BIAS_SSQ, nullptr, nullptr, M, N, K, lda, ldw, ldc, 0, 0, 0, 0, 0, 0, 0, 0, 2, 8, ws, ws_bytes, stream, ssq);
 }
 
 extern "C" int ce_gemm256w4_launch(const void* A, const void* W, void* C, const float* bias, int epilogue, const float* gate,
diff --git a/chronoedit_amd/csrc/ce_gemm384.hip b/chronoedit_amd/csrc/ce_gemm384.hip
--- a/chronoedit_amd/csrc/ce_gemm384.hip
+++ b/chronoedit_amd/csrc/ce_gemm384.hip
@@ -44,7 +44,7 @@
     const bf16* __restrict__ A, const bf16* __restrict__ W, bf16* __restrict__ C, const float* __restrict__ bias,
     const float* __restrict__ gate, const bf16* __restrict__ res, int M, int N, int K, int lda, int ldw, int ldc, int ldres,
     int gate_rows, int tiles_m, int tiles_n, int t_full, int split, float* __restrict__ ws, uint32_t a_seg_magic,
-    uint32_t a_seg_extra, uint32_t w_seg_magic, uint32_t w_seg_extra) {
+    uint32_t a_seg_extra, uint32_t w_seg_magic, uint32_t w_seg_extra, RowSsq ssq) {
   constexpr int BM = T384<NF>::BM, A_TILE = T384<NF>::A_TILE, STAGE = T384<NF>::STAGE, NG = T384<NF>::NG, NP = T384<NF>::NP;
   static_assert(NF >= 9 && NF <= 12, "the W fragments of the second k-step are read in groups 1..8 of the first; rows 8.. of the accumulator live in 128 VGPRs");
   extern __shared__ __attribute__((aligned(16))) unsigned char smem[];
@@ -288,6 +288,8 @@
     return;
   }
   const auto c_rsrc = __builtin_amdgcn_make_buffer_rsrc((void*)C, 0, (uint32_t)(M - 1) * (uint32_t)(ldc * 2) + (uint32_t)N * 2u, 0x00020000);
+  const int slab_col = n0 + wn * 128;
+  const bool ssq_on = EPI == EPI_BIAS && ssq.out != nullptr && slab_col >= ssq.col0 && slab_col + 128 <= ssq.col1;
   f32x4 gA[2], gB[2];
   int g_switch = 0x7fffffff;
   constexpr int RA = 2;
@@ -352,6 +354,10 @@
       }
       const uint32_t coff = (m < M && col_ok) ? (uint32_t)m * (uint32_t)(ldc * 2) + (uint32_t)col0 * 2u : 0xffffffffu;
       __builtin_amdgcn_raw_buffer_store_b128(o, c_rsrc, coff, 0, 0);
+      if (EPI == EPI_BIAS && ssq_on) {
+        const float s = row16_sum(row_ssq8(y));
+        if (fr == 0 && m < M) ssq.out[(size_t)m * ssq.ld + ((slab_col - ssq.col0) >> 7)] = s;
+      }
     }
   }
 }
@@ -404,8 +410,14 @@
 template <int NF>
 static int gemm384_launch_impl(const void* A, const void* W, void* C, const float* bias, int epilogue, const float* gate, const void* res, int M, int N,
                                int K, int lda, int ldw, int ldc, int ldres, int gate_rows, int a_seg_k, long long a_seg_stride, int w_seg_k,
-                               long long w_seg_stride, float* ws, size_t ws_bytes, hipStream_t stream) {
+                               long long w_seg_stride, float* ws, size_t ws_bytes, hipStream_t stream, RowSsq ssq = RowSsq{nullptr, 0, 0, 0}) {
   constexpr int BM = T384<NF>::BM, STAGE = T384<NF>::STAGE;
+  const bool want_ssq = epilogue == EPI_BIAS_SSQ;
+  if (want_ssq) {
+    if (!ssq.out || (ssq.col0 & 127) || (ssq.col1 & 127) || ssq.col0 < 0 || ssq.col1 > N || ssq.col1 <= ssq.col0 || ssq.ld < ((ssq.col1 - ssq.col0) >> 7)) return CE_ERR_ARG;
+    if ((long long)M * ldc * 2 >= (1ll << 32)) return CE_ERR_SHAPE;
+    epilogue = EPI_BIAS;
+  } else
   if (epilogue == EPI_BIAS_T) {
     if ((M & 7) || (long long)N * ldc * 2 >= (1ll << 32) || !bias) return CE_ERR_SHAPE;
   } else
@@ -429,6 +441,7 @@
   const int cus = ce_device_cus();
   int tail = nwg % cus;
   const int split = epilogue == EPI_BIAS_T ? 1 : ce_split_k(tail, kt, cus, BM * BN * sizeof(float), ws ? (long long)ws_bytes : 0);
+  if (want_ssq && split != 1) return CE_ERR_SHAPE;
   if (split == 1) tail = 0;
   const int t_full2 = nwg - tail;
   dim3 grid(t_full2 + tail * split), block(256);
@@ -444,7 +457,7 @@
     }                                                                                                                      \
     hipLaunchKernelGGL((gemm_bf16_384<E, NF>), grid, block, lds, stream, (const bf16*)A, (const bf16*)W, (bf16*)C, bias, gate, \
                        (const bf16*)res, M, N, K, lda, ldw, ldc, ldres, gate_rows, tiles_m, tiles_n, t_full2, split, ws, \
-                       a_seg_magic, a_seg_extra, w_seg_magic, w_seg_extra);                                                \
+                       a_seg_magic, a_seg_extra, w_seg_magic, w_seg_extra, ssq);                                           \
     if (tail)                                                                                                              \
       hipLaunchKernelGGL((gemm384_reduce<E, NF>), dim3(4 * tail), block, 16 * NF * QROW, stream, (bf16*)C, bias, gate,     \
                          (const bf16*)res, M, N, ldc, ldres, gate_rows, tiles_m, tiles_n, t_full2, split, ws);           \
@@ -464,7 +477,7 @@
       }
       hipLaunchKernelGGL((gemm_bf16_384<EPI_BIAS_T, NF>), grid, block, lds, stream, (const bf16*)A, (const bf16*)W, (bf16*)C, bias, gate, (const bf16*)res,
                          M, N, K, lda, ldw, ldc, ldres, gate_rows, tiles_m, tiles_n, t_full2, split, ws, a_seg_magic, a_seg_extra, w_seg_magic,
-                         w_seg_extra);
+                         w_seg_extra, ssq);
       break;
     }
     default: return CE_ERR_ARG;
@@ -481,6 +494,13 @@
                                  w_seg_stride, ws, ws_bytes, stream);
 }
 
+extern "C" int ce_gemm384_ssq_launch(int rows, const void* A, const void* W, void* C, const float* bias, int M, int N, int K, int lda, int ldw, int ldc,
+                                     float* ws, size_t ws_bytes, RowSsq ssq, hipStream_t stream) {
+  if (rows == 384)
+    return gemm384_launch_impl<12>(A, W, C, bias, EPI_BIAS_SSQ, nullptr, nullptr, M, N, K, lda, ldw, ldc, 0, 0, 0, 0, 0, 0, ws, ws_bytes, stream, ssq);
+  return gemm384_launch_impl<9>(A, W, C, bias, EPI_BIAS_SSQ, nullptr, nullptr, M, N, K, lda, ldw, ldc, 0, 0, 0, 0, 0, 0, ws, ws_bytes, stream, ssq);
+}
+
 extern "C" int ce_gemm288_launch(const void* A, const void* W, void* C, const float* bias, int epilogue, const float* gate,
                                  const void* res, int M, int N, int K, int lda, int ldw, int ldc, int ldres, int gate_rows,
                                  int a_seg_k, long long a_seg_stride, int w_seg_k, long long w_seg_stride, float* ws, size_t ws_bytes,
diff --git a/chronoedit_amd/csrc/ce_gemm_epi.h b/chronoedit_amd/csrc/ce_gemm_epi.h
--- a/chronoedit_amd/csrc/ce_gemm_epi.h
+++ b/chronoedit_amd/csrc/ce_gemm_epi.h
@@ -14,7 +14,33 @@
 #define EPI_BIAS_T 7
 #endif
 
+#ifndef EPI_BIAS_SSQ
+#define EPI_BIAS_SSQ 8
+#endif
+
 namespace {
+
+__device__ __forceinline__ float row_ssq8(const u32x4& y) {
+  float s = 0.f;
+#pragma unroll
+  for (int q = 0; q < 4; ++q) {
+    const float lo = bf16lo(y[q]), hi = bf16hi(y[q]);
+    s = __builtin_fmaf(lo, lo, s);
+    s = __builtin_fmaf(hi, hi, s);
+  }
+  return s;
+}
+template <int CTRL>
+__device__ __forceinline__ float dpp_add(float v) {
+  return v + __builtin_bit_cast(float, __builtin_amdgcn_update_dpp(0, __builtin_bit_cast(int, v), CTRL, 0xf, 0xf, true));
+}
+__device__ __forceinline__ float row16_sum(float v) {
+  v = dpp_add<0xB1>(v);
+  v = dpp_add<0x4E>(v);
+  v = dpp_add<0x141>(v);
+  v = dpp_add<0x140>(v);
+  return v;
+}
 
 template <int EPI, int NCH, bool HAS_GATE, typename RowCol>
 __device__ __forceinline__ void epi_chunks_impl(const unsigned char* smem, int row_bytes, RowCol rowcol, int m0, int n0,
diff --git a/chronoedit_amd/csrc/ce_rowops.hip b/chronoedit_amd/csrc/ce_rowops.hip
--- a/chronoedit_amd/csrc/ce_rowops.hip
+++ b/chronoedit_amd/csrc/ce_rowops.hip
@@ -135,18 +135,9 @@
 }
 
 template <bool FULL>
-__global__ __launch_bounds__(256) void rmsnorm_rope_kernel(bf16* __restrict__ x0, const float* __restrict__ w0,
-                                                           bf16* __restrict__ x1, const float* __restrict__ w1,
-                                                           const float* __restrict__ cs, int M, int D, int ld,
-                                                           int head_dim, float eps, int rope_rows) {
-  const int lane = threadIdx.x & 63;
-  const int row = blockIdx.x * 4 + (threadIdx.x >> 6);
-  if (row >= M) return;
-  bf16* __restrict__ x = blockIdx.y ? x1 : x0;
-  const float* __restrict__ w = blockIdx.y ? w1 : w0;
-  const int cs_row = rope_rows > 0 ? row % rope_rows : row;
+__device__ __forceinline__ void rmsnorm_rope_row(bf16* __restrict__ xr, const float* __restrict__ w, const float* __restrict__ cs, int cs_row,
+                                                 int D, int head_dim, float eps, int lane) {
   const int nch = D >> 3;
-  bf16* xr = x + (size_t)row * ld;
   u32x4 raw[ROW_MAXC];
   float s = 0.f;
 #pragma unroll
@@ -199,6 +190,30 @@
       *reinterpret_cast<u32x4*>(xr + c * 8) = o;
     }
   }
+}
+
+template <bool FULL>
+__global__ __launch_bounds__(256) void rmsnorm_rope_kernel(bf16* __restrict__ x0, const float* __restrict__ w0,
+                                                           bf16* __restrict__ x1, const float* __restrict__ w1,
+                                                           const float* __restrict__ cs, int M, int D, int ld,
+                                                           int head_dim, float eps, int rope_rows) {
+  const int lane = threadIdx.x & 63;
+  const int row = blockIdx.x * 4 + (threadIdx.x >> 6);
+  if (row >= M) return;
+  bf16* __restrict__ x = blockIdx.y ? x1 : x0;
+  const float* __restrict__ w = blockIdx.y ? w1 : w0;
+  const int cs_row = rope_rows > 0 ? row % rope_rows : row;
+  rmsnorm_rope_row<FULL>(x + (size_t)row * ld, w, cs, cs_row, D, head_dim, eps, lane);
+}
+
+template <bool FULL>
+__global__ __launch_bounds__(256) void rmsnorm_layers_kernel(bf16* __restrict__ x, const float* __restrict__ w, int M, int D, int ld,
+                                                             int head_dim, float eps) {
+  const int lane = threadIdx.x & 63;
+  const int row = blockIdx.x * 4 + (threadIdx.x >> 6);
+  if (row >= M) return;
+  const int l = blockIdx.y;
+  rmsnorm_rope_row<FULL>(x + (size_t)row * ld + (size_t)l * D, w + (size_t)l * D, nullptr, row, D, head_dim, eps, lane);
 }
 
 template <bool FULL>
@@ -424,6 +439,17 @@
   return (int)hipGetLastError();
 }
 
+CE_API int ce_rmsnorm_layers_bf16(void* x, const float* w, int M, int D, int L, int ld, int head_dim, float eps, hipStream_t stream) {
+  if (!x || !w) return CE_ERR_ARG;
+  if (M <= 0 || D <= 0 || L <= 0 || L > 65535 || (D & 7) || D > 64 * 8 * ROW_MAXC || (ld & 7) || (long long)L * D > ld || (head_dim & 7) || D % head_dim)
+    return CE_ERR_SHAPE;
+  if (D == 64 * 8 * ROW_MAXC)
+    hipLaunchKernelGGL(rmsnorm_layers_kernel<true>, dim3((M + 3) / 4, L), dim3(256), 0, stream, (bf16*)x, w, M, D, ld, head_dim, eps);
+  else
+    hipLaunchKernelGGL(rmsnorm_layers_kernel<false>, dim3((M + 3) / 4, L), dim3(256), 0, stream, (bf16*)x, w, M, D, ld, head_dim, eps);
+  return (int)hipGetLastError();
+}
+
 CE_API int ce_timestep_sinusoid(const int64_t* t, float* out, int dim, hipStream_t stream) {
   if (!t || !out || dim <= 0 || (dim & 1)) return CE_ERR_ARG;
   hipLaunchKernelGGL(timestep_sinusoid_kernel<int64_t>, dim3((dim + 255) / 256), dim3(256), 0, stream, t, out, dim);
diff --git a/chronoedit_amd/hiplib.py b/chronoedit_amd/hiplib.py
--- a/chronoedit_amd/hiplib.py
+++ b/chronoedit_amd/hiplib.py
@@ -26,6 +26,10 @@
 SIGNATURES: Dict[str, List] = {
     "ce_ln_affine_bf16": [_P, _P, _P, _P, _I, _I, _I, _I, _F, _I, _I, _P],
     "ce_rmsnorm_rope_bf16": [_P, _P, _P, _P, _P, _I, _I, _I, _I, _F, _I, _P],
+    "ce_rmsnorm_layers_bf16": [_P, _P, _I, _I, _I, _I, _I, _F, _P],
+    "ce_gemm_bf16_rowssq": [_P, _P, _P, _P, _I, _I, _I, _I, _I, _I, _P, _I, _I, _I, _P, _c.c_size_t, _P],
+    "ce_attention_vt_rawq_bf16": [_P, _P, _P, _I, _I, _I, _P, _I, _I, _I, _I, _I, _F, _I, _P, _I, _P, _P, _I, _F, _P],
+    "ce_attention_2seg_vt_rawq_bf16": [_P, _P, _P, _I, _I, _I, _I, _P, _P, _I, _I, _I, _I, _P, _I, _I, _I, _I, _I, _F, _I, _P, _I, _P, _F, _P],
     "ce_gemm_bf16": [_P, _P, _P, _P, _I, _P, _P, _I, _I, _I, _I, _I, _I, _I, _I, _I, _c.c_longlong, _I, _c.c_longlong, _P, _c.c_size_t, _P],
     "ce_rmsnorm_rope_mxfp8": [_P, _P, _P, _P, _P, _I, _I, _I, _I, _I, _F, _I, _F, _P],
     "ce_v_mxfp8_transpose": [_P, _I, _P, _P, _I, _I, _I, _I, _P],
@@ -87,6 +91,7 @@
     "ce_set_attention_mxfp8_variant": [_I],
     "ce_set_attention_mxfp8_persistent": [_I],
     "ce_diag_attention_exact_route_hits": [_P, _I],
+    "ce_diag_attention_rawq_dump": [_P],
 }
 
 
diff --git a/chronoedit_amd/ops.py b/chronoedit_amd/ops.py
--- a/chronoedit_amd/ops.py
+++ b/chronoedit_amd/ops.py
@@ -206,6 +206,41 @@
                               int(gate_rows), int(a_seg_k), int(a_seg_stride), 0, 0, ws, ws_bytes, _stream()), "ce_gemm_bf16")
     _prof_end(st, f"gemm_{M}x{N}x{K}_epi{epilogue}", 2.0 * M * N * K)
     return out
+
+
+def gemm_rowssq(a: torch.Tensor, w: torch.Tensor, bias: Optional[torch.Tensor], out: torch.Tensor, ssq: torch.Tensor,
+                col0: int = 0, col1: Optional[int] = None) -> bool:
+    _dev(a, torch.bfloat16, "a"), _dev(w, torch.bfloat16, "w"), _dev(out, torch.bfloat16, "out"), _dev(ssq, torch.float32, "ssq")
+    M, K, lda = _rows(a, "a")
+    N, K2, ldw = _rows(w, "w")
+    Mo, No, ldc = _rows(out, "out")
+    Ms, ns, ssq_ld = _rows(ssq, "ssq")
+    col1 = N if col1 is None else col1
+    if K != K2 or (Mo, No) != (M, N) or Ms != M or ns < (col1 - col0) // 128:
+        raise ValueError(f"gemm_rowssq: shapes a {tuple(a.shape)} w {tuple(w.shape)} out {tuple(out.shape)} ssq {tuple(ssq.shape)} [{col0}, {col1})")
+    if bias is not None:
+        _dev(bias, torch.float32, "bias")
+        assert bias.numel() == N and bias.is_contiguous()
+    ws, ws_bytes = _gemm_scratch(a.device)
+    st = _prof_begin()
+    rc = lib().ce_gemm_bf16_rowssq(_ptr(a), _ptr(w), _ptr(out), _ptr(bias), M, N, K, lda, ldw, ldc, _ptr(ssq), ssq_ld, int(col0), int(col1),
+                                   ws, ws_bytes, _stream())
+    if rc == -2:
+        return False
+    _check(rc, "ce_gemm_bf16_rowssq")
+    _prof_end(st, f"gemm_{M}x{N}x{K}_epi{EPI_BIAS}", 2.0 * M * N * K)
+    return True
+
+
+def rmsnorm_layers_(x: torch.Tensor, w: torch.Tensor, head_dim: int, eps: float):
+    _dev(x, torch.bfloat16, "x"), _dev(w, torch.float32, "w")
+    M, cols, ld = _rows(x, "x")
+    assert w.dim() == 2 and w.is_contiguous() and w.shape[0] * w.shape[1] <= cols, (w.shape, x.shape)
+    L, D = w.shape
+    st = _prof_begin()
+    _check(lib().ce_rmsnorm_layers_bf16(_ptr(x), _ptr(w), M, D, L, ld, head_dim, float(eps), _stream()), "ce_rmsnorm_layers_bf16")
+    _prof_end(st, f"rmsnorm_layers_{M}x{D}x{L}", 4.0 * M * D * L)
+    return x
 
 
 def rope_scatter(x: torch.Tensor, cols, weights, D: int, world: int, cos_sin: Optional[torch.Tensor], head_dim: int, eps: float,
@@ -337,7 +372,7 @@
 
 
 def attention_vt(q: torch.Tensor, k: torch.Tensor, vt: torch.Tensor, heads: int, out: Optional[torch.Tensor] = None,
-                 scale: Optional[float] = None, batch: int = 1):
+                 scale: Optional[float] = None, batch: int = 1, raw_q=None):
     for n, t in (("q", q), ("k", k), ("vt", vt)):
         _dev(t, torch.bfloat16, n)
     Nq, Dq, ldq = _rows(q, "q")
@@ -352,8 +387,21 @@
         scale = 128 ** -0.5
     st = _prof_begin()
     nq, l1 = Nq // batch, L1 // batch
-    _check(lib().ce_attention_vt_bf16(_ptr(q), _ptr(k), _ptr(vt), l1, ldk, vt.stride(0), _ptr(out), nq, heads, 128, ldq, ldo, float(scale),
-                                      batch, _stream()), "ce_attention_vt_bf16")
+    if raw_q is not None:
+        ssq, nw, cos_sin, eps = raw_q
+        _dev(ssq, torch.float32, "ssq"), _dev(nw, torch.float32, "w")
+        assert _rows(ssq, "ssq")[0] == Nq and ssq.shape[1] >= heads and nw.is_contiguous() and nw.numel() == Dq
+        rope_rows = 0
+        if cos_sin is not None:
+            _dev(cos_sin, torch.float32, "cos_sin")
+            assert cos_sin.is_contiguous() and cos_sin.shape[1:] == (64, 2) and Nq % cos_sin.shape[0] == 0, (cos_sin.shape, Nq)
+            rope_rows = cos_sin.shape[0]
+        _check(lib().ce_attention_vt_rawq_bf16(_ptr(q), _ptr(k), _ptr(vt), l1, ldk, vt.stride(0), _ptr(out), nq, heads, 128, ldq, ldo,
+                                               float(scale), batch, _ptr(ssq), ssq.stride(0), _ptr(nw), _ptr(cos_sin), rope_rows, float(eps),
+                                               _stream()), "ce_attention_vt_rawq_bf16")
+    else:
+        _check(lib().ce_attention_vt_bf16(_ptr(q), _ptr(k), _ptr(vt), l1, ldk, vt.stride(0), _ptr(out), nq, heads, 128, ldq, ldo, float(scale),
+                                          batch, _stream()), "ce_attention_vt_bf16")
     _prof_end(st, f"attention_{nq}x{l1}+0_h{heads}" + (f"_b{batch}" if batch > 1 else ""), 4.0 * nq * l1 * 128 * heads * batch)
     return out
 
@@ -361,7 +409,7 @@
 def attention_2seg_vt(q: torch.Tensor, k1: torch.Tensor, v1t: torch.Tensor, len1: int, k2: torch.Tensor, v2t: torch.Tensor, len2: int,
                       heads: int, out: Optional[torch.Tensor] = None, scale: Optional[float] = None, batch: int = 1,
                       cols1: Optional[int] = None, cols2: Optional[int] = None, out8: Optional[torch.Tensor] = None,
-                      scale8: Optional[torch.Tensor] = None):
+                      scale8: Optional[torch.Tensor] = None, raw_q=None):
     for n, t in (("q", q), ("k1", k1), ("v1t", v1t), ("k2", k2), ("v2t", v2t)):
         _dev(t, torch.bfloat16, n)
     Nq, Dq, ldq = _rows(q, "q")
@@ -393,9 +441,18 @@
         out = torch.empty((Nq, Dq), dtype=torch.bfloat16, device=q.device)
     _, _, ldo = _rows(out, "out")
     st = _prof_begin()
-    _check(lib().ce_attention_2seg_vt_bf16(_ptr(q), _ptr(k1), _ptr(v1t), len1, ldk1, v1t.stride(0), int(cols1), _ptr(k2), _ptr(v2t),
-                                           len2, ldk2, v2t.stride(0), int(cols2), _ptr(out), nq, heads, 128, ldq, ldo,
-                                           float(scale), batch, _stream()), "ce_attention_2seg_vt_bf16")
+    if raw_q is not None:
+        ssq, nw, eps = raw_q
+        _dev(ssq, torch.float32, "ssq"), _dev(nw, torch.float32, "w")
+        assert _rows(ssq, "ssq")[0] == Nq and ssq.shape[1] >= heads and nw.is_contiguous() and nw.numel() == Dq
+        _check(lib().ce_attention_2seg_vt_rawq_bf16(_ptr(q), _ptr(k1), _ptr(v1t), len1, ldk1, v1t.stride(0), int(cols1), _ptr(k2), _ptr(v2t),
+                                                    len2, ldk2, v2t.stride(0), int(cols2), _ptr(out), nq, heads, 128, ldq, ldo,
+                                                    float(scale), batch, _ptr(ssq), ssq.stride(0), _ptr(nw), float(eps), _stream()),
+               "ce_attention_2seg_vt_rawq_bf16")
+    else:
+        _check(lib().ce_attention_2seg_vt_bf16(_ptr(q), _ptr(k1), _ptr(v1t), len1, ldk1, v1t.stride(0), int(cols1), _ptr(k2), _ptr(v2t),
+                                               len2, ldk2, v2t.stride(0), int(cols2), _ptr(out), nq, heads, 128, ldq, ldo,
+                                               float(scale), batch, _stream()), "ce_attention_2seg_vt_bf16")
     _prof_end(st, f"attention_{nq}x{len1}+{len2}_h{heads}" + (f"_b{batch}" if batch > 1 else ""), 4.0 * nq * (len1 + len2) * 128 * heads * batch)
     return out
 
diff --git a/chronoedit_amd/transformer.py b/chronoedit_amd/transformer.py
--- a/chronoedit_amd/transformer.py
+++ b/chronoedit_amd/transformer.py
@@ -14,6 +14,7 @@
 
 
 _VT_GEMM_SWAPPED = __import__("os").environ.get("CE_VT_GEMM") == "row"
+_FUSED_QNORM = __import__("os").environ.get("CE_FUSED_QNORM", "0") == "1"
 
 
 @dataclass
@@ -184,6 +185,7 @@
         self.sp_batch_cfg = True
         self.fp8_fuse_quant = True
         self.fp8_fuse_attn_quant = True
+        self.fused_qnorm = _FUSED_QNORM
         self.cross_vt = True
         self._sp = None
         self._cfgp = None
@@ -291,6 +293,12 @@
             self._engine.ws_generation += 1
         return self
 
+    def enable_fused_qnorm(self, on: bool = True):
+        self.fused_qnorm = bool(on)
+        if self._engine is not None:
+            self._engine.fused_qnorm = self.fused_qnorm
+        return self
+
     def enable_cross_vt(self, on: bool = True):
         self.cross_vt = bool(on)
         self._engine = None
@@ -324,7 +332,7 @@
         eng = self._engine
         sp = self._sp
         return (self._gen, None if eng is None else eng.ws_generation, self.gemm_dtype, self.fp8_linears, self.attn_dtype, self.v_transposed, self.cross_vt,
-                self.sp_batch_cfg, bool(getattr(self, "rope_plain_temporal", False)), self.cache_context,
+                self.fused_qnorm, self.sp_batch_cfg, bool(getattr(self, "rope_plain_temporal", False)), self.cache_context,
                 None if sp is None else (sp.world, sp.rank), self._cfgp is not None)
 
     @torch.no_grad()
@@ -462,6 +470,7 @@
         self.fuse_quant = bool(getattr(model, "fp8_fuse_quant", True)) and self.F % 128 == 0
         self.fuse_attn_quant = self.fuse_quant and bool(getattr(model, "fp8_fuse_attn_quant", True))
         self.v_transposed = bool(getattr(model, "v_transposed", True))
+        self.fused_qnorm = bool(getattr(model, "fused_qnorm", _FUSED_QNORM))
         if self.fp8:
             if self.D % 256 or self.F % 256:
                 raise NotImplementedError("fp8 GEMMs need inner and ffn dims that are multiples of 256")
@@ -479,6 +488,8 @@
             self.b_k_i_all = torch.cat([f32(blk.attn2.add_k_proj.bias) for blk in model.blocks])
             self.w_v_i_all = self._fuse([blk.attn2.add_v_proj for blk in model.blocks])
             self.b_v_i_all = torch.cat([f32(blk.attn2.add_v_proj.bias) for blk in model.blocks])
+        self.nk2_all = torch.stack([p.nk2 for p in self.blk]).contiguous()
+        self.nk_i_all = torch.stack([p.nk_i for p in self.blk]).contiguous() if self.all_img else None
         self.cross_vt = bool(getattr(model, "cross_vt", True))
         self._ctx_bufs = {}
         self.tables = torch.stack(tables, 0).contiguous()
@@ -572,6 +583,12 @@
             return ws.att
         return y
 
+    def _gemm_raw_q(self, ws, name: str, a: torch.Tensor, w: torch.Tensor, b: torch.Tensor, out: torch.Tensor) -> bool:
+        if not self.fused_qnorm or self.cfg.attention_head_dim != 128 or self.H % 4 or ws.raw_q.get(name) is False:
+            return False
+        ws.raw_q[name] = ops.gemm_rowssq(a, w, b, out, ws.ssq, 0, self.D)
+        return ws.raw_q[name]
+
     def _workspace(self, N: int):
         ws = self._ws.get(N)
         if ws is None:
@@ -579,6 +596,8 @@
             e = lambda *s: torch.empty(s, dtype=torch.bfloat16, device=dev)
             ws = SimpleNamespace(x=e(N, D), h=e(N, D), qkv=e(N, 3 * D), att=e(N, D), q2=e(N, D), ffn=e(N, F),
                                  cols=e(N, self.kpatch), head=e(N, self.w_out.shape[0]))
+            ws.ssq = torch.empty((N, (self.H + 3) // 4 * 4), dtype=torch.float32, device=dev)
+            ws.raw_q = {}
             if self.fp8:
                 ws.a8 = torch.empty((N, max(D, F)), dtype=torch.uint8, device=dev)
                 ws.s8 = (torch.empty((ops.mx_scale_bytes(N, max(D, F)),), dtype=torch.uint8, device=dev) if self.mx else
@@ -687,14 +706,17 @@
             if k_i_all is not None:
                 v_i_all = ops.gemm(enc_i, self.w_v_i_all, self.b_v_i_all)
         kv = []
+        one_launch = not f8
+        if one_launch:
+            ops.rmsnorm_layers_(k_t_all, self.nk2_all, hd, eps)
+            if k_i_all is not None:
+                ops.rmsnorm_layers_(k_i_all, self.nk_i_all, hd, eps)
         for li, p in enumerate(self.blk if not f8 else ()):
             cols = slice(li * D, (li + 1) * D)
             k_t = k_t_all[:, cols]
-            ops.rmsnorm_rope_(k_t, p.nk2, None, hd, eps)
             k_i = None
             if k_i_all is not None:
                 k_i = k_i_all[:, cols]
-                ops.rmsnorm_rope_(k_i, p.nk_i, None, hd, eps)
             if use_vt:
                 kv.append((k_t, v1t[cols], k_i, v2t[cols]))
             else:
@@ -798,13 +820,19 @@
                 if getattr(ws, "vt", None) is None:
                     ws.vt = torch.zeros((D, ops.vt_columns(B * Nl)), dtype=torch.bfloat16, device=self.dev)
                 ops.ln_affine(x, mod[li, 0, 1], mod[li, 0, 0], eps, out=ws.h, ab_rows=Nl, ab_stride=6 * D)
-                ops.gemm(ws.h, p.w_qkv[: 2 * D], p.b_qkv[: 2 * D], out=ws.qkv[:, : 2 * D])
+                raw_q = self._gemm_raw_q(ws, "qk", ws.h, p.w_qkv[: 2 * D], p.b_qkv[: 2 * D], ws.qkv[:, : 2 * D])
+                if not raw_q:
+                    ops.gemm(ws.h, p.w_qkv[: 2 * D], p.b_qkv[: 2 * D], out=ws.qkv[:, : 2 * D])
                 if _VT_GEMM_SWAPPED:
                     ops.gemm(p.w_qkv[2 * D :], ws.h, p.b_qkv[2 * D :], out=ws.vt[:, : B * Nl], epilogue=ops.EPI_BIAS_ROW)
                 else:
                     ops.gemm(ws.h, p.w_qkv[2 * D :], p.b_qkv[2 * D :], out=ws.vt[:, : B * Nl], epilogue=ops.EPI_BIAS_T)
-                ops.rmsnorm_rope_(ws.qkv[:, :D], p.nq1, cs, hd, eps, x2=ws.qkv[:, D : 2 * D], w2=p.nk1)
-                ops.attention_vt(ws.qkv[:, :D], ws.qkv[:, D : 2 * D], ws.vt, H, out=ws.att, batch=B)
+                if raw_q:
+                    ops.rmsnorm_rope_(ws.qkv[:, D : 2 * D], p.nk1, cs, hd, eps)
+                    ops.attention_vt(ws.qkv[:, :D], ws.qkv[:, D : 2 * D], ws.vt, H, out=ws.att, batch=B, raw_q=(ws.ssq, p.nq1, cs, eps))
+                else:
+                    ops.rmsnorm_rope_(ws.qkv[:, :D], p.nq1, cs, hd, eps, x2=ws.qkv[:, D : 2 * D], w2=p.nk1)
+                    ops.attention_vt(ws.qkv[:, :D], ws.qkv[:, D : 2 * D], ws.vt, H, out=ws.att, batch=B)
                 att = ws.att
             elif sp is None:
                 self._ln_linear(ws, x, mod[li, 0, 1], mod[li, 0, 0], p, "qkv", ws.qkv, ab_rows=Nl, ab_stride=6 * D)
@@ -815,11 +843,19 @@
                 att = self._self_attention_ulysses(ws, sp, x, mod[li, 0, 1], mod[li, 0, 0], p, cs, N, Nl, B)
             self._linear(ws, att, p, "o1", x, quantised=q_o1, epilogue=ops.EPI_GATE_RES, gate=gate_msa[li] if B > 1 else mods[0][li, 2],
                          res=x, gate_rows=grow)
-            if p.n2w is not None:
+            q_o2 = bool(ctx.vt and fuse_o2)
+            raw_q2 = False
+            if ctx.vt and not ctx.f8 and not q_o2 and "q2" not in self.fp8_set:
+                a2 = x
+                if p.n2w is not None:
+                    a2 = ops.ln_affine(x, p.n2w, p.n2b, eps, out=ws.h)
+                raw_q2 = self._gemm_raw_q(ws, "q2", a2, p.w_q2, p.b_q2, ws.q2)
+                if not raw_q2:
+                    ops.gemm(a2, p.w_q2, p.b_q2, out=ws.q2)
+            elif p.n2w is not None:
                 self._ln_linear(ws, x, p.n2w, p.n2b, p, "q2", ws.q2)
             else:
                 self._linear(ws, x, p, "q2", ws.q2)
-            q_o2 = bool(ctx.vt and fuse_o2)
             if ctx.f8:
                 seg_t, seg_i = ctx.kv[li]
                 ops.rmsnorm_rope_mxfp8(ws.q2, p.nq2, None, hd, eps, out=ws.q8, scale=ws.sq, post_scale=ops.MXFP8_Q_SCALE)
@@ -835,14 +871,16 @@
                 self._linear(ws, ws.att, p, "o2", x, quantised=q_o2, epilogue=ops.EPI_GATE_RES, gate=None, res=x)
                 k_t = None
             else:
-                ops.rmsnorm_rope_(ws.q2, p.nq2, None, hd, eps)
+                if not raw_q2:
+                    ops.rmsnorm_rope_(ws.q2, p.nq2, None, hd, eps)
                 k_t, v_t, k_i, v_i = ctx.kv[li]
             if k_t is None:
                 pass
             elif ctx.vt and fuse_o2:
                 ops.attention_2seg_vt(ws.q2, k_t, v_t, Tt, k_i, v_i, Ti, H, batch=B, cols1=ctx.c1, cols2=ctx.c2, out8=ws.a8[:, :D], scale8=ws.s8)
             elif ctx.vt:
-                ops.attention_2seg_vt(ws.q2, k_t, v_t, Tt, k_i, v_i, Ti, H, out=ws.att, batch=B, cols1=ctx.c1, cols2=ctx.c2)
+                ops.attention_2seg_vt(ws.q2, k_t, v_t, Tt, k_i, v_i, Ti, H, out=ws.att, batch=B, cols1=ctx.c1, cols2=ctx.c2,
+                                      raw_q=(ws.ssq, p.nq2, eps) if raw_q2 else None)
             elif k_i is not None:
                 ops.attention(ws.q2, k_t, v_t, H, out=ws.att, k2=k_i, v2=v_i, batch=B)
             else:
diff --git a/include/chronoedit_hip.h b/include/chronoedit_hip.h
--- a/include/chronoedit_hip.h
+++ b/include/chronoedit_hip.h
@@ -31,10 +31,15 @@
 int ce_rmsnorm_rope_bf16(void* x, const float* w, void* x2, const float* w2, const float* cos_sin, int M, int D, int ld,
                          int head_dim, float eps, int rope_rows, hipStream_t stream);
 
+int ce_rmsnorm_layers_bf16(void* x, const float* w, int M, int D, int L, int ld, int head_dim, float eps, hipStream_t stream);
+
 int ce_gemm_bf16(const void* A, const void* W, void* C, const float* bias, int epilogue, const float* gate, const void* res,
                  int M, int N, int K, int lda, int ldw, int ldc, int ldres, int gate_rows, int a_seg_k, long long a_seg_stride,
                  int w_seg_k, long long w_seg_stride, void* ws, size_t ws_bytes, hipStream_t stream);
 
+int ce_gemm_bf16_rowssq(const void* A, const void* W, void* C, const float* bias, int M, int N, int K, int lda, int ldw, int ldc, float* ssq,
+                        int ssq_ld, int ssq_col0, int ssq_col1, void* ws, size_t ws_bytes, hipStream_t stream);
+
 
 
 int ce_gemm_bf16_tile_rows(int M, int N, int K, int cus, long long ws_bytes);
@@ -50,9 +55,18 @@
 int ce_attention_vt_bf16(const void* Q, const void* K, const void* Vt, int len, int ldk, int ldvt, void* O, int Nq, int H, int head_dim,
                          int ldq, int ldo, float softmax_scale, int batch, hipStream_t stream);
 
+int ce_attention_vt_rawq_bf16(const void* Q, const void* K, const void* Vt, int len, int ldk, int ldvt, void* O, int Nq, int H, int head_dim,
+                              int ldq, int ldo, float softmax_scale, int batch, const float* ssq, int ssq_ld, const float* nw,
+                              const float* cos_sin, int rope_rows, float eps, hipStream_t stream);
+
 int ce_attention_2seg_vt_bf16(const void* Q, const void* K1, const void* V1t, int len1, int ldk1, int ldv1t, int vt_cols1, const void* K2,
                               const void* V2t, int len2, int ldk2, int ldv2t, int vt_cols2, void* O, int Nq, int H, int head_dim, int ldq,
                               int ldo, float softmax_scale, int batch, hipStream_t stream);
+
+int ce_attention_2seg_vt_rawq_bf16(const void* Q, const void* K1, const void* V1t, int len1, int ldk1, int ldv1t, int vt_cols1, const void* K2,
+                                   const void* V2t, int len2, int ldk2, int ldv2t, int vt_cols2, void* O, int Nq, int H, int head_dim, int ldq,
+                                   int ldo, float softmax_scale, int batch, const float* ssq, int ssq_ld, const float* nw, float eps,
+                                   hipStream_t stream);
 
 int ce_attention_2seg_vt_quant_bf16(const void* Q, const void* K1, const void* V1t, int len1, int ldk1, int ldv1t, int vt_cols1, const void* K2,
                                     const void* V2t, int len2, int ldk2, int ldv2t, int vt_cols2, void* o8, void* scale8, int Nq, int H,
diff --git a/include/chronoedit_hip_diag.h b/include/chronoedit_hip_diag.h
--- a/include/chronoedit_hip_diag.h
+++ b/include/chronoedit_hip_diag.h
@@ -19,6 +19,8 @@
 
 int ce_diag_attention_exact_route_hits(unsigned long long* hits, int reset);
 
+int ce_diag_attention_rawq_dump(void* q_out);
+
 #ifdef __cplusplus
 }
 #endif
```

Result: no change. 3.054, median of 5 (+0.1%).
